# facebookresearch/PartDistillation

Measured on AMD Instinct MI355X. Metric: images/sec training step, R50 Mask2Former 1024² bs=2/GPU, 1/2/4/8 MI355X, higher is better.
Workload: dtype bf16

## Files before the change

### include/pd_fused.h

```cpp
#ifndef PD_FUSED_H
#define PD_FUSED_H

#include <stdint.h>

#ifdef __cplusplus
extern "C" {
#endif

int pd_maxpool3s2_fwd_bf16(const void *x, void *y, void *argmax, int B, int H, int W, int C, void *stream);
int pd_maxpool3s2_bwd_bf16(const void *dy, const void *argmax, void *dx, int B, int H, int W, int C, void *stream);

int pd_affine_act_fwd_bf16(const void *x, const void *residual, const float *scale, const float *bias, void *y,
                           int64_t n, int channels, int relu, void *stream);

int pd_affine_act_bwd_bf16(const void *gy, const void *y, const float *scale, void *gx, void *gres, int64_t n,
                           int channels, int relu, void *stream);
int pd_affine_act_bwd2_bf16(const void *gy, const void *gy2, const void *y, const float *scale, void *gx, void *gres, int64_t n,
                            int channels, int relu, void *stream);

int pd_multi_gather_sumsq(const int64_t *src_ptrs, const int32_t *src_is_bf16, const int32_t *blk_tensor,
                          const int64_t *blk_start, const int64_t *blk_dst, const int32_t *blk_len, float *dst,
                          double *sumsq, int block_begin, int block_end, void *stream);

int pd_nc_sums_f32(const float *x, const float *dy, const float *y, const float *a, const float *b, double *out, int N, int P,
                   int C, int mode, int relu, void *stream);
int pd_nc_affine_f32(const float *x, const float *a, const float *b, float *y, int N, int P, int C, int relu, void *stream);
int pd_nc_affine_amax_f32(const float *x, const float *a, const float *b, float *y, float *amax, int N, int P, int C, int relu, void *stream);
int pd_nc_affine2_amax_f32(const float *dy, const float *x, const float *y, const float *a, const float *p, const float *r, float *dx,
                           float *amax, int N, int P, int C, int relu, void *stream);
int pd_nc_affine2_f32(const float *dy, const float *x, const float *y, const float *a, const float *p, const float *r, float *dx,
                      int N, int P, int C, int relu, void *stream);

int pd_gn_coeffs_fwd(const double *sums, const float *weight, const float *bias, int N, int C, int G, int P, float eps, float *a,
                     float *b, float *mean_c, float *rstd_c, float *xb, void *stream);
int pd_gn_coeffs_bwd(const double *sums, const float *weight, const float *mean_c, const float *rstd_c, int N, int C, int G, int P,
                     float *a, float *pcoef, float *rcoef, float *gw, float *gb, void *stream);

#ifdef __cplusplus
}
#endif
#endif
```

### include/pd_gemm.h

```cpp
#ifndef PD_GEMM_H
#define PD_GEMM_H

#include <stdint.h>

#ifdef __cplusplus
extern "C" {
#endif

int pd_gemm_tn_f32(const float *A, const float *B, const float *bias, float *C, int M, int N, int K, int lda, int ldb,
                   int ldc, int relu, void *stream);

int pd_gemm_tn_f32x3(const float *A, const float *B, const float *bias, float *C, int M, int N, int K, int lda, int ldb,
                     int ldc, int relu, void *stream);

int pd_gemm_wgrad_f32(const float *dY, const float *X, float *dW, float *dB, int M, int N, int K, int ldy, int ldx,
                      int ldw, void *stream);

int pd_gemm_wgrad_acc_f32(const float *dY, const float *X, float *dW, float *dB, int M, int N, int K, int ldy, int ldx,
                          int ldw, void *stream);

int64_t pd_gemm_tn_f32x3_relu_bits_words(int M, int N);
int pd_split3_bf16(const float *W, int N, int K, int ldw, int transpose, void *planes, void *stream);
int pd_gemm_tn_f32x3_pre(const float *A, const void *Bplanes, const float *bias, float *C, uint32_t *bits, float *colsum, int M, int N, int K,
                         int lda, int ldc, int mode, void *stream);
int pd_gemm_tn_f32x3_relu_bits(const float *A, const float *B, const float *bias, float *C, uint32_t *bits, int M, int N, int K, int lda,
                               int ldb, int ldc, void *stream);
int pd_gemm_tn_f32x3_relumask(const float *A, const float *B, const uint32_t *bits, float *C, float *colsum, int M, int N, int K, int lda,
                              int ldb, int ldc, void *stream);

int pd_gemm_wgrad_acc_f32x3(const float *dY, const float *X, float *dW, float *dB, int M, int N, int K, int ldy, int ldx, int ldw,
                            void *stream);
int64_t pd_gemm_wgrad_f32x3_ws_floats(int N, int K);
int pd_gemm_wgrad_acc_f32x3_ws(const float *dY, const float *X, float *dW, float *dB, float *workspace, int64_t workspace_floats, int M, int N,
                               int K, int ldy, int ldx, int ldw, void *stream);

typedef struct PdGemmWgradDesc {
  const float *dY, *X;
  float *dW, *dB;
  int M, N, K, ldy, ldx, ldw;
  const float *y_amax, *x_amax;
} PdGemmWgradDesc;
int64_t pd_gemm_wgrad_f32x3_grouped_table_bytes(int max_count);
int64_t pd_gemm_wgrad_f32x3_grouped_ws_floats(const PdGemmWgradDesc *descs, int count);
int pd_gemm_wgrad_f32x3_grouped(const PdGemmWgradDesc *descs, int count, void *table_host_pinned, void *table_device, float *workspace,
                                int64_t workspace_floats, void *stream);

int pd_conv3x3_wgrad_nhwc_f32x3(const float *dY, const float *X, float *dWk, float *dB, float *workspace, int64_t workspace_floats, int B, int H,
                                int W, int Ci, int Co, void *stream);

int pd_conv3x3_nhwc_f32x3(const float *X, const float *Wk, const float *bias, float *Y, int B, int H, int W, int Ci, int Co,
                          void *stream);

int64_t pd_gemm_wgrad_f16x2_ws_floats(int N, int K);
int pd_gemm_wgrad_f16x2_takes_wide_tiles(int N, int K);
int64_t pd_gemm_wgrad_f16x2_grouped_ws_floats(const PdGemmWgradDesc *descs, int count);
int pd_gemm_wgrad_acc_f16x2_ws(const float *dY, const float *X, float *dW, float *dB, const float *y_amax, const float *x_amax,
                               float *workspace, int64_t workspace_floats, int M, int N, int K, int ldy, int ldx, int ldw, void *stream);
int pd_gemm_wgrad_f16x2_grouped(const PdGemmWgradDesc *descs, int count, void *table_host_pinned, void *table_device, float *workspace,
                                int64_t workspace_floats, void *stream);
int pd_conv3x3_wgrad_nhwc_f16x2(const float *dY, const float *X, float *dWk, float *dB, const float *y_amax, const float *x_amax,
                                float *workspace, int64_t workspace_floats, int B, int H, int W, int Ci, int Co, void *stream);
int pd_gemm_tn_f16x2_which(int M, int N, int K, int lda, int ldb, int mode, int has_bits, int has_a_amax, int has_b_amax, int has_c_amax,
                           int bf16_out);

int pd_conv3x3_nhwc_f16x2(const float *X, const float *Wk, const float *bias, float *Y, const float *x_amax, const float *w_amax, float *y_amax,
                          int B, int H, int W, int Ci, int Co, void *stream);
int64_t pd_gemm_tn_f16x2_bits_words(int M, int N);
int pd_gemm_tn_f16x2(const float *A, const float *B, const float *bias, float *C, uint32_t *bits, float *colsum, const float *a_amax,
                     const float *b_amax, float *c_amax, int M, int N, int K, int lda, int ldb, int ldc, int mode, void *stream);
int pd_row_amax_f32(const float *X, int rows, int cols, int ld, float *out, void *stream);
int pd_gemm_tn_f16x2_bf16out(const float *A, const float *B, const float *bias, void *C_bf16, const float *a_amax, const float *b_amax, int M, int N,
                             int K, int lda, int ldb, int ldc, void *stream);
int pd_cast_bf16_f32_amax(const void *X_bf16, int rows, int cols, float *Y, float *row_amax, void *stream);

#ifdef __cplusplus
}
#endif
#endif
```

### include/pd_rowwise.h

```cpp
#ifndef PD_ROWWISE_H
#define PD_ROWWISE_H

#include <stdint.h>

#ifdef __cplusplus
extern "C" {
#endif

int pd_add_layernorm_fwd(const void *x, int x_dtype, const float *res, const float *gamma, const float *beta, float eps,
                         float *z, float *y, void *y_c, const float *pos, int pos_div, void *ypos_c, int c_dtype,
                         float *mean, float *rstd, int rows, int C, void *stream);

int pd_add_layernorm_bwd(const float *dy, const float *dy2, const void *dy_c, const void *dypos_c, int c_dtype,
                         const float *z, const float *mean, const float *rstd, const float *gamma, float *dz, void *dz_c,
                         int dzc_dtype, float *dgamma, float *dbeta, float *dbias, float *dpos_acc, int pos_div,
                         int rows, int C, void *stream);

int pd_add_layernorm_fwd_amax(const void *x, int x_dtype, const float *res, const float *gamma, const float *beta, float eps,
                              float *z, float *y, void *y_c, const float *pos, int pos_div, void *ypos_c, int c_dtype,
                              float *mean, float *rstd, float *y_amax, float *ypos_amax, int rows, int C, void *stream);
int pd_add_layernorm_bwd_amax(const float *dy, const float *dy2, const void *dy_c, const void *dypos_c, int c_dtype,
                              const float *z, const float *mean, const float *rstd, const float *gamma, float *dz, void *dz_c,
                              int dzc_dtype, float *dgamma, float *dbeta, float *dbias, float *dpos_acc, int pos_div,
                              float *dz_amax, int rows, int C, void *stream);

int pd_colsum_acc(const void *x, int dtype, int rows, int N, float *acc, void *stream);

int pd_relu_bwd_colsum(void *dh, const void *h, int dtype, int rows, int N, float *acc, void *stream);

int pd_mem_prep_fwd(const float *tok, int64_t tok_batch_stride, const float *level_embed, const float *pos, void *mem_c,
                    void *mempos_c, int c_dtype, int B, int HW, int C, void *stream);

int pd_mem_prep_bwd(const void *dmem_c, const void *dmempos_c, int c_dtype, float *dtok, int64_t dtok_batch_stride, int B,
                    int HW, int C, void *stream);

int pd_attn_mask_u8(const void *logits, int dtype, int rows, int n, uint8_t *mask, void *stream);

int pd_matcher_point_terms(const void *x, int dtype, int rows, int n, float *x_f32, float *sigmoid_x, float *softplus_sum,
                           float *sigmoid_sum, void *stream);

int pd_msda_prep_fwd(const float *offs, const float *logits, const float *ref, const int64_t *spatial_shapes, float *loc,
                     float *attn, int64_t tokens, int M, int L, int P, int ld_offs, int ld_logits, void *stream);

int pd_msda_prep_bwd(const float *gloc, const float *gattn, const float *attn, const int64_t *spatial_shapes, float *d_offs,
                     float *d_logits, int64_t tokens, int M, int L, int P, int ld_offs, int ld_logits, void *stream);
int pd_msda_prep_bwd_amax(const float *gloc, const float *gattn, const float *attn, const int64_t *spatial_shapes, float *d_offs, float *d_logits,
                          float *row_amax, int64_t tokens, int M, int L, int P, int ld_offs, int ld_logits, void *stream);

int pd_point_sample_nhwc_f32(const float *in, const float *coords, float *out, int B, int H, int W, int C, int P, void *stream);
int pd_point_sample_nhwc_f32_bf16(const float *in, const float *coords, void *out, int B, int H, int W, int C, int P, void *stream);

int pd_point_sample_planar_f32(const float *in, const float *coords, float *out, int N, int C, int H, int W, int P, void *stream);
int pd_point_sample_planar_bwd_f32(const float *grad_out, const float *coords, float *grad_in, int N, int C, int H, int W, int P, void *stream);
int pd_point_sample_planar_bwd_needs_zero(int C, int H, int W);
int pd_point_sample_planar_bwd_needs_zero_n(int N, int C, int H, int W);

int pd_upsample_add_nhwc_f32(const float *lo, int64_t lo_batch_stride, const float *cur, float *y, int B, int h, int w, int H, int W, int C, void *stream);
int pd_upsample_add_amax_nhwc_f32(const float *lo, int64_t lo_batch_stride, const float *cur, float *y, float *amax, int B, int h, int w, int H, int W, int C,
                                  void *stream);
int pd_upsample2x_bwd_nhwc_f32(const float *dy, float *dlo, int B, int h, int w, int C, void *stream);

#define PD_RESIZE_MAX 4
int pd_resize_bilinear_nhwc_f32(const float *x, int B, int H, int W, int C, const int *heights, const int *widths, void *const *outs, int count,
                                int out_dtype, void *stream);


int pd_add_rows_amax_f32(const float *a, const float *b, float *q, float *a_copy, float *a_amax, float *q_amax, int rows, int cols, void *stream);

int pd_sum3_sum2_f32(const float *a, const float *b, const float *c, const float *d, float *out1, float *out2, int64_t n, void *stream);

int pd_skinny_linear_fwd(const void *x_bf16, const void *w, const void *b, int wb_dtype, float *y, int R, int C, int K, void *stream);
int64_t pd_skinny_linear_partial_floats(int R, int C, int K);
int pd_skinny_linear_bwd(const void *x_bf16, const void *w, int w_dtype, const float *dy, const void *dx_in_bf16, void *dx_out, int dx_dtype,
                         float *partial, void *dw, void *db, int b_dtype, int R, int C, int K, void *stream);

#define PD_TRANSPOSE_MAX 8
typedef struct {
  const void *src;
  void *dst;
  int64_t src_batch_stride, src_row_stride;
  int32_t batch, rows, cols, reserved;
} PdTransposeProblem;
int pd_transpose_batched_f32(const PdTransposeProblem *problems, int count, void *stream);

#define PD_COPY_MAX_SEGS 48
typedef struct PdCopySeg {
  const void *src;
  void *dst;
  int64_t bytes;
} PdCopySeg;
int pd_copy_segments(const PdCopySeg *segs, int count, void *stream);

#ifdef __cplusplus
}
#endif
#endif
```

### partdistillation_amd/csrc/cmdbuf.hip

```cpp
#include <hip/hip_runtime.h>
#include <stdint.h>
#include <string.h>

#include <type_traits>
#include <utility>

#include "pd_common.h"
#include "pd_cmdbuf.h"
#include "pd_attention.h"
#include "pd_conv.h"
#include "pd_declayer.h"
#include "pd_criterion.h"
#include "pd_fused.h"
#include "pd_gemm.h"
#include "pd_grouping.h"
#include "pd_igemm.h"
#include "pd_input.h"
#include "pd_kmeans.h"
#include "pd_msda.h"
#include "pd_mx8.h"
#include "pd_optim.h"
#include "pd_poly.h"
#include "pd_rowwise.h"
#include "pd_smallgemm.h"
// ... 11 lines not shown
  } else if constexpr (std::is_same_v<T, float>) {
    float f; uint32_t u = (uint32_t)w; memcpy(&f, &u, 4); return f;
  } else if constexpr (std::is_same_v<T, double>) {
    double d; memcpy(&d, &w, 8); return d;
  } else {
    return static_cast<T>(static_cast<int64_t>(w));
  }
}

template <auto F> struct Thunk;
template <class... A, int (*F)(A...)>
struct Thunk<F> {
  static constexpr int nargs = (int)sizeof...(A);
  template <size_t... I>
  static int invoke(const uint64_t *w, std::index_sequence<I...>) { return F(word_to<A>(w[I])...); }
  static int call(const uint64_t *w) { return invoke(w, std::index_sequence_for<A...>{}); }
};

struct Entry { const char *name; int (*call)(const uint64_t *); int nargs; };
#define PD_E(f) {#f, &Thunk<&f>::call, Thunk<&f>::nargs}
const Entry kTable[] = {
  PD_E(pd_adamw_clipped),
  PD_E(pd_adamw_clipped_shadow),
  PD_E(pd_add_layernorm_bwd),
  PD_E(pd_add_layernorm_bwd_amax),
  PD_E(pd_add_layernorm_fwd),
  PD_E(pd_add_layernorm_fwd_amax),
  PD_E(pd_add_rows_amax_f32),
  PD_E(pd_affine_act_bwd2_bf16),
  PD_E(pd_affine_act_bwd_bf16),
  PD_E(pd_affine_act_fwd_bf16),
  PD_E(pd_attn_bwd_d32),
  PD_E(pd_attn_fwd_d32),
  PD_E(pd_attn_mask_u8),
  PD_E(pd_cast_bf16_f32_amax),
  PD_E(pd_colsum_acc),
  PD_E(pd_conv3x3_nhwc_f16x2),
  PD_E(pd_conv3x3_nhwc_f32x3),
  PD_E(pd_conv3x3_wgrad_nhwc_f16x2),
  PD_E(pd_conv3x3_wgrad_nhwc_f32x3),
  PD_E(pd_conv_bf16_dgrad),
  PD_E(pd_conv_bf16_fwd),
  PD_E(pd_conv_bf16_wgrad),
  PD_E(pd_conv_bf16_wgrad_grouped),
  PD_E(pd_dec_bwd_a),
  PD_E(pd_dec_bwd_b),
  PD_E(pd_dec_fwd_a),
  PD_E(pd_dec_fwd_b),
  PD_E(pd_dec_pack_grouped),
  PD_E(pd_decoder_head_bf16),
  PD_E(pd_filter_transpose_grouped),
  PD_E(pd_gemm_tn_f16x2),
  PD_E(pd_gemm_tn_f16x2_bf16out),
  PD_E(pd_gemm_tn_f32),
  PD_E(pd_gemm_tn_f32x3),
  PD_E(pd_gemm_tn_f32x3_pre),
  PD_E(pd_gemm_tn_f32x3_relu_bits),
  PD_E(pd_gemm_tn_f32x3_relumask),
  PD_E(pd_gemm_wgrad_acc_f16x2_ws),
  PD_E(pd_gemm_wgrad_acc_f32),
  PD_E(pd_gemm_wgrad_acc_f32x3),
  PD_E(pd_gemm_wgrad_acc_f32x3_ws),
  PD_E(pd_gemm_wgrad_f16x2_grouped),
  PD_E(pd_gemm_wgrad_f32),
  PD_E(pd_gemm_wgrad_f32x3_grouped),
  PD_E(pd_gn_coeffs_bwd),
  PD_E(pd_gn_coeffs_fwd),
  PD_E(pd_igemm_bf16),
  PD_E(pd_igemm_bf16_seq),
  PD_E(pd_kmeans_assign),
  PD_E(pd_kmeans_assign_bounded),
  PD_E(pd_kmeans_assign_partial),
  PD_E(pd_kmeans_reduce),
  PD_E(pd_kmeans_reduce_update),
  PD_E(pd_kmeans_reduce_update_shift),
  PD_E(pd_kmeans_update),
  PD_E(pd_layernorm_rows_f32_bwd),
  PD_E(pd_layernorm_rows_f32_fwd),
  PD_E(pd_loss_vectors_bwd),
  PD_E(pd_loss_vectors_fwd),
  PD_E(pd_lsa_batched),
  PD_E(pd_mask_assign),
  PD_E(pd_mask_point_losses_bwd),
  PD_E(pd_mask_point_losses_fwd),
  PD_E(pd_matcher_costs),
  PD_E(pd_copy_segments),
  PD_E(pd_attn_fwd_d32_ld),
  PD_E(pd_attn_bwd_d32_ld),
  PD_E(pd_match_point_logits),
  PD_E(pd_swin_merge_ln_fwd),
  PD_E(pd_swin_tail_ln_fwd),
  PD_E(pd_swin_tail_ln_bwd),
  PD_E(pd_swin_merge_ln_bwd),
  PD_E(pd_matcher_point_terms),
  PD_E(pd_maxpool3s2_bwd_bf16),
  PD_E(pd_maxpool3s2_fwd_bf16),
  PD_E(pd_mem_prep_bwd),
  PD_E(pd_mem_prep_fwd),
  PD_E(pd_memcpy_d2d_async),
  PD_E(pd_memset_async),
  PD_E(pd_msda_backward),
  PD_E(pd_msda_forward),
  PD_E(pd_msda_forward_amax),
  PD_E(pd_msda_fused_backward),
  PD_E(pd_msda_fused_forward),
  PD_E(pd_msda_prep_bwd),
  PD_E(pd_msda_prep_bwd_amax),
  PD_E(pd_msda_prep_fwd),
  PD_E(pd_multi_gather_sumsq),
  PD_E(pd_mx8_gemm),
  PD_E(pd_mx8_quantize_bf16),
  PD_E(pd_mx8_quantize_grouped),
  PD_E(pd_nc_affine2_amax_f32),
  PD_E(pd_nc_affine2_f32),
  PD_E(pd_nc_affine_amax_f32),
  PD_E(pd_nc_affine_f32),
  PD_E(pd_nc_sums_f32),
  PD_E(pd_normalize_u8_nhwc),
  PD_E(pd_pair_logits_bwd_rows),
  PD_E(pd_pair_logits_bwd_tok),
  PD_E(pd_pair_logits_fwd),
  PD_E(pd_point_sample_nhwc_f32),
  PD_E(pd_point_sample_nhwc_f32_bf16),
  PD_E(pd_point_sample_planar_bwd_f32),
  PD_E(pd_point_sample_planar_f32),
  PD_E(pd_point_sample_u8),
  PD_E(pd_poly_crossings_i32),
  PD_E(pd_relu_bwd_colsum),
  PD_E(pd_resample_cols_canvas_u8),
  PD_E(pd_resample_cols_u8),
  PD_E(pd_resample_rows_u8),
  PD_E(pd_resize_bilinear_nhwc_f32),
  PD_E(pd_rle_sample_groups_canvas_u8),
  PD_E(pd_rle_sample_groups_u8),
  PD_E(pd_rle_sample_u8),
  PD_E(pd_row_amax_f32),
  PD_E(pd_scores_argmax_u8),
  PD_E(pd_sgemm_nn_bf16),
  PD_E(pd_sgemm_nn_splitn_bf16),
  PD_E(pd_sgemm_tn_batched_bf16),
  PD_E(pd_sgemm_tn_bf16),
  PD_E(pd_sgemm_tn_multi_bf16),
  PD_E(pd_sgemm_tn_splitk_bf16),
  PD_E(pd_sgemm_wgrad_bf16),
  PD_E(pd_sgemm_wgrad_grouped_bf16),
  PD_E(pd_sgemm_wgrad_split_bf16),
  PD_E(pd_skinny_linear_bwd),
  PD_E(pd_skinny_linear_fwd),
  PD_E(pd_split3_bf16),
  PD_E(pd_stem7x7_fwd),
  PD_E(pd_stem7x7_wgrad),
  PD_E(pd_sum3_sum2_f32),
  PD_E(pd_sumsq_accumulate),
  PD_E(pd_swin_ln_bwd),
  PD_E(pd_swin_ln_fwd),
  PD_E(pd_transpose_batched_f32),
  PD_E(pd_uncertain_points),
  PD_E(pd_upsample2x_bwd_nhwc_f32),
  PD_E(pd_upsample_add_amax_nhwc_f32),
  PD_E(pd_upsample_add_nhwc_f32),
  PD_E(pd_wgrad_bf16),
  PD_E(pd_wgrad_bf16_seq),
  PD_E(pd_window_attn_bwd_w12),
  PD_E(pd_window_attn_bwd_w7),
  PD_E(pd_window_attn_fwd_w12),
  PD_E(pd_window_attn_fwd_w7),
};
constexpr int kCount = (int)(sizeof(kTable) / sizeof(kTable[0]));
}

extern "C" int pd_memset_async(void *dst, int value, int64_t bytes, void *stream)
{
  if (bytes <= 0) return PD_OK;
  return hipMemsetAsync(dst, value, (size_t)bytes, (hipStream_t)stream) == hipSuccess ? PD_OK : pd_set_error(PD_ERR_LAUNCH, "pd_memset_async failed");
}

extern "C" int pd_memcpy_d2d_async(void *dst, const void *src, int64_t bytes, void *stream)
{
  if (bytes <= 0) return PD_OK;
  return hipMemcpyAsync(dst, src, (size_t)bytes, hipMemcpyDeviceToDevice, (hipStream_t)stream) == hipSuccess ? PD_OK
                                                                                                         : pd_set_error(PD_ERR_LAUNCH, "pd_memcpy_d2d_async failed");
}

extern "C" int pd_cmd_fn_index(const char *name)
{
  if (!name) return -1;
  for (int i = 0; i < kCount; ++i)
    if (!strcmp(kTable[i].name, name)) return i;
  return -1;
}

extern "C" int pd_cmd_fn_nargs(int fn) { return fn >= 0 && fn < kCount ? kTable[fn].nargs : -1; }

extern "C" int pd_cmd_replay(const PdCmd *cmds, int count, const uint64_t *slot_bases, int nslots, void *stream)
{
  uint64_t w[PD_CMD_MAX_ARGS];
  for (int c = 0; c < count; ++c) {
    const PdCmd &k = cmds[c];
    if (k.fn < 0 || k.fn >= kCount || k.nargs != kTable[k.fn].nargs || k.nargs > PD_CMD_MAX_ARGS)
      return pd_set_error(PD_ERR_INVALID_ARG, "pd_cmd_replay: command %d is malformed", c);
    for (int i = 0; i < k.nargs; ++i) {
      const int s = k.kind[i];
      if (s == PD_CMD_LITERAL) w[i] = k.a[i];
      else if (s == PD_CMD_STREAM) w[i] = (uint64_t)(uintptr_t)stream;
      else if (s >= 0 && s < nslots) w[i] = slot_bases[s] + k.a[i];
      else return pd_set_error(PD_ERR_INVALID_ARG, "pd_cmd_replay: command %d argument %d names slot %d of %d", c, i, s, nslots);
    }
    const int rc = kTable[k.fn].call(w);
    if (rc != PD_OK) return rc;
  }
  return PD_OK;
// ... 2 lines not shown
```

### partdistillation_amd/csrc/common.hip

```cpp
#include <hip/hip_runtime.h>
#include <stdarg.h>
#include <stdio.h>
#include <string.h>

#include "pd_common.h"
#include "pd_msda.h"

namespace {
thread_local char g_err[512] = {0};
}

int pd_set_error(int code, const char *fmt, ...)
{
  va_list ap;
  va_start(ap, fmt);
  vsnprintf(g_err, sizeof(g_err), fmt, ap);
  va_end(ap);
  return code;
}

int pd_check_launch(const char *what)
{
  hipError_t e = hipGetLastError();
  if (e == hipSuccess) return PD_OK;
  return pd_set_error(PD_ERR_LAUNCH, "%s: %s", what, hipGetErrorString(e));
}

extern "C" const char *pd_last_error(void) { return g_err; }
extern "C" int pd_abi_version(void) { return 49; }

extern int g_pd_dbg_atomic_scope;
extern int g_pd_dbg_force_generic;
extern int g_pd_dbg_ablate;
extern int g_pd_dbg_x3_narrow;
extern int g_pd_dbg_f16x2;
extern int g_pd_dbg_wgrad_wide;
extern "C" void pd_dbg_set_wgrad_xcd(int v);
extern "C" void pd_dbg_set_wgrad_fast(int v);
extern int g_pd_dbg_bwd_variant;
extern int g_pd_dbg_msda_gate_pct;
extern int g_pd_dbg_wgrad_wgs;
extern int g_pd_dbg_bwd_threads;
extern int g_pd_dbg_attn_scalar;
extern int g_pd_dbg_wattn;
extern int g_pd_dbg_wattn_chunk;
extern int g_pd_dbg_x3;
extern int g_pd_dbg_kmeans;
extern int g_pd_dbg_conv_group_rows;
extern int g_pd_dbg_conv_xcd_major;
extern int g_pd_dbg_sgemm_deep;
extern int g_ig_bn, g_ig_nst, g_ig_splits, g_ig_patch, g_ig_pcls;
extern int g_mx_bn, g_mx_nst;
extern int g_swin_ln_abl;
extern int g_ln_bwd_cap;
extern int g_crit_abl;
extern int g_attn_bwd_kc;
extern int g_wg_nst, g_wg_splits, g_wg_mode;
extern "C" int pd_debug_set(const char *key, int value)
{
  if (!key) return PD_ERR_INVALID_ARG;
  if (!strcmp(key, "msda_bwd_atomic_scope")) { g_pd_dbg_atomic_scope = value; return PD_OK; }
  if (!strcmp(key, "msda_ablate")) { g_pd_dbg_ablate = value; return PD_OK; }
  if (!strcmp(key, "msda_bwd_variant")) { g_pd_dbg_bwd_variant = value; return PD_OK; }
  if (!strcmp(key, "msda_gate_pct")) { g_pd_dbg_msda_gate_pct = value; return PD_OK; }
  if (!strcmp(key, "attn_scalar")) { g_pd_dbg_attn_scalar = value; return PD_OK; }
  if (!strcmp(key, "msda_bwd_threads")) { g_pd_dbg_bwd_threads = value; return PD_OK; }
  if (!strcmp(key, "wgrad_wgs")) { g_pd_dbg_wgrad_wgs = value; return PD_OK; }
  if (!strcmp(key, "kmeans_ablate")) { g_pd_dbg_kmeans = value; return PD_OK; }
  if (!strcmp(key, "wg_nst")) { g_wg_nst = value; return PD_OK; }
  if (!strcmp(key, "wg_splits")) { g_wg_splits = value; return PD_OK; }
  if (!strcmp(key, "wg_mode")) { g_wg_mode = value; return PD_OK; }
  if (!strcmp(key, "ig_bn")) { g_ig_bn = value; return PD_OK; }
  if (!strcmp(key, "ig_patch")) { g_ig_patch = value; return PD_OK; }
  if (!strcmp(key, "ig_pcls")) { g_ig_pcls = value; return PD_OK; }
  if (!strcmp(key, "ig_nst")) { g_ig_nst = value; return PD_OK; }
  if (!strcmp(key, "mx_bn")) { g_mx_bn = value; return PD_OK; }
  if (!strcmp(key, "attn_bwd_kc")) { g_attn_bwd_kc = value; return PD_OK; }
  if (!strcmp(key, "crit_abl")) { g_crit_abl = value; return PD_OK; }
  if (!strcmp(key, "ln_bwd_cap")) { g_ln_bwd_cap = value; return PD_OK; }
  if (!strcmp(key, "swin_ln_abl")) { g_swin_ln_abl = value; return PD_OK; }
  if (!strcmp(key, "mx_nst")) { g_mx_nst = value; return PD_OK; }
  if (!strcmp(key, "ig_splits")) { g_ig_splits = value; return PD_OK; }
  if (!strcmp(key, "sgemm_deep")) { g_pd_dbg_sgemm_deep = value; return PD_OK; }
  if (!strcmp(key, "conv_group_rows")) { g_pd_dbg_conv_group_rows = value; return PD_OK; }
  if (!strcmp(key, "conv_xcd_major")) { g_pd_dbg_conv_xcd_major = value; return PD_OK; }
  if (!strcmp(key, "x3_ablate")) { g_pd_dbg_x3 = value; return PD_OK; }
  if (!strcmp(key, "f16x2_tile")) { g_pd_dbg_f16x2 = value; return PD_OK; }
  if (!strcmp(key, "wgrad_wide")) { g_pd_dbg_wgrad_wide = value; return PD_OK; }
  if (!strcmp(key, "wgrad_xcd")) { pd_dbg_set_wgrad_xcd(value); return PD_OK; }
  if (!strcmp(key, "wgrad_fast")) { pd_dbg_set_wgrad_fast(value); return PD_OK; }
  if (!strcmp(key, "x3_narrow")) { g_pd_dbg_x3_narrow = value; return PD_OK; }
  if (!strcmp(key, "wattn_ablate")) { g_pd_dbg_wattn = value; return PD_OK; }
  if (!strcmp(key, "wattn_chunk")) {
    if (value < 0 || value > 8) return pd_set_error(PD_ERR_INVALID_ARG, "pd_debug_set: wattn_chunk is 0 (automatic) or 1..8, got %d", value);
    g_pd_dbg_wattn_chunk = value;
    return PD_OK;
  }
  if (!strcmp(key, "msda_force_generic")) { g_pd_dbg_force_generic = value; return PD_OK; }
  return pd_set_error(PD_ERR_INVALID_ARG, "pd_debug_set: unknown key %s", key);
}

extern "C" int pd_debug_get(const char *key, int *value)
{
  if (!key || !value) return PD_ERR_INVALID_ARG;
  if (!strcmp(key, "msda_bwd_variant")) { *value = g_pd_dbg_bwd_variant; return PD_OK; }
  if (!strcmp(key, "msda_gate_pct")) { *value = g_pd_dbg_msda_gate_pct; return PD_OK; }
  return pd_set_error(PD_ERR_INVALID_ARG, "pd_debug_get: unknown key %s", key);
}
```

### partdistillation_amd/csrc/fused.hip

```cpp
#include <hip/hip_runtime.h>
#include <stdlib.h>
#include <hip/hip_bf16.h>
#include <stdint.h>

#include "pd_common.h"
#include "pd_fused.h"
#include "pd_msda.h"

namespace {

typedef unsigned short u16x8 __attribute__((ext_vector_type(8)));

__device__ __forceinline__ float bf2f(unsigned short h) { return __uint_as_float((unsigned)h << 16); }
__device__ __forceinline__ unsigned short f2bf(float f)
{
  unsigned u = __float_as_uint(f);
  if ((u & 0x7fffffffu) > 0x7f800000u) return (unsigned short)((u >> 16) | 0x40);
  u += 0x7fffu + ((u >> 16) & 1u);
  return (unsigned short)(u >> 16);
}

__global__ __launch_bounds__(256) void maxpool3s2_fwd(const u16x8 *__restrict__ x, u16x8 *__restrict__ y, unsigned long long *__restrict__ arg,
                                                      int B, int H, int W, int OH, int OW, int c8)
{
// ... 134 lines not shown
  const int b = block_begin + blockIdx.x;
  const int t = blk_tensor[b];
  const int64_t start = blk_start[b];
  const int len = blk_len[b];
  float *d = dst + blk_dst[b];
  const int64_t base = src_ptrs[t];
  float acc = 0.f;
  if (base == 0) {
    for (int i = threadIdx.x; i < len; i += 256) d[i] = 0.f;
  } else if (is_bf16[t]) {
    const unsigned short *s = pd_as_global(reinterpret_cast<const unsigned short *>(base)) + start;
    if ((((uintptr_t)s | (uintptr_t)d) & 15) == 0) {
      const int l8 = len >> 3;
      for (int i = threadIdx.x; i < l8; i += 256) {
        const uint4 u = reinterpret_cast<const uint4 *>(s)[i];
        const float4 a = make_float4(__uint_as_float(u.x << 16), __uint_as_float(u.x & 0xffff0000u), __uint_as_float(u.y << 16), __uint_as_float(u.y & 0xffff0000u));
        const float4 c = make_float4(__uint_as_float(u.z << 16), __uint_as_float(u.z & 0xffff0000u), __uint_as_float(u.w << 16), __uint_as_float(u.w & 0xffff0000u));
        reinterpret_cast<float4 *>(d)[2 * i] = a;
        reinterpret_cast<float4 *>(d)[2 * i + 1] = c;
        acc += (a.x * a.x + a.y * a.y + a.z * a.z + a.w * a.w) + (c.x * c.x + c.y * c.y + c.z * c.z + c.w * c.w);
      }
      for (int i = (l8 << 3) + threadIdx.x; i < len; i += 256) { const float v = bf2f(s[i]); d[i] = v; acc += v * v; }
    } else {
      for (int i = threadIdx.x; i < len; i += 256) { const float v = bf2f(s[i]); d[i] = v; acc += v * v; }
    }
  } else {
    const float *s = pd_as_global(reinterpret_cast<const float *>(base)) + start;
    if ((((uintptr_t)s | (uintptr_t)d) & 15) == 0) {
      const int l4 = len >> 2;
      for (int i = threadIdx.x; i < l4; i += 256) {
        const float4 v = reinterpret_cast<const float4 *>(s)[i];
        reinterpret_cast<float4 *>(d)[i] = v;
        acc += v.x * v.x + v.y * v.y + v.z * v.z + v.w * v.w;
      }
      for (int i = (l4 << 2) + threadIdx.x; i < len; i += 256) { const float v = s[i]; d[i] = v; acc += v * v; }
    } else {
      for (int i = threadIdx.x; i < len; i += 256) { const float v = s[i]; d[i] = v; acc += v * v; }
    }
  }
  if (sumsq) {
    double a = (double)acc;
#pragma unroll
    for (int o = 32; o > 0; o >>= 1) a += __shfl_xor(a, o, 64);
    __shared__ double part[4];
    if ((threadIdx.x & 63) == 0) part[threadIdx.x >> 6] = a;
    __syncthreads();
    if (threadIdx.x == 0) unsafeAtomicAdd(sumsq, part[0] + part[1] + part[2] + part[3]);
  }
}

template <int MODE>
__global__ __launch_bounds__(256) void nc_sums(const float *__restrict__ x, const float *__restrict__ dy, const float *__restrict__ y,
                                                const float *__restrict__ a, const float *__restrict__ b, double *__restrict__ out,
                                                int P, int C, int pix_per_block, int relu)
{
  __shared__ float red[2][256][4];
  const int n = blockIdx.y, cq = C >> 2, q = threadIdx.x % cq, po = threadIdx.x / cq, pstride = 256 / cq;
  const int p0 = blockIdx.x * pix_per_block, p1 = min(P, p0 + pix_per_block);
  const int64_t base = (int64_t)n * P * C + q * 4;
  float4 s0 = make_float4(0, 0, 0, 0), s1 = s0, av = s0, bv = s0;
  if (MODE == 1) { av = *reinterpret_cast<const float4 *>(a + n * C + q * 4); bv = *reinterpret_cast<const float4 *>(b + n * C + q * 4); }
#pragma unroll 4
  for (int p = p0 + po; p < p1; p += pstride) {
    const float4 xv = *reinterpret_cast<const float4 *>(x + base + (int64_t)p * C);
    if (MODE == 0) {
      s0.x += xv.x; s0.y += xv.y; s0.z += xv.z; s0.w += xv.w;
      s1.x += xv.x * xv.x; s1.y += xv.y * xv.y; s1.z += xv.z * xv.z; s1.w += xv.w * xv.w;
    } else {
      float4 g = *reinterpret_cast<const float4 *>(dy + base + (int64_t)p * C);
      if (relu) {
        const float4 yv = *reinterpret_cast<const float4 *>(y + base + (int64_t)p * C);
        g.x = yv.x > 0 ? g.x : 0; g.y = yv.y > 0 ? g.y : 0; g.z = yv.z > 0 ? g.z : 0; g.w = yv.w > 0 ? g.w : 0;
      }
      s0.x += g.x * (xv.x * av.x + bv.x); s0.y += g.y * (xv.y * av.y + bv.y);
      s0.z += g.z * (xv.z * av.z + bv.z); s0.w += g.w * (xv.w * av.w + bv.w);
      s1.x += g.x; s1.y += g.y; s1.z += g.z; s1.w += g.w;
    }
  }
  red[0][threadIdx.x][0] = s0.x; red[0][threadIdx.x][1] = s0.y; red[0][threadIdx.x][2] = s0.z; red[0][threadIdx.x][3] = s0.w;
  red[1][threadIdx.x][0] = s1.x; red[1][threadIdx.x][1] = s1.y; red[1][threadIdx.x][2] = s1.z; red[1][threadIdx.x][3] = s1.w;
  __syncthreads();
  if (threadIdx.x < C) {
    const int c = threadIdx.x, qq = c >> 2, e = c & 3;
    double t0 = 0, t1 = 0;
    for (int k = 0; k < pstride; ++k) { t0 += red[0][k * cq + qq][e]; t1 += red[1][k * cq + qq][e]; }
    unsafeAtomicAdd(out + ((int64_t)n * C + c) * 2, t0);
    unsafeAtomicAdd(out + ((int64_t)n * C + c) * 2 + 1, t1);
  }
}

__device__ __forceinline__ void pixel_amax_store(float4 v, float *__restrict__ amax, int64_t i)
{
  float m = fmaxf(fmaxf(fabsf(v.x), fabsf(v.y)), fmaxf(fabsf(v.z), fabsf(v.w)));
#pragma unroll
  for (int o = 32; o; o >>= 1) m = fmaxf(m, __shfl_xor(m, o, 64));
  if ((threadIdx.x & 63) == 0) amax[i >> 6] = m;
}

template <bool RELU>
__global__ __launch_bounds__(256) void nc_affine(const float4 *__restrict__ x, const float *__restrict__ a, const float *__restrict__ b,
                                                  float4 *__restrict__ y, int64_t n4, int P, int C, float *__restrict__ amax)
{
  const int cq = C >> 2;
  const int64_t stride = (int64_t)gridDim.x * blockDim.x, per_img = (int64_t)P * cq;
  for (int64_t i = (int64_t)blockIdx.x * blockDim.x + threadIdx.x; i < n4; i += stride) {
    const int n = (int)(i / per_img), q = (int)(i % cq);
    const float4 av = *reinterpret_cast<const float4 *>(a + n * C + q * 4), bv = *reinterpret_cast<const float4 *>(b + n * C + q * 4);
    float4 v = x[i];
    v.x = v.x * av.x + bv.x; v.y = v.y * av.y + bv.y; v.z = v.z * av.z + bv.z; v.w = v.w * av.w + bv.w;
    if (RELU) { v.x = fmaxf(v.x, 0.f); v.y = fmaxf(v.y, 0.f); v.z = fmaxf(v.z, 0.f); v.w = fmaxf(v.w, 0.f); }
    y[i] = v;
    if (amax) pixel_amax_store(v, amax, i);
  }
}

template <bool RELU>
__global__ __launch_bounds__(256) void nc_affine2(const float4 *__restrict__ dy, const float4 *__restrict__ x, const float4 *__restrict__ y,
                                                   const float *__restrict__ a, const float *__restrict__ pc, const float *__restrict__ rc,
                                                   float4 *__restrict__ dx, int64_t n4, int P, int C, float *__restrict__ amax)
{
  const int cq = C >> 2;
  const int64_t stride = (int64_t)gridDim.x * blockDim.x, per_img = (int64_t)P * cq;
  for (int64_t i = (int64_t)blockIdx.x * blockDim.x + threadIdx.x; i < n4; i += stride) {
    const int n = (int)(i / per_img), q = (int)(i % cq);
    const float4 av = *reinterpret_cast<const float4 *>(a + n * C + q * 4), pv = *reinterpret_cast<const float4 *>(pc + n * C + q * 4),
                 rv = *reinterpret_cast<const float4 *>(rc + n * C + q * 4);
    float4 g = dy[i];
    const float4 xv = x[i];
    if (RELU) {
      const float4 yv = y[i];
      g.x = yv.x > 0 ? g.x : 0; g.y = yv.y > 0 ? g.y : 0; g.z = yv.z > 0 ? g.z : 0; g.w = yv.w > 0 ? g.w : 0;
    }
    const float4 o = make_float4(g.x * av.x + xv.x * pv.x + rv.x, g.y * av.y + xv.y * pv.y + rv.y, g.z * av.z + xv.z * pv.z + rv.z,
                                 g.w * av.w + xv.w * pv.w + rv.w);
    dx[i] = o;
    if (amax) pixel_amax_store(o, amax, i);
  }
}

inline int grid_for(int64_t n) { int64_t b = (n + 255) / 256; return (int)(b < 1 ? 1 : (b > 8192 ? 8192 : b)); }


__global__ __launch_bounds__(256) void gn_coeffs_fwd(const double *__restrict__ sums, const float *__restrict__ weight,
                                                     const float *__restrict__ bias, int N, int C, int G, double m, double eps,
                                                     float *__restrict__ a, float *__restrict__ b, float *__restrict__ mean_c,
                                                     float *__restrict__ rstd_c, float *__restrict__ xb)
{
  const int i = blockIdx.x * blockDim.x + threadIdx.x;
  if (i >= N * C) return;
  const int n = i / C, c = i - n * C, cpg = C / G, c0 = (c / cpg) * cpg;
  double s0 = 0.0, s1 = 0.0;
  for (int j = 0; j < cpg; ++j) {
    s0 += sums[((int64_t)n * C + c0 + j) * 2];
    s1 += sums[((int64_t)n * C + c0 + j) * 2 + 1];
  }
  const double mean = s0 / m;
  double var = s1 / m - mean * mean;
  var = var < 0.0 ? 0.0 : var;
  const float rstd = (float)(1.0 / sqrt(var + eps)), mu = (float)mean;
  const float av = rstd * weight[c];
  a[i] = av;
  b[i] = bias[c] - mu * av;
  mean_c[i] = mu;
  rstd_c[i] = rstd;
  xb[i] = -mu * rstd;
}

__global__ __launch_bounds__(256) void gn_coeffs_bwd(const double *__restrict__ sums, const float *__restrict__ weight,
                                                     const float *__restrict__ mean_c, const float *__restrict__ rstd_c, int N,
                                                     int C, int G, double m, float *__restrict__ a, float *__restrict__ pcoef,
                                                     float *__restrict__ rcoef, float *__restrict__ gw, float *__restrict__ gb)
{
  const int i = blockIdx.x * blockDim.x + threadIdx.x;
  if (i >= N * C) return;
  const int n = i / C, c = i - n * C, cpg = C / G, c0 = (c / cpg) * cpg;
  double S1 = 0.0, S2 = 0.0;
  for (int j = 0; j < cpg; ++j) {
    const double w = (double)weight[c0 + j];
    S1 += sums[((int64_t)n * C + c0 + j) * 2] * w;
    S2 += sums[((int64_t)n * C + c0 + j) * 2 + 1] * w;
  }
  S1 /= m; S2 /= m;
// ... 52 lines not shown
  dim3 g(grid_for(n8)), b(256);
#define LAUNCH(R, A) hipLaunchKernelGGL((affine_act_fwd<R, A>), g, b, 0, s, (const u16x8 *)x, (const u16x8 *)residual, scale, bias, (u16x8 *)y, n8, c8)
  if (residual) { if (relu) LAUNCH(true, true); else LAUNCH(true, false); }
  else { if (relu) LAUNCH(false, true); else LAUNCH(false, false); }
#undef LAUNCH
  return pd_check_launch("pd_affine_act_fwd_bf16");
}

extern "C" int pd_affine_act_bwd2_bf16(const void *gy, const void *gy2, const void *y, const float *scale, void *gx, void *gres, int64_t n,
                                       int channels, int relu, void *stream_)
{
  if (n < 0 || channels <= 0 || (channels & 7) || (n % channels)) return pd_set_error(PD_ERR_INVALID_ARG, "pd_affine_act_bwd_bf16: n=%lld channels=%d", (long long)n, channels);
  if (n == 0) return PD_OK;
  if (!gy || !scale || !gx || (relu && !y)) return pd_set_error(PD_ERR_INVALID_ARG, "pd_affine_act_bwd_bf16: null pointer");
  const int64_t n8 = n / 8;
  const int c8 = channels / 8;
  hipStream_t s = (hipStream_t)stream_;
  dim3 g(grid_for(n8)), b(256);
#define LAUNCH(R, A, T) hipLaunchKernelGGL((affine_act_bwd<R, A, T>), g, b, 0, s, (const u16x8 *)gy, (const u16x8 *)gy2, (const u16x8 *)y, scale, (u16x8 *)gx, (u16x8 *)gres, n8, c8)
#define LAUNCH2(R, A) do { if (gy2) LAUNCH(R, A, true); else LAUNCH(R, A, false); } while (0)
  if (gres) { if (relu) LAUNCH2(true, true); else LAUNCH2(true, false); }
  else { if (relu) LAUNCH2(false, true); else LAUNCH2(false, false); }
#undef LAUNCH2
#undef LAUNCH
  return pd_check_launch("pd_affine_act_bwd_bf16");
}

extern "C" int pd_affine_act_bwd_bf16(const void *gy, const void *y, const float *scale, void *gx, void *gres, int64_t n,
                                      int channels, int relu, void *stream_)
{
  return pd_affine_act_bwd2_bf16(gy, nullptr, y, scale, gx, gres, n, channels, relu, stream_);
}

extern "C" int pd_multi_gather_sumsq(const int64_t *src_ptrs, const int32_t *src_is_bf16, const int32_t *blk_tensor,
                                     const int64_t *blk_start, const int64_t *blk_dst, const int32_t *blk_len, float *dst,
                                     double *sumsq, int block_begin, int block_end, void *stream_)
{
  if (block_end < block_begin) return pd_set_error(PD_ERR_INVALID_ARG, "pd_multi_gather_sumsq: bad block range");
  if (block_end == block_begin) return PD_OK;
  if (!src_ptrs || !src_is_bf16 || !blk_tensor || !blk_start || !blk_dst || !blk_len || !dst)
    return pd_set_error(PD_ERR_INVALID_ARG, "pd_multi_gather_sumsq: null pointer");
  hipLaunchKernelGGL(multi_gather_sumsq, dim3(block_end - block_begin), dim3(256), 0, (hipStream_t)stream_, src_ptrs, src_is_bf16,
                     blk_tensor, blk_start, blk_dst, blk_len, dst, sumsq, block_begin);
  return pd_check_launch("pd_multi_gather_sumsq");
}

static int nc_check(int N, int P, int C, const char *who)
{
  if (N < 0 || P < 0 || C <= 0 || (C & 3) || (256 % (C >> 2)) != 0 || C > 256)
    return pd_set_error(PD_ERR_INVALID_ARG, "%s: N=%d P=%d C=%d (C must be 4*2^k <= 256)", who, N, P, C);
  return PD_OK;
}

extern "C" int pd_nc_sums_f32(const float *x, const float *dy, const float *y, const float *a, const float *b, double *out,
                              int N, int P, int C, int mode, int relu, void *stream_)
{
  int rc = nc_check(N, P, C, "pd_nc_sums_f32");
  if (rc) return rc;
  if (!out) return pd_set_error(PD_ERR_INVALID_ARG, "pd_nc_sums_f32: null output");
  hipStream_t s = (hipStream_t)stream_;
  (void)hipMemsetAsync(out, 0, (size_t)N * C * 2 * sizeof(double), s);
  if ((int64_t)N * P == 0) return pd_check_launch("pd_nc_sums_f32");
  if (!x || (mode == 1 && (!dy || !a || !b || (relu && !y)))) return pd_set_error(PD_ERR_INVALID_ARG, "pd_nc_sums_f32: null input");
  static const int ppb_env = []() { const char *e = getenv("PD_NC_PPB"); return e ? atoi(e) : 0; }();
  const int64_t np = (int64_t)N * P;
  int ppb = mode == 0 ? (np >= 131072 ? 512 : np >= 32768 ? 256 : np >= 8192 ? 128 : 64) : (np >= 131072 ? 256 : np >= 32768 ? 128 : 32);
  if (ppb_env > 0) ppb = ppb_env;
  dim3 grid((P + ppb - 1) / ppb, N);
  if (mode == 0) hipLaunchKernelGGL(nc_sums<0>, grid, dim3(256), 0, s, x, dy, y, a, b, out, P, C, ppb, relu);
  else hipLaunchKernelGGL(nc_sums<1>, grid, dim3(256), 0, s, x, dy, y, a, b, out, P, C, ppb, relu);
  return pd_check_launch("pd_nc_sums_f32");
}

static int nc_affine_launch(const float *x, const float *a, const float *b, float *y, int N, int P, int C, int relu, void *stream_, float *amax)
{
  int rc = nc_check(N, P, C, "pd_nc_affine_f32");
  if (amax && C != 256) return pd_set_error(PD_ERR_INVALID_ARG, "pd_nc_affine_amax_f32: pixel maxima need C == 256");
  if (rc) return rc;
  const int64_t n4 = (int64_t)N * P * C / 4;
  if (n4 == 0) return PD_OK;
  if (!x || !a || !b || !y) return pd_set_error(PD_ERR_INVALID_ARG, "pd_nc_affine_f32: null pointer");
  hipStream_t s = (hipStream_t)stream_;
  if (relu) hipLaunchKernelGGL(nc_affine<true>, dim3(grid_for(n4)), dim3(256), 0, s, (const float4 *)x, a, b, (float4 *)y, n4, P, C, amax);
  else hipLaunchKernelGGL(nc_affine<false>, dim3(grid_for(n4)), dim3(256), 0, s, (const float4 *)x, a, b, (float4 *)y, n4, P, C, amax);
  return pd_check_launch("pd_nc_affine_f32");
}

extern "C" int pd_nc_affine_f32(const float *x, const float *a, const float *b, float *y, int N, int P, int C, int relu, void *stream_)
{
  return nc_affine_launch(x, a, b, y, N, P, C, relu, stream_, nullptr);
}

extern "C" int pd_nc_affine_amax_f32(const float *x, const float *a, const float *b, float *y, float *amax, int N, int P, int C, int relu, void *stream_)
{
  return nc_affine_launch(x, a, b, y, N, P, C, relu, stream_, amax);
}

static int nc_affine2_launch(const float *dy, const float *x, const float *y, const float *a, const float *p, const float *r,
                             float *dx, int N, int P, int C, int relu, void *stream_, float *amax)
{
  int rc = nc_check(N, P, C, "pd_nc_affine2_f32");
  if (amax && C != 256) return pd_set_error(PD_ERR_INVALID_ARG, "pd_nc_affine2_amax_f32: pixel maxima need C == 256");
  if (rc) return rc;
  const int64_t n4 = (int64_t)N * P * C / 4;
  if (n4 == 0) return PD_OK;
  if (!dy || !x || !a || !p || !r || !dx || (relu && !y)) return pd_set_error(PD_ERR_INVALID_ARG, "pd_nc_affine2_f32: null pointer");
  hipStream_t s = (hipStream_t)stream_;
  if (relu) hipLaunchKernelGGL(nc_affine2<true>, dim3(grid_for(n4)), dim3(256), 0, s, (const float4 *)dy, (const float4 *)x, (const float4 *)y, a, p, r, (float4 *)dx, n4, P, C, amax);
  else hipLaunchKernelGGL(nc_affine2<false>, dim3(grid_for(n4)), dim3(256), 0, s, (const float4 *)dy, (const float4 *)x, (const float4 *)y, a, p, r, (float4 *)dx, n4, P, C, amax);
  return pd_check_launch("pd_nc_affine2_f32");
}

extern "C" int pd_nc_affine2_f32(const float *dy, const float *x, const float *y, const float *a, const float *p, const float *r,
                                 float *dx, int N, int P, int C, int relu, void *stream_)
{
  return nc_affine2_launch(dy, x, y, a, p, r, dx, N, P, C, relu, stream_, nullptr);
}

extern "C" int pd_nc_affine2_amax_f32(const float *dy, const float *x, const float *y, const float *a, const float *p, const float *r,
                                      float *dx, float *amax, int N, int P, int C, int relu, void *stream_)
{
  return nc_affine2_launch(dy, x, y, a, p, r, dx, N, P, C, relu, stream_, amax);
}

extern "C" int pd_gn_coeffs_fwd(const double *sums, const float *weight, const float *bias, int N, int C, int G, int P, float eps,
                                float *a, float *b, float *mean_c, float *rstd_c, float *xb, void *stream_)
{
  if (N < 0 || C <= 0 || G <= 0 || (C % G) || P <= 0) return pd_set_error(PD_ERR_INVALID_ARG, "pd_gn_coeffs_fwd: N=%d C=%d G=%d P=%d", N, C, G, P);
  if (N == 0) return PD_OK;
  if (!sums || !weight || !bias || !a || !b || !mean_c || !rstd_c || !xb) return pd_set_error(PD_ERR_INVALID_ARG, "pd_gn_coeffs_fwd: null pointer");
  hipLaunchKernelGGL(gn_coeffs_fwd, dim3((N * C + 255) / 256), dim3(256), 0, (hipStream_t)stream_, sums, weight, bias, N, C, G,
                     (double)P * (C / G), (double)eps, a, b, mean_c, rstd_c, xb);
  return pd_check_launch("pd_gn_coeffs_fwd");
}

extern "C" int pd_gn_coeffs_bwd(const double *sums, const float *weight, const float *mean_c, const float *rstd_c, int N, int C,
                                int G, int P, float *a, float *pcoef, float *rcoef, float *gw, float *gb, void *stream_)
{
  if (N < 0 || C <= 0 || G <= 0 || (C % G) || P <= 0) return pd_set_error(PD_ERR_INVALID_ARG, "pd_gn_coeffs_bwd: N=%d C=%d G=%d P=%d", N, C, G, P);
  if (N == 0) return PD_OK;
  if (!sums || !weight || !mean_c || !rstd_c || !a || !pcoef || !rcoef || !gw || !gb) return pd_set_error(PD_ERR_INVALID_ARG, "pd_gn_coeffs_bwd: null pointer");
  hipLaunchKernelGGL(gn_coeffs_bwd, dim3((N * C + 255) / 256), dim3(256), 0, (hipStream_t)stream_, sums, weight, mean_c, rstd_c, N, C,
                     G, (double)P * (C / G), a, pcoef, rcoef, gw, gb);
  return pd_check_launch("pd_gn_coeffs_bwd");
}
```

### partdistillation_amd/csrc/gemm_f16x2.hip

```cpp
#include <hip/hip_runtime.h>
#include <stdint.h>
#include <stdlib.h>
#include <utility>
#include <type_traits>

#include "f16x2.h"
#include "pd_common.h"
#include "xcd.h"
#include "pd_gemm.h"
#include "pd_msda.h"

#ifndef PD_ABL
#define PD_ABL 0
#endif

namespace {
using namespace pdh2;
__device__ __forceinline__ int xcd_chunk(int bid, int nb) { return pd_xcd_chunk(bid, nb); }
__device__ __forceinline__ unsigned short f2bf_rne(float f)
{
  unsigned u = __float_as_uint(f);
  if ((u & 0x7fffffffu) > 0x7f800000u) return (unsigned short)((u >> 16) | 0x40u);
  u += 0x7fffu + ((u >> 16) & 1u);
  return (unsigned short)(u >> 16);
}

template <int TM, int TN, int WN, int BKK, int MODE, bool CONV = false, int NRS = 1, int FAST = 0>
__global__ __launch_bounds__((TM / 64) * (TN / WN) * 64, (TM == 256 ? 1 : 2))
void gemm_tn_f16x2(const float *__restrict__ A, const float *__restrict__ B, const float *__restrict__ bias, float *__restrict__ C,
                   int M, int N, int K, int lda, int ldb, int ldc, int ntiles_n, uint32_t *__restrict__ bits,
                   float *__restrict__ colsum, const float *__restrict__ a_amax, const float *__restrict__ b_amax,
                   unsigned *__restrict__ c_amax, int H, int W, int tap_minor)
{
  constexpr int WVN = TN / WN, NW = (TM / 64) * WVN, NTH = NW * 64, NJ = WN / 32;
  constexpr int TPR = BKK / 4, RPP = NTH / TPR, APASS = TM / RPP, BPASS = TN / RPP, NPAN = BKK / 8;
  static_assert(TM % RPP == 0 && TN % RPP == 0, "staging passes");
  constexpr int ASZ = 2 * NPAN * TM * 8, BSZ = 2 * NPAN * TN * 8;
  extern __shared__ __attribute__((aligned(16))) float sc[];
  h16_t *smem = reinterpret_cast<h16_t *>(sc + 2 * (TM + TN));
  auto As = [&](int buf, int pl, int pan, int r) -> h16_t * { return smem + buf * (ASZ + BSZ) + (((pl * NPAN + pan) * TM + r) << 3); };
  auto Bs = [&](int buf, int pl, int pan, int r) -> h16_t * { return smem + buf * (ASZ + BSZ) + ASZ + (((pl * NPAN + pan) * TN + r) << 3); };
  const int lb = xcd_chunk(blockIdx.x, gridDim.x);
  const int m0 = (lb / ntiles_n) * TM, n0 = (lb % ntiles_n) * TN;
  const int t = threadIdx.x, lane = t & 63, wave = t >> 6;
  const int wm = (wave / WVN) * 64, wn = (wave % WVN) * WN;
  const int lr = t / TPR, lk = (t % TPR) * 4;
  for (int r = t; r < TM + TN; r += NTH) {
    const bool isa = r < TM;
    const int g = isa ? m0 + r : n0 + r - TM;
    const float *am = isa ? a_amax : b_amax;
    float s = 1.f, inv = 1.f;
    if (!(PD_ABL & 32) && am && g < (isa ? M : N)) {
      float mx = am[g];
      if (CONV && isa) {
        const int pix = g % (H * W), y = pix / W, x = pix - y * W;
#pragma unroll
        for (int dy = -1; dy <= 1; ++dy)
#pragma unroll
          for (int dx = -1; dx <= 1; ++dx)
            if (y + dy >= 0 && y + dy < H && x + dx >= 0 && x + dx < W) mx = fmaxf(mx, am[g + dy * W + dx]);
      }
      row_scale(mx, s, inv);
    }
    sc[r] = s; sc[TM + TN + r] = inv;
  }
  __syncthreads();
  float sa[APASS], sb[BPASS];
#pragma unroll
  for (int j = 0; j < APASS; ++j) sa[j] = sc[lr + RPP * j];
#pragma unroll
  for (int j = 0; j < BPASS; ++j) sb[j] = sc[TM + lr + RPP * j];
  float4 ra[NRS][APASS], rb[NRS][BPASS];
  int py[APASS], px[APASS];
  if (CONV) {
#pragma unroll
    for (int j = 0; j < APASS; ++j) {
      const int pix = (m0 + lr + RPP * j) % (H * W);
      py[j] = pix / W;
      px[j] = pix - py[j] * W;
    }
  }
  auto gload = [&](int rs, int k0) {
    if (PD_ABL & 8) {
#pragma unroll
      for (int j = 0; j < APASS; ++j) ra[rs][j] = make_float4(1.f, 0.5f, 0.25f, (float)k0);
#pragma unroll
      for (int j = 0; j < BPASS; ++j) rb[rs][j] = make_float4(1.f, 0.5f, 0.25f, (float)k0);
      return;
    }
    const int k = k0 + lk;
    int dy = 0, dx = 0, kc = k, kb = k;
    if (CONV) {
      int tap;
      if (tap_minor) { const int s = k0 / BKK; const int cb = s / 9; tap = s - cb * 9; kc = cb * BKK + lk; kb = tap * lda + kc; }
// ... 942 lines not shown
        }
        hipLaunchKernelGGL(split_planes_f16x2, dim3((unsigned)(((int64_t)N * (K / 4) + 255) / 256)), dim3(256), 0, st, B, ldb, b_amax, planes, N, K);
        const float *bpl = reinterpret_cast<const float *>(planes);
        if (p.abl == 16) KPC(true, 16, true, bpl);
        else if (a_amax) KPC(true, 0, true, bpl);
        else KPC(false, 0, true, bpl);
        return pd_check_launch("pd_gemm_tn_f16x2 (producer / consumer wavefronts, weight planes)");
      }
      if (p.abl) {
        with_constant(p.abl, KpcAbl{}, [&](auto abl) { KPC(true, decltype(abl)::value, false, B); });
        return pd_check_launch("pd_gemm_tn_f16x2 (producer / consumer wavefronts, ablation)");
      }
#endif
      if (a_amax) KPC(true, 0, false, B);
      else KPC(false, 0, false, B);
#undef KPC
      return pd_check_launch("pd_gemm_tn_f16x2 (producer / consumer wavefronts)");
    }
#define GO(TM, TN, WN, NRS, FAST) return launch_f16x2<TM, TN, WN, 16, false, NRS, FAST>(A, B, bias, C, M, N, K, lda, ldb, ldc, mode, bits, colsum, a_amax, b_amax, c_amax, st, flags)
    case F16X2_TILE256:
      if (p.refuse)
        return pd_set_error(PD_ERR_INVALID_ARG, bits ? "pd_gemm_tn_f16x2: sign bits need N %% 256 == 0 and M >= 1024" : "pd_gemm_tn_f16x2: 256 x 256 tiles need N %% 256 == 0 and M >= 1024");
      if (p.nrs == 1) GO(256, 256, 128, 1, 0);
      if (!p.fast) GO(256, 256, 128, 2, 0);
      GO(256, 256, 128, 2, 1);
    default:
      if (p.nrs == 1) GO(128, 128, 64, 1, 0);
      if (!p.fast) GO(128, 128, 64, 2, 0);
      GO(128, 128, 64, 2, 1);
#undef GO
  }
}

extern "C" int pd_gemm_tn_f16x2_which(int M, int N, int K, int lda, int ldb, int mode, int has_bits, int has_a_amax, int has_b_amax, int has_c_amax,
                                      int bf16_out)
{
  const F16x2Plan p = f16x2_plan(M, N, K, lda, ldb, mode, has_bits != 0, has_a_amax != 0, has_b_amax != 0, has_c_amax != 0, bf16_out != 0, g_pd_dbg_f16x2,
                                 cu_count());
  return p.refuse ? -1 : (int)p.family;
}

extern "C" int pd_gemm_tn_f16x2(const float *A, const float *B, const float *bias, float *C, uint32_t *bits, float *colsum, const float *a_amax,
                                const float *b_amax, float *c_amax, int M, int N, int K, int lda, int ldb, int ldc, int mode, void *stream_)
{
  return gemm_tn_f16x2_impl(A, B, bias, C, bits, colsum, a_amax, b_amax, c_amax, M, N, K, lda, ldb, ldc, mode, stream_, 0);
}

extern "C" int pd_gemm_tn_f16x2_bf16out(const float *A, const float *B, const float *bias, void *C_bf16, const float *a_amax, const float *b_amax,
                                        int M, int N, int K, int lda, int ldb, int ldc, void *stream_)
{
  return gemm_tn_f16x2_impl(A, B, bias, reinterpret_cast<float *>(C_bf16), nullptr, nullptr, a_amax, b_amax, nullptr, M, N, K, lda, ldb, ldc, 0, stream_, 1);
}

extern "C" int pd_cast_bf16_f32_amax(const void *X_bf16, int rows, int cols, float *Y, float *row_amax, void *stream_)
{
  if (rows < 0 || cols <= 0 || (cols & 7)) return pd_set_error(PD_ERR_INVALID_ARG, "pd_cast_bf16_f32_amax: rows=%d cols=%d (a multiple of 8)", rows, cols);
  if (rows == 0) return PD_OK;
  if (!X_bf16 || !Y || !row_amax || ((uintptr_t)X_bf16 & 15) || ((uintptr_t)Y & 15)) return pd_set_error(PD_ERR_INVALID_ARG, "pd_cast_bf16_f32_amax: null / misaligned pointer");
  hipLaunchKernelGGL(cast_bf16_f32_amax, dim3((unsigned)((rows + 3) / 4)), dim3(256), 0, (hipStream_t)stream_, (const unsigned short *)X_bf16, rows, cols, Y,
                     row_amax);
  return pd_check_launch("pd_cast_bf16_f32_amax");
}

extern "C" int pd_conv3x3_nhwc_f16x2(const float *X, const float *Wk, const float *bias, float *Y, const float *x_amax, const float *w_amax,
                                     float *y_amax, int B, int H, int W, int Ci, int Co, void *stream_)
{
  if (B < 0 || H <= 0 || W <= 0 || Ci <= 0 || Co <= 0 || (Ci & 15))
    return pd_set_error(PD_ERR_INVALID_ARG, "pd_conv3x3_nhwc_f16x2: B=%d H=%d W=%d Ci=%d (%% 16) Co=%d", B, H, W, Ci, Co);
  if (B == 0) return PD_OK;
  if (!X || !Wk || !Y || ((uintptr_t)X & 15) || ((uintptr_t)Wk & 15)) return pd_set_error(PD_ERR_INVALID_ARG, "pd_conv3x3_nhwc_f16x2: null / misaligned pointer");
  const int64_t M = (int64_t)B * H * W;
  if (M > 0x7fffffffLL - 4096) return pd_set_error(PD_ERR_INVALID_ARG, "pd_conv3x3_nhwc_f16x2: too many pixels");
  hipStream_t st = (hipStream_t)stream_;
  const int dbg = g_pd_dbg_f16x2;
#ifdef PD_PROBES
  if ((dbg == DBG_KPC_ANY || dbg == DBG_KPC_PLANES_STAMPS) && x_amax && w_amax && !y_amax && (Co % 256) == 0 && (Ci % KR_KC) == 0 && ((Ci / KR_KC) & (Ci / KR_KC - 1)) == 0 && M >= 8192 &&
      H < 65536 && W < 65536 && M * Ci * 4 < (1ll << 31) && (int64_t)Co * 9 * Ci * 4 < (1ll << 31)) {
    const int np = Co / 256, G = items_grid(cu_count(), M, np);
    if (dbg == DBG_KPC_PLANES_STAMPS) {
      launch_lds<gemm_kpc_f16x2<true, 16, false, true>>(G, 768, KP_LDS, st, X, Wk, bias, Y, (int)M, 9 * Ci, Ci, 9 * Ci, Co, np, x_amax, w_amax, H, W);
      return pd_check_launch("pd_conv3x3_nhwc_f16x2 (producer / consumer wavefronts, stamps)");
    }
    launch_lds<gemm_kpc_f16x2<true, 0, false, true>>(G, 768, KP_LDS, st, X, Wk, bias, Y, (int)M, 9 * Ci, Ci, 9 * Ci, Co, np, x_amax, w_amax, H, W);
    return pd_check_launch("pd_conv3x3_nhwc_f16x2 (producer / consumer wavefronts)");
  }
#endif
  const bool wide = dbg == DBG_WIDE_1 || (dbg != DBG_TILE_1 && (Co % 256) == 0 && M >= 65536);
  if (dbg == DBG_GUARDED || dbg == DBG_CONV_KORDER) {
    if (wide) return launch_f16x2<256, 256, 128, 16, true>(X, Wk, bias, Y, (int)M, Co, 9 * Ci, Ci, 9 * Ci, Co, 0, nullptr, nullptr, x_amax, w_amax, y_amax, st, H, W);
    return launch_f16x2<128, 128, 64, 16, true>(X, Wk, bias, Y, (int)M, Co, 9 * Ci, Ci, 9 * Ci, Co, 0, nullptr, nullptr, x_amax, w_amax, y_amax, st, H, W);
  }
  if (wide) return launch_f16x2<256, 256, 128, 16, true, 1, 1>(X, Wk, bias, Y, (int)M, Co, 9 * Ci, Ci, 9 * Ci, Co, 0, nullptr, nullptr, x_amax, w_amax, y_amax, st, H, W);
  return launch_f16x2<128, 128, 64, 16, true, 1, 1>(X, Wk, bias, Y, (int)M, Co, 9 * Ci, Ci, 9 * Ci, Co, 0, nullptr, nullptr, x_amax, w_amax, y_amax, st, H, W);
}

extern "C" int pd_row_amax_f32(const float *X, int rows, int cols, int ld, float *out, void *stream_)
{
  if (rows < 0 || cols < 0) return pd_set_error(PD_ERR_INVALID_ARG, "pd_row_amax_f32: negative size");
  if (rows == 0) return PD_OK;
  if (!X || !out) return pd_set_error(PD_ERR_INVALID_ARG, "pd_row_amax_f32: null pointer");
  hipLaunchKernelGGL(row_amax_f32, dim3((unsigned)((rows + 3) / 4)), dim3(256), 0, (hipStream_t)stream_, X, rows, cols, ld, out);
  return pd_check_launch("pd_row_amax_f32");
}

extern "C" int pd_debug_read_kpc_trace(unsigned long long *dst)
{
// ... 3 lines not shown
```

### partdistillation_amd/csrc/rowwise.hip

```cpp
#include <hip/hip_runtime.h>
#include <stdint.h>
#include <string.h>

#include "pd_common.h"
#include "pd_msda.h"
#include "pd_rowwise.h"

int g_ln_bwd_cap = 0;
namespace {

typedef unsigned short bf16_t;

__device__ __forceinline__ float bf2f(bf16_t h) { return __uint_as_float((unsigned)h << 16); }
__device__ __forceinline__ bf16_t f2bf(float f)
{
  unsigned u = __float_as_uint(f);
  if ((u & 0x7fffffffu) > 0x7f800000u) return (bf16_t)((u >> 16) | 0x40);
  u += 0x7fffu + ((u >> 16) & 1u);
  return (bf16_t)(u >> 16);
}

__device__ __forceinline__ float4 ld4(const float *p) { return *reinterpret_cast<const float4 *>(p); }
__device__ __forceinline__ float4 ld4(const bf16_t *p)
{
// ... 606 lines not shown
    const int lx = x0 - tx0, ly = y0 - ty0;
    float acc = 0.f;
    if (vy0 && vx0) acc += tile[ly * (PST + 1) + lx] * wnw;
    if (vy0 && vx1) acc += tile[ly * (PST + 1) + lx + 1] * wne;
    if (vy1 && vx0) acc += tile[(ly + 1) * (PST + 1) + lx] * wsw;
    if (vy1 && vx1) acc += tile[(ly + 1) * (PST + 1) + lx + 1] * wse;
    out[(int64_t)n * P + p] = acc;
  }
}

__global__ __launch_bounds__(256) void point_sample_tiled_bwd(const float *__restrict__ gout, const float *__restrict__ coords,
                                                              float *__restrict__ gin, int H, int W, int P, int tiles_x)
{
  extern __shared__ float tile[];
  const int n = blockIdx.y, ty0 = (blockIdx.x / tiles_x) * PST, tx0 = (blockIdx.x % tiles_x) * PST;
  for (int i = threadIdx.x; i < PST * PST; i += 256) tile[i] = 0.f;
  __syncthreads();
  const float *cn = coords + (int64_t)n * P * 2, *gn = gout + (int64_t)n * P;
  for (int p = threadIdx.x; p < P; p += 256) {
    const float2 c = *reinterpret_cast<const float2 *>(cn + 2 * p);
    const float gx = 2.0f * c.x - 1.0f, gy = 2.0f * c.y - 1.0f;
    const float ix = ((gx + 1.f) * W - 1.f) / 2.f, iy = ((gy + 1.f) * H - 1.f) / 2.f;
    const float fx = floorf(ix), fy = floorf(iy);
    if (fx < tx0 - 1.f || fx >= tx0 + PST || fy < ty0 - 1.f || fy >= ty0 + PST) continue;
    const int x0 = (int)fx, y0 = (int)fy, x1 = x0 + 1, y1 = y0 + 1;
    const float g = gn[p];
    const float wnw = (x1 - ix) * (y1 - iy), wne = (ix - x0) * (y1 - iy), wsw = (x1 - ix) * (iy - y0), wse = (ix - x0) * (iy - y0);
    const int lx0 = x0 - tx0, ly0 = y0 - ty0, lx1 = lx0 + 1, ly1 = ly0 + 1;
    const bool ax0 = lx0 >= 0 && lx0 < PST && x0 < W, ax1 = lx1 >= 0 && lx1 < PST && x1 < W;
    const bool ay0 = ly0 >= 0 && ly0 < PST && y0 < H, ay1 = ly1 >= 0 && ly1 < PST && y1 < H;
    if (ay0 && ax0) atomicAdd(&tile[ly0 * PST + lx0], g * wnw);
    if (ay0 && ax1) atomicAdd(&tile[ly0 * PST + lx1], g * wne);
    if (ay1 && ax0) atomicAdd(&tile[ly1 * PST + lx0], g * wsw);
    if (ay1 && ax1) atomicAdd(&tile[ly1 * PST + lx1], g * wse);
  }
  __syncthreads();
  float *m = gin + (int64_t)n * H * W;
  for (int i = threadIdx.x; i < PST * PST; i += 256) {
    const int y = ty0 + i / PST, x = tx0 + i % PST;
    if (y < H && x < W) m[(int64_t)y * W + x] = tile[i];
  }
}

__device__ __forceinline__ void up_src(int dst, float scale, int in_size, int &i0, int &ip, float &l0, float &l1)
{
  float src = scale * (dst + 0.5f) - 0.5f;
  src = src < 0.f ? 0.f : src;
  i0 = (int)src;
  ip = (i0 < in_size - 1) ? 1 : 0;
  l1 = src - i0;
  l0 = 1.f - l1;
}

__global__ __launch_bounds__(256) void upsample_add_nhwc(const float *__restrict__ lo, const float *__restrict__ cur,
                                                         float *__restrict__ y, int B, int h, int w, int H, int W, int C4,
                                                         float sh, float sw, float *__restrict__ amax, int64_t lo_bs4)
{
  const int64_t total = (int64_t)B * H * W * C4;
  for (int64_t i = (int64_t)blockIdx.x * blockDim.x + threadIdx.x; i < total; i += (int64_t)gridDim.x * blockDim.x) {
    const int c = (int)(i % C4);
    int64_t t = i / C4;
    const int ox = (int)(t % W); t /= W;
    const int oy = (int)(t % H);
    const int b = (int)(t / H);
    int y0, yp, x0, xp; float hy0, hy1, wx0, wx1;
    up_src(oy, sh, h, y0, yp, hy0, hy1);
    up_src(ox, sw, w, x0, xp, wx0, wx1);
    const float4 *L = reinterpret_cast<const float4 *>(lo) + (int64_t)b * lo_bs4;
    const float4 a = L[((int64_t)y0 * w + x0) * C4 + c], bq = L[((int64_t)y0 * w + x0 + xp) * C4 + c];
    const float4 cq = L[((int64_t)(y0 + yp) * w + x0) * C4 + c], d = L[((int64_t)(y0 + yp) * w + x0 + xp) * C4 + c];
    const float4 u = reinterpret_cast<const float4 *>(cur)[i];
    float4 o;
    o.x = u.x + (hy0 * (wx0 * a.x + wx1 * bq.x) + hy1 * (wx0 * cq.x + wx1 * d.x));
    o.y = u.y + (hy0 * (wx0 * a.y + wx1 * bq.y) + hy1 * (wx0 * cq.y + wx1 * d.y));
    o.z = u.z + (hy0 * (wx0 * a.z + wx1 * bq.z) + hy1 * (wx0 * cq.z + wx1 * d.z));
    o.w = u.w + (hy0 * (wx0 * a.w + wx1 * bq.w) + hy1 * (wx0 * cq.w + wx1 * d.w));
    reinterpret_cast<float4 *>(y)[i] = o;
    if (amax) {
      float m = amax4(o);
#pragma unroll
      for (int of = 32; of; of >>= 1) m = fmaxf(m, __shfl_xor(m, of, 64));
      if ((threadIdx.x & 63) == 0) amax[i >> 6] = m;
    }
  }
}

struct ResizeLevels { void *out[PD_RESIZE_MAX]; int h[PD_RESIZE_MAX], w[PD_RESIZE_MAX]; int64_t first[PD_RESIZE_MAX + 1]; int count; };

template <bool BF16>
__global__ __launch_bounds__(256) void resize_bilinear_nhwc_multi(const float *__restrict__ x, int B, int H, int W, int C4, ResizeLevels lv)
{
  for (int64_t i = (int64_t)blockIdx.x * 256 + threadIdx.x; i < lv.first[lv.count]; i += (int64_t)gridDim.x * 256) {
    int l = 0;
#pragma unroll
    for (int k = 1; k < PD_RESIZE_MAX; ++k) l += (k < lv.count && i >= lv.first[k]) ? 1 : 0;
    const int h = lv.h[l], w = lv.w[l];
    int64_t t = i - lv.first[l];
    const int c = (int)(t % C4); t /= C4;
    const int ox = (int)(t % w); t /= w;
    const int oy = (int)(t % h);
    const int b = (int)(t / h);
    int y0, yp, x0, xp; float hy0, hy1, wx0, wx1;
    up_src(oy, (float)H / (float)h, H, y0, yp, hy0, hy1);
    up_src(ox, (float)W / (float)w, W, x0, xp, wx0, wx1);
    const float4 *L = reinterpret_cast<const float4 *>(x) + (int64_t)b * H * W * C4;
    const float4 a = L[((int64_t)y0 * W + x0) * C4 + c], bq = L[((int64_t)y0 * W + x0 + xp) * C4 + c];
    const float4 cq = L[((int64_t)(y0 + yp) * W + x0) * C4 + c], d = L[((int64_t)(y0 + yp) * W + x0 + xp) * C4 + c];
    float4 o;
    o.x = hy0 * (wx0 * a.x + wx1 * bq.x) + hy1 * (wx0 * cq.x + wx1 * d.x);
    o.y = hy0 * (wx0 * a.y + wx1 * bq.y) + hy1 * (wx0 * cq.y + wx1 * d.y);
    o.z = hy0 * (wx0 * a.z + wx1 * bq.z) + hy1 * (wx0 * cq.z + wx1 * d.z);
    o.w = hy0 * (wx0 * a.w + wx1 * bq.w) + hy1 * (wx0 * cq.w + wx1 * d.w);
    const int64_t oi = (((int64_t)b * h + oy) * w + ox) * C4 + c;
    if (BF16) st4(reinterpret_cast<bf16_t *>(lv.out[l]) + oi * 4, o);
    else st4(reinterpret_cast<float *>(lv.out[l]) + oi * 4, o);
  }
}

__global__ __launch_bounds__(256) void upsample2x_bwd_nhwc(const float *__restrict__ dy, float *__restrict__ dlo, int B, int h,
                                                           int w, int C4)
{
  const int H = 2 * h, W = 2 * w;
  const int64_t total = (int64_t)B * h * w * C4;
  for (int64_t i = (int64_t)blockIdx.x * blockDim.x + threadIdx.x; i < total; i += (int64_t)gridDim.x * blockDim.x) {
// ... 351 lines not shown
    return pd_set_error(PD_ERR_INVALID_ARG, "pd_msda_prep_bwd: row strides %d / %d (>= row length, multiples of 4)", ld_offs, ld_logits);
  if (tokens < 0 || M <= 0 || L <= 0 || P <= 0) return pd_set_error(PD_ERR_INVALID_ARG, "pd_msda_prep_bwd: tokens=%lld M=%d L=%d P=%d", (long long)tokens, M, L, P);
  if (tokens == 0) return PD_OK;
  if (!gloc || !gattn || !attn || !spatial_shapes || !d_offs || !d_logits) return pd_set_error(PD_ERR_INVALID_ARG, "pd_msda_prep_bwd: null pointer");
  const int64_t total = tokens * M;
  const dim3 g((unsigned)((total + 255) / 256)), b(256);
  hipStream_t s = (hipStream_t)stream_;
  const int LP = L * P;
#define LAUNCH(KER) hipLaunchKernelGGL(KER, g, b, 0, s, gloc, gattn, attn, spatial_shapes, d_offs, d_logits, total, M, L, P, ld_offs, ld_logits, row_amax)
  if ((P & 1) == 0 && LP == 12) LAUNCH(msda_prep_bwd_v<3>);
  else if ((P & 1) == 0 && LP == 16) LAUNCH(msda_prep_bwd_v<4>);
  else if ((P & 1) == 0 && LP == 8) LAUNCH(msda_prep_bwd_v<2>);
  else hipLaunchKernelGGL(msda_prep_bwd, g, b, 0, s, gloc, gattn, attn, spatial_shapes, d_offs, d_logits, total, M, L, P, ld_offs, ld_logits);
#undef LAUNCH
  return pd_check_launch("pd_msda_prep_bwd");
}

extern "C" int pd_msda_prep_bwd(const float *gloc, const float *gattn, const float *attn, const int64_t *spatial_shapes, float *d_offs,
                                float *d_logits, int64_t tokens, int M, int L, int P, int ld_offs, int ld_logits, void *stream_)
{
  return msda_prep_bwd_launch(gloc, gattn, attn, spatial_shapes, d_offs, d_logits, tokens, M, L, P, ld_offs, ld_logits, stream_, nullptr);
}

extern "C" int pd_msda_prep_bwd_amax(const float *gloc, const float *gattn, const float *attn, const int64_t *spatial_shapes, float *d_offs,
                                     float *d_logits, float *row_amax, int64_t tokens, int M, int L, int P, int ld_offs, int ld_logits, void *stream_)
{
  return msda_prep_bwd_launch(gloc, gattn, attn, spatial_shapes, d_offs, d_logits, tokens, M, L, P, ld_offs, ld_logits, stream_, row_amax);
}

extern "C" int pd_point_sample_nhwc_f32(const float *in, const float *coords, float *out, int B, int H, int W, int C, int P,
                                        void *stream_)
{
  if (B < 0 || H <= 0 || W <= 0 || C <= 0 || (C & 3) || P < 0) return pd_set_error(PD_ERR_INVALID_ARG, "pd_point_sample_nhwc_f32: B=%d H=%d W=%d C=%d P=%d", B, H, W, C, P);
  if (B == 0 || P == 0) return PD_OK;
  if (!in || !coords || !out) return pd_set_error(PD_ERR_INVALID_ARG, "pd_point_sample_nhwc_f32: null pointer");
  const int64_t total = (int64_t)B * P;
  const unsigned grid = (unsigned)((total + 3) / 4 < 16384 ? (total + 3) / 4 : 16384);
  hipLaunchKernelGGL(point_sample_nhwc<float>, dim3(grid), dim3(256), 0, (hipStream_t)stream_, in, coords, out, B, H, W, C, P);
  return pd_check_launch("pd_point_sample_nhwc_f32");
}

extern "C" int pd_point_sample_nhwc_f32_bf16(const float *in, const float *coords, void *out, int B, int H, int W, int C, int P,
                                             void *stream_)
{
  if (B < 0 || H <= 0 || W <= 0 || C <= 0 || (C & 3) || P < 0) return pd_set_error(PD_ERR_INVALID_ARG, "pd_point_sample_nhwc_f32_bf16: B=%d H=%d W=%d C=%d P=%d", B, H, W, C, P);
  if (B == 0 || P == 0) return PD_OK;
  if (!in || !coords || !out) return pd_set_error(PD_ERR_INVALID_ARG, "pd_point_sample_nhwc_f32_bf16: null pointer");
  const int64_t total = (int64_t)B * P;
  const unsigned grid = (unsigned)((total + 3) / 4 < 16384 ? (total + 3) / 4 : 16384);
  hipLaunchKernelGGL(point_sample_nhwc<bf16_t>, dim3(grid), dim3(256), 0, (hipStream_t)stream_, in, coords, (bf16_t *)out, B, H, W, C, P);
  return pd_check_launch("pd_point_sample_nhwc_f32_bf16");
}

static int upsample_add_launch(const float *lo, int64_t lo_bs, const float *cur, float *y, int B, int h, int w, int H, int W, int C, void *stream_, float *amax)
{
  if (lo_bs == 0) lo_bs = (int64_t)h * w * C;
  if (lo_bs < (int64_t)h * w * C || (lo_bs & 3)) return pd_set_error(PD_ERR_INVALID_ARG, "pd_upsample_add_nhwc_f32: lo_batch_stride %lld (>= h w C, a multiple of 4)", (long long)lo_bs);
  if (amax && C != 256) return pd_set_error(PD_ERR_INVALID_ARG, "pd_upsample_add_amax_nhwc_f32: pixel maxima need C == 256");
  if (B < 0 || h <= 0 || w <= 0 || H <= 0 || W <= 0 || C <= 0 || (C & 3)) return pd_set_error(PD_ERR_INVALID_ARG, "pd_upsample_add_nhwc_f32: bad sizes");
  if (B == 0) return PD_OK;
  if (!lo || !cur || !y) return pd_set_error(PD_ERR_INVALID_ARG, "pd_upsample_add_nhwc_f32: null pointer");
  const int64_t total = (int64_t)B * H * W * (C / 4);
  const unsigned grid = (unsigned)((total + 255) / 256 < 32768 ? (total + 255) / 256 : 32768);
  hipLaunchKernelGGL(upsample_add_nhwc, dim3(grid), dim3(256), 0, (hipStream_t)stream_, lo, cur, y, B, h, w, H, W, C / 4,
                     (float)h / (float)H, (float)w / (float)W, amax, lo_bs / 4);
  return pd_check_launch("pd_upsample_add_nhwc_f32");
}

extern "C" int pd_upsample_add_nhwc_f32(const float *lo, int64_t lo_batch_stride, const float *cur, float *y, int B, int h, int w, int H, int W, int C,
                                        void *stream_)
{
  return upsample_add_launch(lo, lo_batch_stride, cur, y, B, h, w, H, W, C, stream_, nullptr);
}

extern "C" int pd_upsample_add_amax_nhwc_f32(const float *lo, int64_t lo_batch_stride, const float *cur, float *y, float *amax, int B, int h, int w, int H,
                                             int W, int C, void *stream_)
{
  return upsample_add_launch(lo, lo_batch_stride, cur, y, B, h, w, H, W, C, stream_, amax);
}

extern "C" int pd_upsample2x_bwd_nhwc_f32(const float *dy, float *dlo, int B, int h, int w, int C, void *stream_)
{
  if (B < 0 || h <= 0 || w <= 0 || C <= 0 || (C & 3)) return pd_set_error(PD_ERR_INVALID_ARG, "pd_upsample2x_bwd_nhwc_f32: bad sizes");
  if (B == 0) return PD_OK;
  if (!dy || !dlo) return pd_set_error(PD_ERR_INVALID_ARG, "pd_upsample2x_bwd_nhwc_f32: null pointer");
  const int64_t total = (int64_t)B * h * w * (C / 4);
  const unsigned grid = (unsigned)((total + 255) / 256 < 32768 ? (total + 255) / 256 : 32768);
  hipLaunchKernelGGL(upsample2x_bwd_nhwc, dim3(grid), dim3(256), 0, (hipStream_t)stream_, dy, dlo, B, h, w, C / 4);
  return pd_check_launch("pd_upsample2x_bwd_nhwc_f32");
}

extern "C" int pd_point_sample_planar_f32(const float *in, const float *coords, float *out, int N, int C, int H, int W, int P, void *stream_)
{
  if (N < 0 || C <= 0 || H <= 0 || W <= 0 || P < 0) return pd_set_error(PD_ERR_INVALID_ARG, "pd_point_sample_planar_f32: N=%d C=%d H=%d W=%d P=%d", N, C, H, W, P);
  if ((int64_t)N * P == 0) return PD_OK;
  if (!in || !coords || !out) return pd_set_error(PD_ERR_INVALID_ARG, "pd_point_sample_planar_f32: null pointer");
  const int tx = (W + PST - 1) / PST, ty = (H + PST - 1) / PST;
  if (C == 1 && tx * ty <= 1 && N <= 65535) {
    hipLaunchKernelGGL(point_sample_tiled_fwd, dim3(tx * ty, N), dim3(256), (PST + 1) * (PST + 1) * sizeof(float), (hipStream_t)stream_, in,
                       coords, out, H, W, P, tx);
    return pd_check_launch("pd_point_sample_planar_f32");
  }
  const int64_t blocks = ((int64_t)N * P + 255) / 256;
  hipLaunchKernelGGL(point_sample_planar_fwd, dim3((unsigned)(blocks > 65536 ? 65536 : blocks)), dim3(256), 0, (hipStream_t)stream_, in, coords, out,
                     N, C, H, W, P);
  return pd_check_launch("pd_point_sample_planar_f32");
}

extern "C" int pd_point_sample_planar_bwd_f32(const float *grad_out, const float *coords, float *grad_in, int N, int C, int H, int W, int P,
                                              void *stream_)
{
  if (N < 0 || C <= 0 || H <= 0 || W <= 0 || P < 0) return pd_set_error(PD_ERR_INVALID_ARG, "pd_point_sample_planar_bwd_f32: N=%d C=%d H=%d W=%d P=%d", N, C, H, W, P);
  if ((int64_t)N * P == 0) return PD_OK;
  if (!grad_out || !coords || !grad_in) return pd_set_error(PD_ERR_INVALID_ARG, "pd_point_sample_planar_bwd_f32: null pointer");
  const int tx = (W + PST - 1) / PST, ty = (H + PST - 1) / PST;
  if (C == 1 && tx * ty <= 16 && N <= 65535) {
    hipLaunchKernelGGL(point_sample_tiled_bwd, dim3(tx * ty, N), dim3(256), PST * PST * sizeof(float), (hipStream_t)stream_, grad_out, coords,
                       grad_in, H, W, P, tx);
    return pd_check_launch("pd_point_sample_planar_bwd_f32");
// ... 210 lines not shown
```

### partdistillation_amd/functions/conv_x3.py

```python
import torch
from torch.autograd import Function

from .. import lib as _lib


H2 = __import__("os").environ.get("PD_H2_CONV", "1") != "0"
H2_1X1 = __import__("os").environ.get("PD_H2_1X1", "1") != "0"
WGRAD_X3 = True


def supported(x, conv):
    return (x.is_cuda and x.dtype == torch.float32 and x.dim() == 4 and conv.weight.dtype == torch.float32
            and tuple(conv.kernel_size) == (3, 3) and tuple(conv.stride) == (1, 1) and tuple(conv.padding) == (1, 1)
            and tuple(conv.dilation) == (1, 1) and conv.groups == 1 and x.shape[1] % 16 == 0 and conv.weight.shape[0] % 16 == 0
            and x.is_contiguous(memory_format=torch.channels_last))


def _pixel_amax(x):
    from . import amax_cache
    from .gemm import row_amax
    am = amax_cache.get(x)
    return am if am is not None else row_amax(x.permute(0, 2, 3, 1).reshape(-1, x.shape[1]))


# ... 16 lines not shown
class Conv3x3X3(Function):
    @staticmethod
    def forward(ctx, x, weight, bias):
        if not x.is_cuda:
            raise RuntimeError("pd_conv3x3_nhwc_f32x3 runs on the GPU only (no CPU fallback in partdistillation_amd)")
        x = x.contiguous(memory_format=torch.channels_last)
        wk = weight.permute(0, 2, 3, 1).contiguous()
        x_am = _pixel_amax(x) if H2 else None
        ctx.save_for_backward(x, weight, x_am)
        ctx.has_bias = bias is not None
        return _raw(x, wk, bias, weight.shape[0], x_am)

    @staticmethod
    def backward(ctx, dy):
        x, weight, x_am = ctx.saved_tensors
        dy = dy.contiguous(memory_format=torch.channels_last)
        co, ci = weight.shape[0], weight.shape[1]
        dx = dw = db = None
        dy_am = _pixel_amax(dy) if x_am is not None else None
        if ctx.needs_input_grad[0]:
            wt = weight.permute(0, 2, 3, 1).reshape(co, 9, ci).flip(1).permute(2, 1, 0).contiguous()
            dx = _raw(dy, wt, None, ci, dy_am)
        want_w, want_b = ctx.needs_input_grad[1], ctx.has_bias and ctx.needs_input_grad[2]
        if (want_w or want_b) and WGRAD_X3 and ci % 128 == 0 and co % 4 == 0:
            from .gemm import _wgrad_workspace
            L = _lib.load()
            B, _, H, W = x.shape
            buf = torch.zeros(co * 9 * ci + co, dtype=torch.float32, device=x.device)
            dwk, dbv = buf[:co * 9 * ci].view(co, 3, 3, ci), buf[co * 9 * ci:]
            ws = _wgrad_workspace(x.device, int((L.pd_gemm_wgrad_f16x2_ws_floats if x_am is not None else L.pd_gemm_wgrad_f32x3_ws_floats)(co, 9 * ci)))
            if x_am is not None:
                _lib.check(L.pd_conv3x3_wgrad_nhwc_f16x2(dy.data_ptr(), x.data_ptr(), dwk.data_ptr(), dbv.data_ptr() if want_b else None,
                                                         dy_am.data_ptr(), x_am.data_ptr(), ws.data_ptr() if ws is not None else None,
                                                         ws.numel() if ws is not None else 0, B, H, W, ci, co, _lib.current_stream()))
            else:
                _lib.check(L.pd_conv3x3_wgrad_nhwc_f32x3(dy.data_ptr(), x.data_ptr(), dwk.data_ptr(), dbv.data_ptr() if want_b else None,
                                                         ws.data_ptr() if ws is not None else None, ws.numel() if ws is not None else 0,
                                                         B, H, W, ci, co, _lib.current_stream()))
            dw = dwk.permute(0, 3, 1, 2) if want_w else None
            db = dbv if want_b else None
        elif want_w or want_b:
            _, dw, db = torch.ops.aten.convolution_backward(dy, x, weight, [co] if ctx.has_bias else None, [1, 1], [1, 1], [1, 1], False,
                                                            [0, 0], 1, [False, True, ctx.has_bias])
        return dx, dw, db


def conv3x3(x, weight, bias=None):
    return Conv3x3X3.apply(x, weight, bias)


class Conv1x1OwnWgrad(Function):

    @staticmethod
    def forward(ctx, x, weight, bias):
        ctx.has_bias = bias is not None
        ctx.x_bf16 = x.dtype == torch.bfloat16
        if H2 and H2_1X1 and x.is_contiguous(memory_format=torch.channels_last):
            from .gemm import cast_rows_amax, gemm_tn_h2, row_amax
            B, ci, Hh, Ww = x.shape
            co = weight.shape[0]
            if ctx.x_bf16:
                x2, x_am = cast_rows_amax(x.permute(0, 2, 3, 1).reshape(-1, ci))
                x = x2.view(B, Hh, Ww, ci).permute(0, 3, 1, 2)
            else:
                x_am = _pixel_amax(x)
            w2 = weight.reshape(co, ci)
            y = gemm_tn_h2(x.permute(0, 2, 3, 1).reshape(-1, ci), w2, bias, a_amax=x_am, b_amax=row_amax(w2))
            ctx.save_for_backward(x, weight, x_am)
            return y.view(B, Hh, Ww, co).permute(0, 3, 1, 2)
        if ctx.x_bf16:
            x = x.float()
        ctx.save_for_backward(x, weight, None)
        return torch.ops.aten.convolution(x, weight, bias, [1, 1], [0, 0], [1, 1], False, [0, 0], 1)

    @staticmethod
    def backward(ctx, dy):
        from .gemm import gemm_tn_h2, gemm_tn_h2_bf16out, gemm_wgrad_acc, row_amax
        x, weight, x_am = ctx.saved_tensors
        dy = dy.contiguous(memory_format=torch.channels_last)
        co, ci = weight.shape[0], weight.shape[1]
        dx = dw = db = None
        rows = lambda t: t.permute(0, 2, 3, 1).reshape(-1, t.shape[1])
        h2 = x_am is not None
        dy_am = _pixel_amax(dy) if h2 else None
        if ctx.needs_input_grad[0]:
            if h2:
                wt = weight.reshape(co, ci).t().contiguous()
                B, _, Hh, Ww = x.shape
                mm = gemm_tn_h2_bf16out if ctx.x_bf16 else gemm_tn_h2
                dx = mm(rows(dy), wt, None, a_amax=dy_am, b_amax=row_amax(wt)).view(B, Hh, Ww, ci).permute(0, 3, 1, 2)
            else:
                dx = torch.ops.aten.convolution_backward(dy, x, weight, None, [1, 1], [0, 0], [1, 1], False, [0, 0], 1, [True, False, False])[0]
                dx = dx.to(torch.bfloat16) if ctx.x_bf16 else dx
        want_w, want_b = ctx.needs_input_grad[1], ctx.has_bias and ctx.needs_input_grad[2]
        if want_w or want_b:
            buf = torch.zeros(co * ci + co, dtype=torch.float32, device=x.device)
            dw2, dbv = buf[:co * ci].view(co, ci), buf[co * ci:]
            if h2:
                gemm_wgrad_acc(rows(dy), rows(x), dw2, dbv if want_b else None, h2=True, y_amax=dy_am, x_amax=x_am)
            else:
                gemm_wgrad_acc(rows(dy), rows(x), dw2, dbv if want_b else None, x3=True)
            dw = dw2.view(co, ci, 1, 1).as_strided(weight.shape, weight.stride()) if want_w else None
            db = dbv if want_b else None
        return dx, dw, db


def conv1x1_supported(x, conv):
    return (WGRAD_X3 and x.is_cuda and (x.dtype == torch.float32 or (x.dtype == torch.bfloat16 and H2 and H2_1X1 and x.shape[1] % 8 == 0))
            and x.dim() == 4 and conv.weight.dtype == torch.float32
            and tuple(conv.kernel_size) == (1, 1) and tuple(conv.stride) == (1, 1) and tuple(conv.padding) == (0, 0)
            and tuple(conv.dilation) == (1, 1) and conv.groups == 1 and x.shape[1] % 4 == 0 and conv.weight.shape[0] % 4 == 0
            and x.is_contiguous(memory_format=torch.channels_last) and torch.is_grad_enabled())


def conv1x1(x, weight, bias=None):
    return Conv1x1OwnWgrad.apply(x, weight, bias)
```

### partdistillation_amd/functions/fused.py

```python
import numpy as np
import torch
from torch.autograd import Function

from . import amax_cache

from .. import lib as _lib


def _stream():
    return _lib.current_stream()


def _nhwc(t):
    return t if t.is_contiguous(memory_format=torch.channels_last) else t.contiguous(memory_format=torch.channels_last)


class MaxPool3x3S2(Function):

    @staticmethod
    def forward(ctx, x):
        x = _nhwc(x)
        B, C, H, W = x.shape
        OH, OW = (H - 1) // 2 + 1, (W - 1) // 2 + 1
        y = torch.empty((B, C, OH, OW), dtype=x.dtype, device=x.device, memory_format=torch.channels_last)
        arg = torch.empty(B * OH * OW * C, dtype=torch.uint8, device=x.device)
        _lib.check(_lib.load().pd_maxpool3s2_fwd_bf16(x.data_ptr(), y.data_ptr(), arg.data_ptr(), B, H, W, C, _stream()))
        ctx.save_for_backward(arg)
        ctx.dims = (B, C, H, W)
        return y

    @staticmethod
    def backward(ctx, gy):
        (arg,) = ctx.saved_tensors
        B, C, H, W = ctx.dims
        gy = _nhwc(gy)
        gx = torch.empty((B, C, H, W), dtype=gy.dtype, device=gy.device, memory_format=torch.channels_last)
        _lib.check(_lib.load().pd_maxpool3s2_bwd_bf16(gy.data_ptr(), arg.data_ptr(), gx.data_ptr(), B, H, W, C, _stream()))
        return gx


def max_pool3x3s2_supported(x):
    return x.is_cuda and x.dtype == torch.bfloat16 and x.dim() == 4 and x.shape[1] % 8 == 0 and x.is_contiguous(memory_format=torch.channels_last)


def max_pool3x3s2(x):
    return MaxPool3x3S2.apply(x)


class AffineAct(Function):

    @staticmethod
    def forward(ctx, x, scale, bias, residual, relu):
# ... 184 lines not shown
        bt, bs, bd, bl, first = [], [], [], [], []
        for t, (n, off) in enumerate(zip(numels, dst_offsets)):
            first.append(len(bt))
            for s in range(0, max(n, 1), self.CHUNK):
                bt.append(t), bs.append(s), bd.append(off + s), bl.append(min(self.CHUNK, n - s))
        first.append(len(bt))
        self.first_block = first
        self.nblocks, self.ntensors = len(bt), len(numels)
        self.blk_tensor = torch.tensor(bt, dtype=torch.int32, device=device)
        self.blk_start = torch.tensor(bs, dtype=torch.int64, device=device)
        self.blk_dst = torch.tensor(bd, dtype=torch.int64, device=device)
        self.blk_len = torch.tensor(bl, dtype=torch.int32, device=device)
        pin = device.type == "cuda"
        self._host_ptrs = PinnedRing(self.ntensors, torch.int64, pin)
        self._host_bf16 = PinnedRing(self.ntensors, torch.int32, pin)
        self.src_ptrs = torch.zeros(self.ntensors, dtype=torch.int64, device=device)
        self.src_bf16 = torch.zeros(self.ntensors, dtype=torch.int32, device=device)
        self._last = None

    def upload(self, grads, t_begin=0):
        tp, tb = self._host_ptrs.acquire(), self._host_bf16.acquire()
        hp, hb = tp.numpy(), tb.numpy()
        for i, g in enumerate(grads, start=t_begin):
            if g is None:
                hp[i], hb[i] = 0, 0
            else:
                hp[i], hb[i] = g.data_ptr(), 1 if g.dtype == torch.bfloat16 else 0
        t_end = t_begin + len(grads)
        last = self._last
        capturing = self.src_ptrs.is_cuda and torch.cuda.is_current_stream_capturing()
        if last is not None and not capturing and (last[0][t_begin:t_end] == hp[t_begin:t_end]).all() and (last[1][t_begin:t_end] == hb[t_begin:t_end]).all():
            self._host_ptrs.release(), self._host_bf16.release()
            return
        if last is None:
            last = self._last = (hp.copy(), hb.copy())
            last[0][:] = -1
        last[0][t_begin:t_end] = hp[t_begin:t_end]
        last[1][t_begin:t_end] = hb[t_begin:t_end]
        self.src_ptrs[t_begin:t_end].copy_(tp[t_begin:t_end], non_blocking=True)
        self.src_bf16[t_begin:t_end].copy_(tb[t_begin:t_end], non_blocking=True)
        self._host_ptrs.release(), self._host_bf16.release()

    def gather(self, dst, sumsq=None, t_begin=0, t_end=None):
        t_end = self.ntensors if t_end is None else t_end
        b0, b1 = self.first_block[t_begin], self.first_block[t_end]
        with torch.cuda.device(dst.device):
            rc = _lib.load().pd_multi_gather_sumsq(self.src_ptrs.data_ptr(), self.src_bf16.data_ptr(), self.blk_tensor.data_ptr(),
                                                   self.blk_start.data_ptr(), self.blk_dst.data_ptr(), self.blk_len.data_ptr(),
                                                   dst.data_ptr(), sumsq.data_ptr() if sumsq is not None else None, b0, b1,
                                                   _stream())
        _lib.check(rc)


class GroupNormNHWC(Function):

    @staticmethod
    def forward(ctx, x, weight, bias, groups, eps, relu):
        N, C, H, W = x.shape
        P = H * W
        lib = _lib.load()
        st = _stream()
        sums = torch.empty((N, C, 2), dtype=torch.float64, device=x.device)
        coef = torch.empty((5, N, C), dtype=torch.float32, device=x.device)
        _lib.check(lib.pd_nc_sums_f32(x.data_ptr(), None, None, None, None, sums.data_ptr(), N, P, C, 0, 0, st))
        _lib.check(lib.pd_gn_coeffs_fwd(sums.data_ptr(), weight.data_ptr(), bias.data_ptr(), N, C, groups, P, float(eps),
                                        coef[0].data_ptr(), coef[1].data_ptr(), coef[2].data_ptr(), coef[3].data_ptr(),
                                        coef[4].data_ptr(), st))
        y = torch.empty_like(x, memory_format=torch.channels_last)
        if C == 256:
            am = torch.empty(N * P, dtype=torch.float32, device=x.device)
            _lib.check(lib.pd_nc_affine_amax_f32(x.data_ptr(), coef[0].data_ptr(), coef[1].data_ptr(), y.data_ptr(), am.data_ptr(), N, P, C, int(relu), st))
            ctx.y_am = am
        else:
            _lib.check(lib.pd_nc_affine_f32(x.data_ptr(), coef[0].data_ptr(), coef[1].data_ptr(), y.data_ptr(), N, P, C, int(relu), st))
            ctx.y_am = None
        ctx.save_for_backward(x, y if relu else None, weight, coef)
        ctx.groups, ctx.relu = groups, relu
        return y

    @staticmethod
    def backward(ctx, gy):
        x, y, weight, coef = ctx.saved_tensors
        N, C, H, W = x.shape
        P, G = H * W, ctx.groups
        gy = _nhwc(gy)
        lib = _lib.load()
        st = _stream()
        mean_c, rstd_c, xb = coef[2], coef[3], coef[4]
        sums = torch.empty((N, C, 2), dtype=torch.float64, device=x.device)
        _lib.check(lib.pd_nc_sums_f32(x.data_ptr(), gy.data_ptr(), y.data_ptr() if y is not None else None, rstd_c.data_ptr(),
                                      xb.data_ptr(), sums.data_ptr(), N, P, C, 1, int(ctx.relu), st))
        out = torch.empty((3 * N * C + 2 * C,), dtype=torch.float32, device=x.device)
        a, pc, rc = out[:N * C], out[N * C:2 * N * C], out[2 * N * C:3 * N * C]
        gw, gb = out[3 * N * C:3 * N * C + C], out[3 * N * C + C:]
        _lib.check(lib.pd_gn_coeffs_bwd(sums.data_ptr(), weight.data_ptr(), mean_c.data_ptr(), rstd_c.data_ptr(), N, C, G, P,
                                        a.data_ptr(), pc.data_ptr(), rc.data_ptr(), gw.data_ptr(), gb.data_ptr(), st))
        dx = torch.empty_like(x, memory_format=torch.channels_last)
        if C == 256:
            am = torch.empty(N * P, dtype=torch.float32, device=x.device)
            _lib.check(lib.pd_nc_affine2_amax_f32(gy.data_ptr(), x.data_ptr(), y.data_ptr() if y is not None else None, a.data_ptr(),
                                                  pc.data_ptr(), rc.data_ptr(), dx.data_ptr(), am.data_ptr(), N, P, C, int(ctx.relu), st))
            amax_cache.put(dx, am)
        else:
            _lib.check(lib.pd_nc_affine2_f32(gy.data_ptr(), x.data_ptr(), y.data_ptr() if y is not None else None, a.data_ptr(),
                                             pc.data_ptr(), rc.data_ptr(), dx.data_ptr(), N, P, C, int(ctx.relu), st))
        return dx, gw, gb, None, None, None


def group_norm_nhwc_supported(x, groups):
    C = x.shape[1] if x.dim() == 4 else 0
    return (x.is_cuda and x.dtype == torch.float32 and x.dim() == 4 and C % 4 == 0 and C <= 256 and 256 % (C // 4) == 0
            and C % groups == 0 and not torch.is_autocast_enabled())


def group_norm_nhwc(x, weight, bias, groups=32, eps=1e-5, relu=False):
    if not group_norm_nhwc_supported(x, groups):
        raise RuntimeError("pd group norm: fp32 CUDA NCHW-shaped tensor with C = 4*2^k <= 256 required (no fallback here)")
    y = GroupNormNHWC.apply(_nhwc(x), weight, bias, groups, eps, relu)
    am = getattr(y.grad_fn, "y_am", None) if y.grad_fn is not None else None
    if am is not None:
        amax_cache.put(y, am)
    return y
```

### partdistillation_amd/functions/gemm.py

```python
import ctypes

import torch
from torch.autograd import Function

from .. import lib as _lib


def _stream():
    return _lib.current_stream()


def gemm_tn(a, b, bias=None, relu=False):
    if not a.is_cuda:
        raise RuntimeError("pd_gemm_tn_f32 runs on the GPU only (no CPU fallback in partdistillation_amd)")
    assert a.dtype == torch.float32 and b.dtype == torch.float32 and a.stride(1) == 1 and b.stride(1) == 1
    M, K = a.shape
    N = b.shape[0]
    c = torch.empty((M, N), dtype=torch.float32, device=a.device)
    with torch.cuda.device(a.device):
        rc = _lib.load().pd_gemm_tn_f32(a.data_ptr(), b.data_ptr(), bias.data_ptr() if bias is not None else None,
                                        c.data_ptr(), M, N, K, a.stride(0), b.stride(0), N, int(relu), _stream())
    _lib.check(rc)
    return c

# ... 39 lines not shown

def cast_rows_amax(x):
    assert x.is_cuda and x.dtype == torch.bfloat16 and x.dim() == 2 and x.is_contiguous() and x.shape[1] % 8 == 0
    y = torch.empty(x.shape, dtype=torch.float32, device=x.device)
    am = torch.empty(x.shape[0], dtype=torch.float32, device=x.device)
    _lib.check(_lib.load().pd_cast_bf16_f32_amax(x.data_ptr(), x.shape[0], x.shape[1], y.data_ptr(), am.data_ptr(), _stream()))
    return y, am


def gemm_tn_h2_bf16out(a, b, bias=None, a_amax=None, b_amax=None):
    if not a.is_cuda:
        raise RuntimeError("pd_gemm_tn_f16x2_bf16out runs on the GPU only (no CPU fallback in partdistillation_amd)")
    assert a.dtype == torch.float32 and b.dtype == torch.float32 and a.stride(1) == 1 and b.stride(1) == 1 and b.shape[1] == a.shape[1]
    M, K = a.shape
    N = b.shape[0]
    c = torch.empty((M, N), dtype=torch.bfloat16, device=a.device)
    p = lambda t: t.data_ptr() if t is not None else None
    _lib.check(_lib.load().pd_gemm_tn_f16x2_bf16out(a.data_ptr(), b.data_ptr(), p(bias), c.data_ptr(), p(a_amax), p(b_amax), M, N, K, a.stride(0),
                                                    b.stride(0), N, _stream()))
    return c


def h2_bits_supported(M, N):
    return N % 256 == 0 and M >= 1024


def gemm_tn_h2(a, b, bias=None, mode=0, bits=None, colsum=None, a_amax=None, b_amax=None, c_amax=None, want_bits=False):
    if not a.is_cuda:
        raise RuntimeError("pd_gemm_tn_f16x2 runs on the GPU only (no CPU fallback in partdistillation_amd)")
    assert a.dtype == torch.float32 and b.dtype == torch.float32 and a.stride(1) == 1 and b.stride(1) == 1
    M, K = a.shape
    N = b.shape[0]
    assert b.shape[1] == K
    for v, n in ((a_amax, M), (b_amax, N), (c_amax, M)):
        assert v is None or (v.dtype == torch.float32 and v.is_contiguous() and v.numel() == n)
    L = _lib.load()
    c = torch.empty((M, N), dtype=torch.float32, device=a.device)
    if mode == 1 and want_bits:
        bits = torch.empty(int(L.pd_gemm_tn_f16x2_bits_words(M, N)), dtype=torch.int32, device=a.device)
    p = lambda t: t.data_ptr() if t is not None else None
    args = (a.data_ptr(), b.data_ptr(), p(bias), c.data_ptr(), p(bits), p(colsum), p(a_amax), p(b_amax), p(c_amax), M, N, K, a.stride(0), b.stride(0), N, mode,
            _stream())
    if not _TIMING["on"]:
        _lib.check(L.pd_gemm_tn_f16x2(*args))
        return (c, bits) if (mode == 1 and want_bits) else c
    which = int(L.pd_gemm_tn_f16x2_which(M, N, K, a.stride(0), b.stride(0), mode, int(bits is not None), int(a_amax is not None),
                                         int(b_amax is not None), int(c_amax is not None), 0))
    label = (f"gemm_rows_f16x2_k256<true, {mode}>" if which == 2 else f"gemm_ra_f16x2_k256<{mode}>" if which == 3
             else "gemm_kres_f16x2<true, 0>" if which == 4 else "gemm_kpc_f16x2<true, 0, false, false>" if which == 5
             else f"gemm_tn_f16x2<{'256, 256, 128, 16' if which == 1 else '128, 128, 64, 16'}, {mode}>")
    with _timed_fwd(2.0 * M * N * K, label, 4.0 * (M * K + N * K + M * N)):
        _lib.check(L.pd_gemm_tn_f16x2(*args))
    return (c, bits) if (mode == 1 and want_bits) else c


def split3(w, transpose=False):
    assert w.is_cuda and w.dtype == torch.float32 and w.dim() == 2 and w.stride(1) == 1
    N, K = w.shape
    out = torch.empty((3, K, N) if transpose else (3, N, K), dtype=torch.bfloat16, device=w.device)
    _lib.check(_lib.load().pd_split3_bf16(w.data_ptr(), N, K, w.stride(0), int(transpose), out.data_ptr(), _stream()))
    return out


def pre_supported(M, N, K):
    return N % 256 == 0 and K % 16 == 0 and M >= 1024 and (-(-M // 256)) * (N // 256) >= 128


def gemm_tn_x3_pre(a, planes, bias=None, mode=0, bits=None, colsum=None, want_bits=False):
    assert a.is_cuda and a.dtype == torch.float32 and a.stride(1) == 1 and planes.dtype == torch.bfloat16 and planes.is_contiguous()
    M, K = a.shape
    N = planes.shape[1]
    assert planes.shape[2] == K
    L = _lib.load()
    c = torch.empty((M, N), dtype=torch.float32, device=a.device)
    if mode == 1 and want_bits:
        bits = torch.empty(int(L.pd_gemm_tn_f32x3_relu_bits_words(M, N)), dtype=torch.int32, device=a.device)
    _lib.check(L.pd_gemm_tn_f32x3_pre(a.data_ptr(), planes.data_ptr(), bias.data_ptr() if bias is not None else None, c.data_ptr(),
                                      bits.data_ptr() if bits is not None else None, colsum.data_ptr() if colsum is not None else None,
                                      M, N, K, a.stride(0), N, mode, _stream()))
    return (c, bits) if (mode == 1 and want_bits) else c


def relu_bits_supported(M, N):
    return N % 256 == 0 and M >= 1024


def gemm_tn_x3_relu_bits(a, b, bias):
    assert a.is_cuda and a.dtype == torch.float32 and b.dtype == torch.float32 and a.stride(1) == 1 and b.stride(1) == 1
    M, K = a.shape
    N = b.shape[0]
    L = _lib.load()
    c = torch.empty((M, N), dtype=torch.float32, device=a.device)
    bits = torch.empty(int(L.pd_gemm_tn_f32x3_relu_bits_words(M, N)), dtype=torch.int32, device=a.device)
    with _timed_fwd(2.0 * M * N * K, "gemm_tn_f32x3_wide<relu + sign bits>"):
        _lib.check(L.pd_gemm_tn_f32x3_relu_bits(a.data_ptr(), b.data_ptr(), bias.data_ptr() if bias is not None else None, c.data_ptr(),
                                                bits.data_ptr(), M, N, K, a.stride(0), b.stride(0), N, _stream()))
    return c, bits


def gemm_tn_x3_relumask(a, b, bits, colsum):
    assert a.is_cuda and a.dtype == torch.float32 and b.dtype == torch.float32 and a.stride(1) == 1 and b.stride(1) == 1
    M, K = a.shape
    N = b.shape[0]
    assert bits.dtype == torch.int32 and colsum.dtype == torch.float32 and colsum.numel() == N
    c = torch.empty((M, N), dtype=torch.float32, device=a.device)
    with _timed_fwd(2.0 * M * N * K, "gemm_tn_f32x3_wide<relu mask + column sums>"):
# ... 207 lines not shown
```

### partdistillation_amd/lib.py

```python
import ctypes
import os
import subprocess

_HERE = os.path.dirname(os.path.abspath(__file__))
LIB_PATH = os.environ.get("PD_LIB_PATH") or os.path.join(_HERE, "libpd_hip.so")
CSRC = os.path.join(_HERE, "csrc")

PD_F32, PD_F64, PD_BF16 = 0, 1, 2
ABI_VERSION = 49

_c_int, _c_vp = ctypes.c_int, ctypes.c_void_p

SIGNATURES = {
    "pd_msda_forward": (_c_int, [_c_vp] * 6 + [_c_int] * 9 + [_c_vp]),
    "pd_msda_backward": (_c_int, [_c_vp] * 9 + [_c_int] * 9 + [_c_vp]),
    "pd_msda_backward_last_gate": (_c_int, [_c_vp]),
    "pd_stem7x7_fwd": (_c_int, [_c_vp, _c_int] + [_c_vp] * 4 + [_c_int] * 4 + [_c_vp]),
    "pd_stem_wgrad_workspace_floats": (ctypes.c_int64, []),
    "pd_stem7x7_wgrad": (_c_int, [_c_vp, _c_int] + [_c_vp] * 4 + [_c_int, _c_vp] + [_c_int] * 4 + [_c_vp]),
    "pd_msda_fused_supported": (_c_int, [_c_int] * 7),
    "pd_msda_fused_forward": (_c_int, [_c_vp] * 4 + [_c_int] + [_c_vp] * 4 + [_c_int] * 7 + [_c_vp]),
    "pd_msda_fused_backward": (_c_int, [_c_vp] * 4 + [_c_int] + [_c_vp] * 6 + [_c_int, _c_vp, _c_vp] + [_c_int] * 7 + [_c_vp]),
    "pd_lsa_batched": (_c_int, [_c_vp] * 4 + [_c_int] * 3 + [_c_vp]),
    "pd_sumsq_accumulate": (_c_int, [_c_vp, ctypes.c_int64, _c_int, _c_vp, _c_vp]),
    "pd_adamw_clipped": (_c_int, [_c_vp] * 4 + [ctypes.c_int64, _c_int] + [ctypes.c_double] * 5 + [_c_int, _c_vp, ctypes.c_double, _c_vp, _c_vp]),
    "pd_gemm_tn_f32": (_c_int, [_c_vp] * 4 + [_c_int] * 7 + [_c_vp]),
    "pd_gemm_tn_f32x3": (_c_int, [_c_vp] * 4 + [_c_int] * 7 + [_c_vp]),
    "pd_gemm_wgrad_f16x2_takes_wide_tiles": (_c_int, [_c_int] * 2),
    "pd_gemm_wgrad_f16x2_ws_floats": (ctypes.c_int64, [_c_int] * 2),
    "pd_gemm_wgrad_f16x2_grouped_ws_floats": (ctypes.c_int64, [_c_vp, _c_int]),
    "pd_gemm_wgrad_acc_f16x2_ws": (_c_int, [_c_vp] * 7 + [ctypes.c_int64] + [_c_int] * 6 + [_c_vp]),
    "pd_gemm_wgrad_f16x2_grouped": (_c_int, [_c_vp, _c_int, _c_vp, _c_vp, _c_vp, ctypes.c_int64, _c_vp]),
    "pd_conv3x3_wgrad_nhwc_f16x2": (_c_int, [_c_vp] * 7 + [ctypes.c_int64] + [_c_int] * 5 + [_c_vp]),
    "pd_conv3x3_nhwc_f16x2": (_c_int, [_c_vp] * 7 + [_c_int] * 5 + [_c_vp]),
    "pd_gemm_tn_f16x2_which": (_c_int, [_c_int] * 11),
    "pd_gemm_tn_f16x2_bits_words": (ctypes.c_int64, [_c_int] * 2),
    "pd_gemm_tn_f16x2": (_c_int, [_c_vp] * 9 + [_c_int] * 7 + [_c_vp]),
    "pd_gemm_tn_f16x2_bf16out": (_c_int, [_c_vp] * 6 + [_c_int] * 6 + [_c_vp]),
    "pd_cast_bf16_f32_amax": (_c_int, [_c_vp, _c_int, _c_int, _c_vp, _c_vp, _c_vp]),
    "pd_row_amax_f32": (_c_int, [_c_vp, _c_int, _c_int, _c_int, _c_vp, _c_vp]),
    "pd_gemm_tn_f32x3_relumask": (_c_int, [_c_vp] * 5 + [_c_int] * 6 + [_c_vp]),
    "pd_gemm_tn_f32x3_relu_bits": (_c_int, [_c_vp] * 5 + [_c_int] * 6 + [_c_vp]),
    "pd_gemm_tn_f32x3_relu_bits_words": (ctypes.c_int64, [_c_int] * 2),
    "pd_split3_bf16": (_c_int, [_c_vp, _c_int, _c_int, _c_int, _c_int, _c_vp, _c_vp]),
    "pd_gemm_tn_f32x3_pre": (_c_int, [_c_vp] * 6 + [_c_int] * 6 + [_c_vp]),
    "pd_gemm_wgrad_f32": (_c_int, [_c_vp] * 4 + [_c_int] * 6 + [_c_vp]),
    "pd_gemm_wgrad_acc_f32": (_c_int, [_c_vp] * 4 + [_c_int] * 6 + [_c_vp]),
    "pd_conv3x3_nhwc_f32x3": (_c_int, [_c_vp] * 4 + [_c_int] * 5 + [_c_vp]),
    "pd_gemm_wgrad_acc_f32x3": (_c_int, [_c_vp] * 4 + [_c_int] * 6 + [_c_vp]),
    "pd_conv3x3_wgrad_nhwc_f32x3": (_c_int, [_c_vp] * 5 + [ctypes.c_int64] + [_c_int] * 5 + [_c_vp]),
    "pd_gemm_wgrad_f32x3_ws_floats": (ctypes.c_int64, [_c_int] * 2),
    "pd_gemm_wgrad_f32x3_grouped_table_bytes": (ctypes.c_int64, [_c_int]),
    "pd_gemm_wgrad_f32x3_grouped_ws_floats": (ctypes.c_int64, [_c_vp, _c_int]),
    "pd_gemm_wgrad_f32x3_grouped": (_c_int, [_c_vp, _c_int, _c_vp, _c_vp, _c_vp, ctypes.c_int64, _c_vp]),
    "pd_gemm_wgrad_acc_f32x3_ws": (_c_int, [_c_vp] * 5 + [ctypes.c_int64] + [_c_int] * 6 + [_c_vp]),
    "pd_adamw_clipped_shadow": (_c_int, [_c_vp] * 5 + [ctypes.c_int64] + [ctypes.c_double] * 5 + [_c_int, _c_vp, ctypes.c_double, _c_vp, _c_vp]),
    "pd_conv_bf16_supported": (_c_int, [_c_int] * 5),
    "pd_conv_bf16_fwd": (_c_int, [_c_vp] * 6 + [_c_int] * 11 + [_c_vp]),
    "pd_conv_bf16_wgrad_workspace_floats": (ctypes.c_int64, [_c_int] * 6),
    "pd_conv_bf16_wgrad": (_c_int, [_c_vp] * 4 + [ctypes.c_int64] + [_c_int] * 10 + [_c_vp]),
    "pd_conv_bf16_wgrad_grouped_table_bytes": (ctypes.c_int64, [_c_int]),
    "pd_conv_bf16_wgrad_grouped_workspace_floats": (ctypes.c_int64, [_c_vp, _c_int]),
    "pd_conv_bf16_wgrad_grouped": (_c_int, [_c_vp, _c_int, _c_vp, _c_vp, _c_vp, ctypes.c_int64, _c_vp]),
    "pd_conv_bf16_dgrad": (_c_int, [_c_vp] * 4 + [_c_int] * 10 + [_c_vp]),
    "pd_maxpool3s2_fwd_bf16": (_c_int, [_c_vp] * 3 + [_c_int] * 4 + [_c_vp]),
    "pd_maxpool3s2_bwd_bf16": (_c_int, [_c_vp] * 3 + [_c_int] * 4 + [_c_vp]),
    "pd_affine_act_fwd_bf16": (_c_int, [_c_vp] * 5 + [ctypes.c_int64, _c_int, _c_int, _c_vp]),
    "pd_affine_act_bwd_bf16": (_c_int, [_c_vp] * 5 + [ctypes.c_int64, _c_int, _c_int, _c_vp]),
    "pd_affine_act_bwd2_bf16": (_c_int, [_c_vp] * 6 + [ctypes.c_int64, _c_int, _c_int, _c_vp]),
    "pd_multi_gather_sumsq": (_c_int, [_c_vp] * 8 + [_c_int, _c_int, _c_vp]),
    "pd_attn_workspace_floats": (ctypes.c_int64, [_c_int] * 4),
    "pd_attn_fwd_d32": (_c_int, [_c_vp] * 7 + [_c_int] * 4 + [ctypes.c_float, _c_int, _c_vp]),
    "pd_attn_bwd_d32": (_c_int, [_c_vp] * 11 + [_c_int] * 4 + [ctypes.c_float, _c_int, _c_vp]),
    "pd_attn_fwd_d32_ld": (_c_int, [_c_vp] * 7 + [_c_int] * 4 + [ctypes.c_float, _c_int, _c_int, _c_vp]),
    "pd_attn_bwd_d32_ld": (_c_int, [_c_vp] * 11 + [_c_int] * 4 + [ctypes.c_float, _c_int, _c_int, _c_vp]),
    "pd_nc_sums_f32": (_c_int, [_c_vp] * 6 + [_c_int] * 5 + [_c_vp]),
    "pd_nc_affine_f32": (_c_int, [_c_vp] * 4 + [_c_int] * 4 + [_c_vp]),
    "pd_nc_affine_amax_f32": (_c_int, [_c_vp] * 5 + [_c_int] * 4 + [_c_vp]),
    "pd_nc_affine2_amax_f32": (_c_int, [_c_vp] * 8 + [_c_int] * 4 + [_c_vp]),
    "pd_upsample_add_amax_nhwc_f32": (_c_int, [_c_vp, ctypes.c_int64] + [_c_vp] * 3 + [_c_int] * 6 + [_c_vp]),
    "pd_nc_affine2_f32": (_c_int, [_c_vp] * 7 + [_c_int] * 4 + [_c_vp]),
    "pd_add_layernorm_fwd": (_c_int, [_c_vp, _c_int, _c_vp, _c_vp, _c_vp, ctypes.c_float, _c_vp, _c_vp, _c_vp, _c_vp, _c_int, _c_vp,
                                      _c_int, _c_vp, _c_vp, _c_int, _c_int, _c_vp]),
    "pd_add_layernorm_bwd": (_c_int, [_c_vp] * 4 + [_c_int] + [_c_vp] * 6 + [_c_int] + [_c_vp] * 4 + [_c_int] * 3 + [_c_vp]),
    "pd_add_layernorm_fwd_amax": (_c_int, [_c_vp, _c_int, _c_vp, _c_vp, _c_vp, ctypes.c_float, _c_vp, _c_vp, _c_vp, _c_vp, _c_int, _c_vp,
                                           _c_int, _c_vp, _c_vp, _c_vp, _c_vp, _c_int, _c_int, _c_vp]),
    "pd_add_layernorm_bwd_amax": (_c_int, [_c_vp] * 4 + [_c_int] + [_c_vp] * 6 + [_c_int] + [_c_vp] * 4 + [_c_int] + [_c_vp] + [_c_int] * 2 + [_c_vp]),
    "pd_colsum_acc": (_c_int, [_c_vp, _c_int, _c_int, _c_int, _c_vp, _c_vp]),
    "pd_relu_bwd_colsum": (_c_int, [_c_vp, _c_vp, _c_int, _c_int, _c_int, _c_vp, _c_vp]),
    "pd_mem_prep_fwd": (_c_int, [_c_vp, ctypes.c_int64, _c_vp, _c_vp, _c_vp, _c_vp, _c_int, _c_int, _c_int, _c_int, _c_vp]),
    "pd_mem_prep_bwd": (_c_int, [_c_vp, _c_vp, _c_int, _c_vp, ctypes.c_int64, _c_int, _c_int, _c_int, _c_vp]),
    "pd_attn_mask_u8": (_c_int, [_c_vp, _c_int, _c_int, _c_int, _c_vp, _c_vp]),
    "pd_add_rows_amax_f32": (_c_int, [_c_vp] * 6 + [_c_int, _c_int, _c_vp]),
    "pd_sum3_sum2_f32": (_c_int, [_c_vp] * 6 + [ctypes.c_int64, _c_vp]),
    "pd_transpose_batched_f32": (_c_int, [_c_vp, _c_int, _c_vp]),
    "pd_normalize_u8_nhwc": (_c_int, [_c_vp, _c_int, _c_int, _c_int, _c_vp, _c_vp, _c_vp, _c_vp]),
    "pd_resize_bilinear_nhwc_f32": (_c_int, [_c_vp] + [_c_int] * 4 + [_c_vp] * 3 + [_c_int, _c_int, _c_vp]),
    "pd_matcher_point_terms": (_c_int, [_c_vp, _c_int, _c_int, _c_int, _c_vp, _c_vp, _c_vp, _c_vp, _c_vp]),
    "pd_match_point_logits": (_c_int, [_c_vp] * 4 + [_c_int] * 7 + [_c_vp]),
    "pd_matcher_costs": (_c_int, [_c_vp, _c_int, _c_vp] + [ctypes.c_int64] * 3 + [_c_vp] * 3 + [_c_int] * 6 + [ctypes.c_float] * 3 + [_c_vp]),
    "pd_mask_point_losses_fwd": (_c_int, [_c_vp] * 5 + [_c_int, _c_int, _c_vp]),
    "pd_mask_point_losses_bwd": (_c_int, [_c_vp] * 6 + [_c_int, _c_int, _c_vp]),
    "pd_uncertain_points": (_c_int, [_c_vp] * 4 + [_c_int] * 4 + [_c_vp]),
    "pd_point_sample_u8": (_c_int, [_c_vp] * 4 + [_c_int] * 5 + [_c_vp]),
    "pd_skinny_linear_fwd": (_c_int, [_c_vp] * 3 + [_c_int, _c_vp] + [_c_int] * 3 + [_c_vp]),
    "pd_skinny_linear_partial_floats": (ctypes.c_int64, [_c_int] * 3),
    "pd_skinny_linear_bwd": (_c_int, [_c_vp, _c_vp, _c_int, _c_vp, _c_vp, _c_vp, _c_int, _c_vp, _c_vp, _c_vp] + [_c_int] * 4 + [_c_vp]),
    "pd_loss_vectors_fwd": (_c_int, [_c_vp, ctypes.c_int64, ctypes.c_int64] + [_c_vp] * 9 + [_c_int] * 5 + [_c_vp]),
    "pd_loss_vectors_bwd": (_c_int, [_c_vp, ctypes.c_int64, ctypes.c_int64] + [_c_vp] * 10 + [_c_int] * 5 + [_c_vp]),
    "pd_pair_logits_fwd": (_c_int, [_c_vp] * 5 + [_c_int] * 4 + [_c_vp]),
    "pd_pair_logits_bwd_tok": (_c_int, [_c_vp] * 5 + [_c_int] * 4 + [_c_vp]),
    "pd_pair_logits_workspace_floats": (ctypes.c_int64, [_c_int] * 3),
    "pd_pair_logits_bwd_rows": (_c_int, [_c_vp] * 6 + [_c_int] * 4 + [_c_vp]),
    "pd_msda_prep_fwd": (_c_int, [_c_vp] * 6 + [ctypes.c_int64] + [_c_int] * 5 + [_c_vp]),
    "pd_msda_prep_bwd_amax": (_c_int, [_c_vp] * 7 + [ctypes.c_int64] + [_c_int] * 5 + [_c_vp]),
    "pd_msda_forward_amax": (_c_int, [_c_vp] * 7 + [_c_int] * 9 + [_c_vp]),
    "pd_msda_prep_bwd": (_c_int, [_c_vp] * 6 + [ctypes.c_int64] + [_c_int] * 5 + [_c_vp]),
    "pd_sgemm_tn_batched_bf16": (_c_int, [_c_vp] * 3 + [_c_int] * 7 + [ctypes.c_int64] * 3 + [_c_vp]),
    "pd_sgemm_tn_multi_bf16": (_c_int, [_c_vp, _c_int, _c_int, _c_vp]),
    "pd_decoder_head_bf16": (_c_int, [_c_vp] * 3 + [ctypes.c_float] + [_c_vp] * 10 + [_c_int] * 4 + [_c_vp]),
    "pd_dec_fwd_a": (_c_int, [_c_vp] * 3 + [_c_int] + [_c_vp] * 4 + [ctypes.c_float] + [_c_vp] * 10 + [_c_int] + [_c_vp]),
    "pd_dec_fwd_b": (_c_int, [_c_vp] * 3 + [_c_int] + [_c_vp] * 20 + [ctypes.c_float] + [_c_vp] * 13 + [_c_int] * 2 + [_c_vp]),
    "pd_dec_bwd_b": (_c_int, [_c_vp] * 14 + [_c_int] + [_c_vp] * 15 + [_c_int] + [_c_vp]),
    "pd_dec_split": (_c_int, []),
    "pd_dec_workspace_bytes": (ctypes.c_int64, [_c_int]),
    "pd_dec_pack_table_bytes": (ctypes.c_int64, [_c_int]),
    "pd_dec_pack_grouped": (_c_int, [_c_vp, _c_int, _c_vp, _c_vp, _c_vp]),
    "pd_dec_bwd_a": (_c_int, [_c_vp] * 11 + [_c_int] + [_c_vp] * 4 + [_c_int] + [_c_vp]),
    "pd_sgemm_split_workspace_floats": (ctypes.c_int64, [_c_int] * 3),
# ... 160 lines not shown
```

### partdistillation_amd/modeling/pixel_decoder/msdeformattn.py

```python
from typing import Callable, Dict, List, Optional, Union

import numpy as np
import torch
import torch.nn.functional as F
from torch import nn
from torch.nn.init import normal_

from ...compat import SEM_SEG_HEADS_REGISTRY, ShapeSpec, configurable
from ...compat.layers import Conv2d, c2_xavier_fill, get_norm
from ..transformer_decoder.position_encoding import PositionEmbeddingSine
from ...functions import conv_x3
from ...functions.fused import group_norm_nhwc, group_norm_nhwc_supported
from ...functions.gemm import linear_f32
from .ops.modules import MSDeformAttn
from ...functions.encoder_core import EncoderCore, EncoderSpec
from ...functions.rowwise import supports_width, upsample_add, upsample_add_supported


class MSDeformAttnTransformerEncoderLayer(nn.Module):
    def __init__(self, d_model=256, d_ffn=1024, dropout=0.1, activation="relu", n_levels=4, n_heads=8, n_points=4):
        super().__init__()
        assert activation == "relu"
        self.self_attn = MSDeformAttn(d_model, n_levels, n_heads, n_points)
        self.dropout1 = nn.Dropout(dropout)
        self.norm1 = nn.LayerNorm(d_model)
        self.linear1 = nn.Linear(d_model, d_ffn)
        self.dropout2 = nn.Dropout(dropout)
        self.linear2 = nn.Linear(d_ffn, d_model)
        self.dropout3 = nn.Dropout(dropout)
        self.norm2 = nn.LayerNorm(d_model)

    def forward(self, src, pos, reference_points, spatial_shapes, level_start_index, padding_mask=None):
        q = src if pos is None else src + pos
        attn = self.self_attn(q, reference_points, src, spatial_shapes, level_start_index, padding_mask)
        src = self.norm1(src + self.dropout1(attn))
        lin = MSDeformAttn._linear
        if self.dropout2.p == 0.0 and src.dtype == torch.float32 and src.is_cuda and not torch.is_autocast_enabled():
            hidden = linear_f32(src, self.linear1.weight, self.linear1.bias, True)
        else:
            hidden = self.dropout2(F.relu(self.linear1(src)))
        ffn = lin(self.linear2, hidden)
        return self.norm2(src + self.dropout3(ffn))


class MSDeformAttnTransformerEncoder(nn.Module):
    def __init__(self, encoder_layer_factory, num_layers):
        super().__init__()
        self.layers = nn.ModuleList([encoder_layer_factory() for _ in range(num_layers)])
        self.num_layers = num_layers
        self._ref_cache = {}

    @staticmethod
    def get_reference_points(spatial_shapes, valid_ratios, device):
        refs = []
        for lvl, (H_, W_) in enumerate(spatial_shapes):
            H_, W_ = int(H_), int(W_)
            ry, rx = torch.meshgrid(torch.linspace(0.5, H_ - 0.5, H_, dtype=torch.float32, device=device),
                                    torch.linspace(0.5, W_ - 0.5, W_, dtype=torch.float32, device=device), indexing="ij")
            ry = ry.reshape(-1)[None] / (valid_ratios[:, None, lvl, 1] * H_)
            rx = rx.reshape(-1)[None] / (valid_ratios[:, None, lvl, 0] * W_)
            refs.append(torch.stack((rx, ry), -1))
        ref = torch.cat(refs, 1)
        return ref[:, :, None] * valid_ratios[:, None]

    def forward(self, src, spatial_shapes, level_start_index, valid_ratios, pos=None, padding_mask=None,
# ... 100 lines not shown


class MSDeformAttnTransformerEncoderOnly(nn.Module):
    def __init__(self, d_model=256, nhead=8, num_encoder_layers=6, dim_feedforward=1024, dropout=0.1,
                 activation="relu", num_feature_levels=4, enc_n_points=4):
        super().__init__()
        self.d_model, self.nhead = d_model, nhead
        self.encoder = MSDeformAttnTransformerEncoder(
            lambda: MSDeformAttnTransformerEncoderLayer(d_model, dim_feedforward, dropout, activation,
                                                        num_feature_levels, nhead, enc_n_points), num_encoder_layers)
        self.level_embed = nn.Parameter(torch.Tensor(num_feature_levels, d_model))
        self._shape_cache = {}
        self._reset_parameters()

    def _reset_parameters(self):
        for p in self.parameters():
            if p.dim() > 1:
                nn.init.xavier_uniform_(p)
        for m in self.modules():
            if isinstance(m, MSDeformAttn):
                m._reset_parameters()
        normal_(self.level_embed)

    def forward(self, srcs, pos_embeds):
        shapes_host = [(int(s.shape[2]), int(s.shape[3])) for s in srcs]
        key = (tuple(shapes_host), str(srcs[0].device))
        if key not in self._shape_cache:
            sh = torch.as_tensor(shapes_host, dtype=torch.long, device=srcs[0].device)
            self._shape_cache[key] = (sh, torch.cat((sh.new_zeros((1,)), sh.prod(1).cumsum(0)[:-1])))
        spatial_shapes, level_start_index = self._shape_cache[key]
        if srcs[0].is_cuda:
            src = CatLevels.apply(*srcs)
        else:
            src = torch.cat([s.flatten(2).transpose(1, 2) for s in srcs], 1)
        if src.is_cuda and src.dtype == torch.float32 and self.level_embed.dtype == torch.float32 and self.d_model % 128 == 0:
            pos = LevelPos.apply(self.level_embed, *pos_embeds)
        else:
            pos = torch.cat([p.flatten(2).transpose(1, 2) + self.level_embed[i].view(1, 1, -1)
                             for i, p in enumerate(pos_embeds)], 1)
        valid_ratios = src.new_ones((src.shape[0], len(srcs), 2))
        memory = self.encoder(src, spatial_shapes, level_start_index, valid_ratios, pos, None, shapes_host=shapes_host)
        return memory, spatial_shapes, level_start_index, shapes_host


CONV_X3 = bool(int(__import__("os").environ.get("PD_CONV_X3", "1")))


def _as_fp32_input(x, conv):
    if x.dtype == torch.bfloat16 and CONV_X3 and conv_x3.conv1x1_supported(x, conv) and x.requires_grad:
        return x
    return x.float()


def _conv_gn(conv, gn, x, relu=False):
    if CONV_X3 and conv_x3.supported(x, conv):
        y = conv_x3.conv3x3(x, conv.weight, conv.bias)
    elif CONV_X3 and conv_x3.conv1x1_supported(x, conv):
        y = conv_x3.conv1x1(x, conv.weight, conv.bias)
    else:
        y = F.conv2d(x, conv.weight, conv.bias, conv.stride, conv.padding, conv.dilation, conv.groups)
    if isinstance(gn, nn.GroupNorm) and group_norm_nhwc_supported(y, gn.num_groups):
        return group_norm_nhwc(y, gn.weight, gn.bias, gn.num_groups, gn.eps, relu)
    if gn is not None:
        y = gn(y)
    return F.relu(y) if relu else y


@SEM_SEG_HEADS_REGISTRY.register()
class MSDeformAttnPixelDecoder(nn.Module):
    @configurable
    def __init__(self, input_shape: Dict[str, ShapeSpec], *, transformer_dropout: float, transformer_nheads: int,
                 transformer_dim_feedforward: int, transformer_enc_layers: int, conv_dim: int, mask_dim: int,
                 norm: Optional[Union[str, Callable]] = None, transformer_in_features: List[str], common_stride: int):
        super().__init__()
        tf_shape = {k: v for k, v in input_shape.items() if k in transformer_in_features}
        by_stride = sorted(input_shape.items(), key=lambda kv: kv[1].stride)
        self.in_features = [k for k, _ in by_stride]
        self.feature_strides = [v.stride for _, v in by_stride]
        self.feature_channels = [v.channels for _, v in by_stride]
        tf_by_stride = sorted(tf_shape.items(), key=lambda kv: kv[1].stride)
        self.transformer_in_features = [k for k, _ in tf_by_stride]
        tf_channels = [v.channels for _, v in tf_by_stride]
        self.transformer_feature_strides = [v.stride for _, v in tf_by_stride]
        self.transformer_num_feature_levels = len(self.transformer_in_features)
        chans = tf_channels[::-1] if self.transformer_num_feature_levels > 1 else [tf_channels[-1]]
        self.input_proj = nn.ModuleList(
            [nn.Sequential(nn.Conv2d(c, conv_dim, kernel_size=1), nn.GroupNorm(32, conv_dim)) for c in chans])
        for proj in self.input_proj:
            nn.init.xavier_uniform_(proj[0].weight, gain=1)
            nn.init.constant_(proj[0].bias, 0)
        self.transformer = MSDeformAttnTransformerEncoderOnly(
            d_model=conv_dim, dropout=transformer_dropout, nhead=transformer_nheads,
            dim_feedforward=transformer_dim_feedforward, num_encoder_layers=transformer_enc_layers,
            num_feature_levels=self.transformer_num_feature_levels)
        self.pe_layer = PositionEmbeddingSine(conv_dim // 2, normalize=True)
        self.mask_dim = mask_dim
        self.mask_features = Conv2d(conv_dim, mask_dim, kernel_size=1, stride=1, padding=0)
        c2_xavier_fill(self.mask_features)
        self.maskformer_num_feature_levels = 3
        self.common_stride = common_stride
        self.num_fpn_levels = int(np.log2(min(self.transformer_feature_strides)) - np.log2(self.common_stride))
        lateral_convs, output_convs = [], []
        use_bias = norm == ""
        for idx, in_channels in enumerate(self.feature_channels[: self.num_fpn_levels]):
            lateral = Conv2d(in_channels, conv_dim, kernel_size=1, bias=use_bias, norm=get_norm(norm, conv_dim))
            output = Conv2d(conv_dim, conv_dim, kernel_size=3, stride=1, padding=1, bias=use_bias,
                            norm=get_norm(norm, conv_dim), activation=F.relu)
            c2_xavier_fill(lateral)
            c2_xavier_fill(output)
            self.add_module(f"adapter_{idx + 1}", lateral)
            self.add_module(f"layer_{idx + 1}", output)
            lateral_convs.append(lateral)
            output_convs.append(output)
        self.lateral_convs = lateral_convs[::-1]
        self.output_convs = output_convs[::-1]

    @classmethod
    def from_config(cls, cfg, input_shape: Dict[str, ShapeSpec]):
        head = cfg.MODEL.SEM_SEG_HEAD
        return dict(
            input_shape={k: v for k, v in input_shape.items() if k in head.IN_FEATURES},
            conv_dim=head.CONVS_DIM, mask_dim=head.MASK_DIM, norm=head.NORM,
            transformer_dropout=cfg.MODEL.MASK_FORMER.DROPOUT, transformer_nheads=cfg.MODEL.MASK_FORMER.NHEADS,
            transformer_dim_feedforward=1024,
            transformer_enc_layers=head.TRANSFORMER_ENC_LAYERS,
            transformer_in_features=head.DEFORMABLE_TRANSFORMER_ENCODER_IN_FEATURES,
            common_stride=head.COMMON_STRIDE)

    def forward_features(self, features):
        with torch.autocast(device_type=next(iter(features.values())).device.type, enabled=False):
            srcs, pos = [], []
            for idx, f in enumerate(self.transformer_in_features[::-1]):
                x = _as_fp32_input(features[f], self.input_proj[idx][0])
                srcs.append(_conv_gn(self.input_proj[idx][0], self.input_proj[idx][1], x))
                pos.append(self.pe_layer(x))
            y, spatial_shapes, level_start_index, shapes_host = self.transformer(srcs, pos)
            bs = y.shape[0]
            sizes = [h * w for h, w in shapes_host]
            out = [z.transpose(1, 2).reshape(bs, -1, h, w) for z, (h, w) in zip(torch.split(y, sizes, dim=1), shapes_host)]
            for idx, f in enumerate(self.in_features[: self.num_fpn_levels][::-1]):
                x = _as_fp32_input(features[f], self.lateral_convs[idx])
                lat, outc = self.lateral_convs[idx], self.output_convs[idx]
                cur = _conv_gn(lat, lat.norm, x, relu=lat.activation is not None)
                if upsample_add_supported(out[-1], cur):
                    y = upsample_add(out[-1], cur)
                else:
                    y = cur + F.interpolate(out[-1], size=cur.shape[-2:], mode="bilinear", align_corners=False)
                out.append(_conv_gn(outc, outc.norm, y, relu=outc.activation is not None))
            multi_scale = out[: self.maskformer_num_feature_levels]
            mf = self.mask_features
            if CONV_X3 and mf.norm is None and mf.activation is None and conv_x3.conv1x1_supported(out[-1], mf):
                return conv_x3.conv1x1(out[-1], mf.weight, mf.bias), out[0], multi_scale
            return mf(out[-1]), out[0], multi_scale
```

Measured before the change: 108.6.

## Fuse GroupNorm stats into split-K conv1x1 and GN into upsample-add in pixel decoder

Adds a split-K f16x2 GEMM for small-tile conv1x1 projections whose reduce step also accumulates per-channel GroupNorm sums, so GN can skip a separate statistics pass. It fuses the lateral GroupNorm affine into the upsample-add kernel and recomputes ReLU masks from x and the forward coefficients in backward instead of reading y. A pooled buffer for GN sums avoids per-call allocation and memset. This reduces memory passes and raises occupancy on low-tile GEMMs, at the cost of split-K workspace traffic and more code paths.

```diff
diff --git a/include/pd_fused.h b/include/pd_fused.h
--- a/include/pd_fused.h
+++ b/include/pd_fused.h
@@ -30,6 +30,10 @@
                            float *amax, int N, int P, int C, int relu, void *stream);
 int pd_nc_affine2_f32(const float *dy, const float *x, const float *y, const float *a, const float *p, const float *r, float *dx,
                       int N, int P, int C, int relu, void *stream);
+int pd_nc_sums_acc_f32(const float *x, const float *dy, const float *y, const float *a, const float *b, const float *fa, const float *fb,
+                       double *out, int N, int P, int C, int mode, int relu, void *stream);
+int pd_nc_affine2_xmask_f32(const float *dy, const float *x, const float *fa, const float *fb, const float *a, const float *p, const float *r,
+                            float *dx, float *amax, int N, int P, int C, void *stream);
 
 int pd_gn_coeffs_fwd(const double *sums, const float *weight, const float *bias, int N, int C, int G, int P, float eps, float *a,
                      float *b, float *mean_c, float *rstd_c, float *xb, void *stream);
diff --git a/include/pd_gemm.h b/include/pd_gemm.h
--- a/include/pd_gemm.h
+++ b/include/pd_gemm.h
@@ -69,6 +69,11 @@
 int pd_gemm_tn_f16x2(const float *A, const float *B, const float *bias, float *C, uint32_t *bits, float *colsum, const float *a_amax,
                      const float *b_amax, float *c_amax, int M, int N, int K, int lda, int ldb, int ldc, int mode, void *stream);
 int pd_row_amax_f32(const float *X, int rows, int cols, int ld, float *out, void *stream);
+int pd_gemm_tn_f16x2_splitk_slices(int M, int N, int K);
+int pd_gemm_tn_f16x2_splitk_slices_cu(int M, int N, int K, int cu);
+int pd_gemm_tn_f16x2_splitk(const float *A, const float *B, const float *bias, float *C, const float *a_amax, const float *b_amax, float *workspace,
+                            int64_t workspace_floats, double *sums, int rows_per_image, int M, int N, int K, int lda, int ldb, int ldc, int S,
+                            void *stream);
 int pd_gemm_tn_f16x2_bf16out(const float *A, const float *B, const float *bias, void *C_bf16, const float *a_amax, const float *b_amax, int M, int N,
                              int K, int lda, int ldb, int ldc, void *stream);
 int pd_cast_bf16_f32_amax(const void *X_bf16, int rows, int cols, float *Y, float *row_amax, void *stream);
diff --git a/include/pd_rowwise.h b/include/pd_rowwise.h
--- a/include/pd_rowwise.h
+++ b/include/pd_rowwise.h
@@ -58,6 +58,8 @@
 int pd_upsample_add_nhwc_f32(const float *lo, int64_t lo_batch_stride, const float *cur, float *y, int B, int h, int w, int H, int W, int C, void *stream);
 int pd_upsample_add_amax_nhwc_f32(const float *lo, int64_t lo_batch_stride, const float *cur, float *y, float *amax, int B, int h, int w, int H, int W, int C,
                                   void *stream);
+int pd_upsample_add_affine_nhwc_f32(const float *lo, int64_t lo_batch_stride, const float *x, const float *a, const float *b, float *y, float *amax, int B,
+                                    int h, int w, int H, int W, int C, void *stream);
 int pd_upsample2x_bwd_nhwc_f32(const float *dy, float *dlo, int B, int h, int w, int C, void *stream);
 
 #define PD_RESIZE_MAX 4
diff --git a/partdistillation_amd/csrc/cmdbuf.hip b/partdistillation_amd/csrc/cmdbuf.hip
--- a/partdistillation_amd/csrc/cmdbuf.hip
+++ b/partdistillation_amd/csrc/cmdbuf.hip
@@ -87,6 +87,7 @@
   PD_E(pd_filter_transpose_grouped),
   PD_E(pd_gemm_tn_f16x2),
   PD_E(pd_gemm_tn_f16x2_bf16out),
+  PD_E(pd_gemm_tn_f16x2_splitk),
   PD_E(pd_gemm_tn_f32),
   PD_E(pd_gemm_tn_f32x3),
   PD_E(pd_gemm_tn_f32x3_pre),
@@ -148,8 +149,10 @@
   PD_E(pd_mx8_quantize_grouped),
   PD_E(pd_nc_affine2_amax_f32),
   PD_E(pd_nc_affine2_f32),
+  PD_E(pd_nc_affine2_xmask_f32),
   PD_E(pd_nc_affine_amax_f32),
   PD_E(pd_nc_affine_f32),
+  PD_E(pd_nc_sums_acc_f32),
   PD_E(pd_nc_sums_f32),
   PD_E(pd_normalize_u8_nhwc),
   PD_E(pd_pair_logits_bwd_rows),
@@ -192,6 +195,7 @@
   PD_E(pd_transpose_batched_f32),
   PD_E(pd_uncertain_points),
   PD_E(pd_upsample2x_bwd_nhwc_f32),
+  PD_E(pd_upsample_add_affine_nhwc_f32),
   PD_E(pd_upsample_add_amax_nhwc_f32),
   PD_E(pd_upsample_add_nhwc_f32),
   PD_E(pd_wgrad_bf16),
diff --git a/partdistillation_amd/csrc/common.hip b/partdistillation_amd/csrc/common.hip
--- a/partdistillation_amd/csrc/common.hip
+++ b/partdistillation_amd/csrc/common.hip
@@ -27,7 +27,7 @@
 }
 
 extern "C" const char *pd_last_error(void) { return g_err; }
-extern "C" int pd_abi_version(void) { return 49; }
+extern "C" int pd_abi_version(void) { return 50; }
 
 extern int g_pd_dbg_atomic_scope;
 extern int g_pd_dbg_force_generic;
@@ -35,6 +35,7 @@
 extern int g_pd_dbg_x3_narrow;
 extern int g_pd_dbg_f16x2;
 extern int g_pd_dbg_wgrad_wide;
+extern int g_pd_dbg_splitk_tiles;
 extern "C" void pd_dbg_set_wgrad_xcd(int v);
 extern "C" void pd_dbg_set_wgrad_fast(int v);
 extern int g_pd_dbg_bwd_variant;
@@ -86,6 +87,7 @@
   if (!strcmp(key, "conv_xcd_major")) { g_pd_dbg_conv_xcd_major = value; return PD_OK; }
   if (!strcmp(key, "x3_ablate")) { g_pd_dbg_x3 = value; return PD_OK; }
   if (!strcmp(key, "f16x2_tile")) { g_pd_dbg_f16x2 = value; return PD_OK; }
+  if (!strcmp(key, "f16x2_splitk_tiles")) { g_pd_dbg_splitk_tiles = value; return PD_OK; }
   if (!strcmp(key, "wgrad_wide")) { g_pd_dbg_wgrad_wide = value; return PD_OK; }
   if (!strcmp(key, "wgrad_xcd")) { pd_dbg_set_wgrad_xcd(value); return PD_OK; }
   if (!strcmp(key, "wgrad_fast")) { pd_dbg_set_wgrad_fast(value); return PD_OK; }
diff --git a/partdistillation_amd/csrc/fused.hip b/partdistillation_amd/csrc/fused.hip
--- a/partdistillation_amd/csrc/fused.hip
+++ b/partdistillation_amd/csrc/fused.hip
@@ -210,14 +210,16 @@
 template <int MODE>
 __global__ __launch_bounds__(256) void nc_sums(const float *__restrict__ x, const float *__restrict__ dy, const float *__restrict__ y,
                                                 const float *__restrict__ a, const float *__restrict__ b, double *__restrict__ out,
-                                                int P, int C, int pix_per_block, int relu)
+                                                int P, int C, int pix_per_block, int relu, const float *__restrict__ fa,
+                                                const float *__restrict__ fb)
 {
   __shared__ float red[2][256][4];
   const int n = blockIdx.y, cq = C >> 2, q = threadIdx.x % cq, po = threadIdx.x / cq, pstride = 256 / cq;
   const int p0 = blockIdx.x * pix_per_block, p1 = min(P, p0 + pix_per_block);
   const int64_t base = (int64_t)n * P * C + q * 4;
-  float4 s0 = make_float4(0, 0, 0, 0), s1 = s0, av = s0, bv = s0;
-  if (MODE == 1) { av = *reinterpret_cast<const float4 *>(a + n * C + q * 4); bv = *reinterpret_cast<const float4 *>(b + n * C + q * 4); }
+  float4 s0 = make_float4(0, 0, 0, 0), s1 = s0, av = s0, bv = s0, fav = s0, fbv = s0;
+  if (MODE != 0) { av = *reinterpret_cast<const float4 *>(a + n * C + q * 4); bv = *reinterpret_cast<const float4 *>(b + n * C + q * 4); }
+  if (MODE == 2) { fav = *reinterpret_cast<const float4 *>(fa + n * C + q * 4); fbv = *reinterpret_cast<const float4 *>(fb + n * C + q * 4); }
 #pragma unroll 4
   for (int p = p0 + po; p < p1; p += pstride) {
     const float4 xv = *reinterpret_cast<const float4 *>(x + base + (int64_t)p * C);
@@ -226,7 +228,10 @@
       s1.x += xv.x * xv.x; s1.y += xv.y * xv.y; s1.z += xv.z * xv.z; s1.w += xv.w * xv.w;
     } else {
       float4 g = *reinterpret_cast<const float4 *>(dy + base + (int64_t)p * C);
-      if (relu) {
+      if (MODE == 2) {
+        const float4 yv = make_float4(xv.x * fav.x + fbv.x, xv.y * fav.y + fbv.y, xv.z * fav.z + fbv.z, xv.w * fav.w + fbv.w);
+        g.x = yv.x > 0 ? g.x : 0; g.y = yv.y > 0 ? g.y : 0; g.z = yv.z > 0 ? g.z : 0; g.w = yv.w > 0 ? g.w : 0;
+      } else if (relu) {
         const float4 yv = *reinterpret_cast<const float4 *>(y + base + (int64_t)p * C);
         g.x = yv.x > 0 ? g.x : 0; g.y = yv.y > 0 ? g.y : 0; g.z = yv.z > 0 ? g.z : 0; g.w = yv.w > 0 ? g.w : 0;
       }
@@ -272,10 +277,11 @@
   }
 }
 
-template <bool RELU>
+template <int RELU>
 __global__ __launch_bounds__(256) void nc_affine2(const float4 *__restrict__ dy, const float4 *__restrict__ x, const float4 *__restrict__ y,
                                                    const float *__restrict__ a, const float *__restrict__ pc, const float *__restrict__ rc,
-                                                   float4 *__restrict__ dx, int64_t n4, int P, int C, float *__restrict__ amax)
+                                                   float4 *__restrict__ dx, int64_t n4, int P, int C, float *__restrict__ amax,
+                                                   const float *__restrict__ fa, const float *__restrict__ fb)
 {
   const int cq = C >> 2;
   const int64_t stride = (int64_t)gridDim.x * blockDim.x, per_img = (int64_t)P * cq;
@@ -285,7 +291,11 @@
                  rv = *reinterpret_cast<const float4 *>(rc + n * C + q * 4);
     float4 g = dy[i];
     const float4 xv = x[i];
-    if (RELU) {
+    if (RELU == 2) {
+      const float4 fav = *reinterpret_cast<const float4 *>(fa + n * C + q * 4), fbv = *reinterpret_cast<const float4 *>(fb + n * C + q * 4);
+      const float4 yv = make_float4(xv.x * fav.x + fbv.x, xv.y * fav.y + fbv.y, xv.z * fav.z + fbv.z, xv.w * fav.w + fbv.w);
+      g.x = yv.x > 0 ? g.x : 0; g.y = yv.y > 0 ? g.y : 0; g.z = yv.z > 0 ? g.z : 0; g.w = yv.w > 0 ? g.w : 0;
+    } else if (RELU == 1) {
       const float4 yv = y[i];
       g.x = yv.x > 0 ? g.x : 0; g.y = yv.y > 0 ? g.y : 0; g.z = yv.z > 0 ? g.z : 0; g.w = yv.w > 0 ? g.w : 0;
     }
@@ -444,24 +454,39 @@
   return PD_OK;
 }
 
-extern "C" int pd_nc_sums_f32(const float *x, const float *dy, const float *y, const float *a, const float *b, double *out,
-                              int N, int P, int C, int mode, int relu, void *stream_)
+static int nc_sums_launch(const float *x, const float *dy, const float *y, const float *a, const float *b, const float *fa, const float *fb,
+                          double *out, int N, int P, int C, int mode, int relu, bool zero, void *stream_)
 {
   int rc = nc_check(N, P, C, "pd_nc_sums_f32");
   if (rc) return rc;
   if (!out) return pd_set_error(PD_ERR_INVALID_ARG, "pd_nc_sums_f32: null output");
   hipStream_t s = (hipStream_t)stream_;
-  (void)hipMemsetAsync(out, 0, (size_t)N * C * 2 * sizeof(double), s);
+  if (zero) (void)hipMemsetAsync(out, 0, (size_t)N * C * 2 * sizeof(double), s);
   if ((int64_t)N * P == 0) return pd_check_launch("pd_nc_sums_f32");
-  if (!x || (mode == 1 && (!dy || !a || !b || (relu && !y)))) return pd_set_error(PD_ERR_INVALID_ARG, "pd_nc_sums_f32: null input");
+  const bool xmask = mode == 1 && relu && fa && fb;
+  if (!x || (mode == 1 && (!dy || !a || !b || (relu && !y && !xmask)))) return pd_set_error(PD_ERR_INVALID_ARG, "pd_nc_sums_f32: null input");
   static const int ppb_env = []() { const char *e = getenv("PD_NC_PPB"); return e ? atoi(e) : 0; }();
   const int64_t np = (int64_t)N * P;
   int ppb = mode == 0 ? (np >= 131072 ? 512 : np >= 32768 ? 256 : np >= 8192 ? 128 : 64) : (np >= 131072 ? 256 : np >= 32768 ? 128 : 32);
   if (ppb_env > 0) ppb = ppb_env;
   dim3 grid((P + ppb - 1) / ppb, N);
-  if (mode == 0) hipLaunchKernelGGL(nc_sums<0>, grid, dim3(256), 0, s, x, dy, y, a, b, out, P, C, ppb, relu);
-  else hipLaunchKernelGGL(nc_sums<1>, grid, dim3(256), 0, s, x, dy, y, a, b, out, P, C, ppb, relu);
+  if (mode == 0) hipLaunchKernelGGL(nc_sums<0>, grid, dim3(256), 0, s, x, dy, y, a, b, out, P, C, ppb, relu, fa, fb);
+  else if (xmask) hipLaunchKernelGGL(nc_sums<2>, grid, dim3(256), 0, s, x, dy, y, a, b, out, P, C, ppb, relu, fa, fb);
+  else hipLaunchKernelGGL(nc_sums<1>, grid, dim3(256), 0, s, x, dy, y, a, b, out, P, C, ppb, relu, fa, fb);
   return pd_check_launch("pd_nc_sums_f32");
+}
+
+extern "C" int pd_nc_sums_f32(const float *x, const float *dy, const float *y, const float *a, const float *b, double *out,
+                              int N, int P, int C, int mode, int relu, void *stream_)
+{
+  return nc_sums_launch(x, dy, y, a, b, nullptr, nullptr, out, N, P, C, mode, relu, true, stream_);
+}
+
+extern "C" int pd_nc_sums_acc_f32(const float *x, const float *dy, const float *y, const float *a, const float *b, const float *fa,
+                                  const float *fb, double *out, int N, int P, int C, int mode, int relu, void *stream_)
+{
+  if ((fa == nullptr) != (fb == nullptr)) return pd_set_error(PD_ERR_INVALID_ARG, "pd_nc_sums_acc_f32: fa and fb come together");
+  return nc_sums_launch(x, dy, y, a, b, fa, fb, out, N, P, C, mode, relu, false, stream_);
 }
 
 static int nc_affine_launch(const float *x, const float *a, const float *b, float *y, int N, int P, int C, int relu, void *stream_, float *amax)
@@ -489,18 +514,28 @@
 }
 
 static int nc_affine2_launch(const float *dy, const float *x, const float *y, const float *a, const float *p, const float *r,
-                             float *dx, int N, int P, int C, int relu, void *stream_, float *amax)
+                             float *dx, int N, int P, int C, int relu, void *stream_, float *amax, const float *fa = nullptr,
+                             const float *fb = nullptr)
 {
   int rc = nc_check(N, P, C, "pd_nc_affine2_f32");
   if (amax && C != 256) return pd_set_error(PD_ERR_INVALID_ARG, "pd_nc_affine2_amax_f32: pixel maxima need C == 256");
   if (rc) return rc;
   const int64_t n4 = (int64_t)N * P * C / 4;
   if (n4 == 0) return PD_OK;
-  if (!dy || !x || !a || !p || !r || !dx || (relu && !y)) return pd_set_error(PD_ERR_INVALID_ARG, "pd_nc_affine2_f32: null pointer");
+  const bool xmask = relu && fa && fb;
+  if (!dy || !x || !a || !p || !r || !dx || (relu && !y && !xmask)) return pd_set_error(PD_ERR_INVALID_ARG, "pd_nc_affine2_f32: null pointer");
   hipStream_t s = (hipStream_t)stream_;
-  if (relu) hipLaunchKernelGGL(nc_affine2<true>, dim3(grid_for(n4)), dim3(256), 0, s, (const float4 *)dy, (const float4 *)x, (const float4 *)y, a, p, r, (float4 *)dx, n4, P, C, amax);
-  else hipLaunchKernelGGL(nc_affine2<false>, dim3(grid_for(n4)), dim3(256), 0, s, (const float4 *)dy, (const float4 *)x, (const float4 *)y, a, p, r, (float4 *)dx, n4, P, C, amax);
+  if (xmask) hipLaunchKernelGGL(nc_affine2<2>, dim3(grid_for(n4)), dim3(256), 0, s, (const float4 *)dy, (const float4 *)x, (const float4 *)y, a, p, r, (float4 *)dx, n4, P, C, amax, fa, fb);
+  else if (relu) hipLaunchKernelGGL(nc_affine2<1>, dim3(grid_for(n4)), dim3(256), 0, s, (const float4 *)dy, (const float4 *)x, (const float4 *)y, a, p, r, (float4 *)dx, n4, P, C, amax, fa, fb);
+  else hipLaunchKernelGGL(nc_affine2<0>, dim3(grid_for(n4)), dim3(256), 0, s, (const float4 *)dy, (const float4 *)x, (const float4 *)y, a, p, r, (float4 *)dx, n4, P, C, amax, fa, fb);
   return pd_check_launch("pd_nc_affine2_f32");
+}
+
+extern "C" int pd_nc_affine2_xmask_f32(const float *dy, const float *x, const float *fa, const float *fb, const float *a, const float *p,
+                                       const float *r, float *dx, float *amax, int N, int P, int C, void *stream_)
+{
+  if (!fa || !fb) return pd_set_error(PD_ERR_INVALID_ARG, "pd_nc_affine2_xmask_f32: null forward coefficients");
+  return nc_affine2_launch(dy, x, nullptr, a, p, r, dx, N, P, C, 1, stream_, amax, fa, fb);
 }
 
 extern "C" int pd_nc_affine2_f32(const float *dy, const float *x, const float *y, const float *a, const float *p, const float *r,
diff --git a/partdistillation_amd/csrc/gemm_f16x2.hip b/partdistillation_amd/csrc/gemm_f16x2.hip
--- a/partdistillation_amd/csrc/gemm_f16x2.hip
+++ b/partdistillation_amd/csrc/gemm_f16x2.hip
@@ -40,6 +40,9 @@
   h16_t *smem = reinterpret_cast<h16_t *>(sc + 2 * (TM + TN));
   auto As = [&](int buf, int pl, int pan, int r) -> h16_t * { return smem + buf * (ASZ + BSZ) + (((pl * NPAN + pan) * TM + r) << 3); };
   auto Bs = [&](int buf, int pl, int pan, int r) -> h16_t * { return smem + buf * (ASZ + BSZ) + ASZ + (((pl * NPAN + pan) * TN + r) << 3); };
+  if (gridDim.y > 1) {
+    A += (int64_t)blockIdx.y * K; B += (int64_t)blockIdx.y * K; C += (int64_t)blockIdx.y * M * ldc;
+  }
   const int lb = xcd_chunk(blockIdx.x, gridDim.x);
   const int m0 = (lb / ntiles_n) * TM, n0 = (lb % ntiles_n) * TN;
   const int t = threadIdx.x, lane = t & 63, wave = t >> 6;
@@ -1088,6 +1091,104 @@
   return gemm_tn_f16x2_impl(A, B, bias, reinterpret_cast<float *>(C_bf16), nullptr, nullptr, a_amax, b_amax, nullptr, M, N, K, lda, ldb, ldc, 0, stream_, 1);
 }
 
+int g_pd_dbg_splitk_tiles = 0;
+
+static int f16x2_splitk_slices(int M, int N, int K, int ncu, int dbg_tiles)
+{
+  if (M <= 0 || N <= 0 || K < 1024 || (N & 3) || N > 1024 || (256 % (N >> 2)) != 0) return 1;
+  const int64_t tiles = (int64_t)((M + 127) / 128) * ((N + 127) / 128);
+  if (dbg_tiles < 0 || tiles > (dbg_tiles > 0 ? dbg_tiles : ncu / 2)) return 1;
+  int S = 1;
+  while (S < 8 && tiles * (2 * S) <= ncu && (K % (2 * S)) == 0 && ((K / (2 * S)) % 32) == 0 && K / (2 * S) >= 256) S *= 2;
+  return S;
+}
+
+namespace {
+template <int S>
+__global__ __launch_bounds__(256) void gemm_tn_f16x2_splitk_reduce(const float *__restrict__ ws, const float *__restrict__ bias, float *__restrict__ C,
+                                                                   double *__restrict__ sums, int M, int N, int ldc, int P, int rpb)
+{
+  __shared__ float red[2][256][4];
+  const int img = blockIdx.y, cq = N >> 2, q = threadIdx.x % cq, po = threadIdx.x / cq, pstride = 256 / cq;
+  const int p0 = blockIdx.x * rpb, p1 = min(P, p0 + rpb);
+  const int64_t slab = (int64_t)M * N;
+  const float4 bv = bias ? *reinterpret_cast<const float4 *>(bias + q * 4) : make_float4(0.f, 0.f, 0.f, 0.f);
+  float4 s0 = make_float4(0.f, 0.f, 0.f, 0.f), s1 = s0;
+  for (int p = p0 + po; p < p1; p += pstride) {
+    const int64_t row = (int64_t)img * P + p;
+    const float *src = ws + row * N + q * 4;
+    float4 u[S];
+#pragma unroll
+    for (int s = 0; s < S; ++s) u[s] = *reinterpret_cast<const float4 *>(src + s * slab);
+    float4 v = u[0];
+#pragma unroll
+    for (int s = 1; s < S; ++s) { v.x += u[s].x; v.y += u[s].y; v.z += u[s].z; v.w += u[s].w; }
+    v.x += bv.x; v.y += bv.y; v.z += bv.z; v.w += bv.w;
+    *reinterpret_cast<float4 *>(C + row * ldc + q * 4) = v;
+    s0.x += v.x; s0.y += v.y; s0.z += v.z; s0.w += v.w;
+    s1.x += v.x * v.x; s1.y += v.y * v.y; s1.z += v.z * v.z; s1.w += v.w * v.w;
+  }
+  if (!sums) return;
+  red[0][threadIdx.x][0] = s0.x; red[0][threadIdx.x][1] = s0.y; red[0][threadIdx.x][2] = s0.z; red[0][threadIdx.x][3] = s0.w;
+  red[1][threadIdx.x][0] = s1.x; red[1][threadIdx.x][1] = s1.y; red[1][threadIdx.x][2] = s1.z; red[1][threadIdx.x][3] = s1.w;
+  __syncthreads();
+  if (threadIdx.x < N) {
+    const int c = threadIdx.x, qq = c >> 2, e = c & 3;
+    double t0 = 0, t1 = 0;
+    for (int k = 0; k < pstride; ++k) { t0 += red[0][k * cq + qq][e]; t1 += red[1][k * cq + qq][e]; }
+    unsafeAtomicAdd(sums + ((int64_t)img * N + c) * 2, t0);
+    unsafeAtomicAdd(sums + ((int64_t)img * N + c) * 2 + 1, t1);
+  }
+}
+}
+
+extern "C" int pd_gemm_tn_f16x2_splitk_slices(int M, int N, int K)
+{
+  return f16x2_splitk_slices(M, N, K, cu_count(), g_pd_dbg_splitk_tiles);
+}
+
+extern "C" int pd_gemm_tn_f16x2_splitk_slices_cu(int M, int N, int K, int cu)
+{
+  return f16x2_splitk_slices(M, N, K, cu, 0);
+}
+
+extern "C" int pd_gemm_tn_f16x2_splitk(const float *A, const float *B, const float *bias, float *C, const float *a_amax, const float *b_amax,
+                                       float *workspace, int64_t workspace_floats, double *sums, int rows_per_image, int M, int N, int K, int lda,
+                                       int ldb, int ldc, int S, void *stream_)
+{
+  if (M < 0 || N <= 0 || K <= 0) return pd_set_error(PD_ERR_INVALID_ARG, "pd_gemm_tn_f16x2_splitk: M=%d N=%d K=%d", M, N, K);
+  if (S != 2 && S != 4 && S != 8) return pd_set_error(PD_ERR_INVALID_ARG, "pd_gemm_tn_f16x2_splitk: %d slices (2, 4 or 8; one slice is pd_gemm_tn_f16x2)", S);
+  if ((K % S) != 0 || ((K / S) % 16) != 0)
+    return pd_set_error(PD_ERR_INVALID_ARG, "pd_gemm_tn_f16x2_splitk: K = %d in %d slices: a slice must be a multiple of the 16-deep step", K, S);
+  if ((N & 3) || N > 1024 || (256 % (N >> 2)) != 0 || (ldc & 3) || ldc < N)
+    return pd_set_error(PD_ERR_INVALID_ARG, "pd_gemm_tn_f16x2_splitk: N=%d (4 * 2^k <= 1024), ldc=%d (>= N, a multiple of 4)", N, ldc);
+  if (M == 0) return PD_OK;
+  if (!A || !B || !C || !workspace) return pd_set_error(PD_ERR_INVALID_ARG, "pd_gemm_tn_f16x2_splitk: null pointer");
+  if ((lda & 3) || (ldb & 3) || lda < K || ldb < K || ((uintptr_t)A & 15) || ((uintptr_t)B & 15) || ((uintptr_t)C & 15) || ((uintptr_t)workspace & 15) ||
+      (bias && ((uintptr_t)bias & 15)))
+    return pd_set_error(PD_ERR_INVALID_ARG, "pd_gemm_tn_f16x2_splitk: lda, ldb multiples of 4 and >= K; A, B, C, bias, workspace 16-byte aligned");
+  if (workspace_floats < (int64_t)S * M * N) return pd_set_error(PD_ERR_INVALID_ARG, "pd_gemm_tn_f16x2_splitk: workspace of %lld floats, %lld needed", (long long)workspace_floats, (long long)S * M * N);
+  if (sums && (N > 256 || rows_per_image <= 0 || (M % rows_per_image) != 0))
+    return pd_set_error(PD_ERR_INVALID_ARG, "pd_gemm_tn_f16x2_splitk: statistics need N <= 256 and M = images x rows_per_image (M=%d, %d rows)", M, rows_per_image);
+  hipStream_t st = (hipStream_t)stream_;
+  constexpr int TM = 128, TN = 128, NTH = 256;
+  constexpr size_t stage = (size_t)2 * 2 * (TM + TN) * 16 * sizeof(h16_t), red = (size_t)(NTH / 64) * 64 * 33 * sizeof(float);
+  constexpr size_t lds = (stage > red ? stage : red) + (size_t)2 * (TM + TN) * sizeof(float);
+  const int tn = (N + TN - 1) / TN, tm = (M + TM - 1) / TM;
+  hipLaunchKernelGGL((gemm_tn_f16x2<128, 128, 64, 16, 0, false, 2, 1>), dim3((unsigned)((int64_t)tm * tn), (unsigned)S), dim3(NTH), lds, st, A, B,
+                     (const float *)nullptr, workspace, M, N, K / S, lda, ldb, N, tn, (uint32_t *)nullptr, (float *)nullptr, a_amax, b_amax,
+                     (unsigned *)nullptr, 0, 0, 1);
+  int rc = pd_check_launch("pd_gemm_tn_f16x2_splitk");
+  if (rc) return rc;
+  const int P = sums ? rows_per_image : M, images = sums ? M / rows_per_image : 1;
+  const int rpb = M >= 8192 ? 32 : 16;
+  const dim3 grid((unsigned)((P + rpb - 1) / rpb), (unsigned)images);
+#define REDUCE(NS) hipLaunchKernelGGL(gemm_tn_f16x2_splitk_reduce<NS>, grid, dim3(256), 0, st, workspace, bias, C, sums, M, N, ldc, P, rpb)
+  if (S == 2) REDUCE(2); else if (S == 4) REDUCE(4); else REDUCE(8);
+#undef REDUCE
+  return pd_check_launch("pd_gemm_tn_f16x2_splitk (reduce)");
+}
+
 extern "C" int pd_cast_bf16_f32_amax(const void *X_bf16, int rows, int cols, float *Y, float *row_amax, void *stream_)
 {
   if (rows < 0 || cols <= 0 || (cols & 7)) return pd_set_error(PD_ERR_INVALID_ARG, "pd_cast_bf16_f32_amax: rows=%d cols=%d (a multiple of 8)", rows, cols);
diff --git a/partdistillation_amd/csrc/rowwise.hip b/partdistillation_amd/csrc/rowwise.hip
--- a/partdistillation_amd/csrc/rowwise.hip
+++ b/partdistillation_amd/csrc/rowwise.hip
@@ -682,9 +682,11 @@
   l0 = 1.f - l1;
 }
 
+template <bool AFFINE>
 __global__ __launch_bounds__(256) void upsample_add_nhwc(const float *__restrict__ lo, const float *__restrict__ cur,
                                                          float *__restrict__ y, int B, int h, int w, int H, int W, int C4,
-                                                         float sh, float sw, float *__restrict__ amax, int64_t lo_bs4)
+                                                         float sh, float sw, float *__restrict__ amax, int64_t lo_bs4,
+                                                         const float *__restrict__ ga, const float *__restrict__ gb)
 {
   const int64_t total = (int64_t)B * H * W * C4;
   for (int64_t i = (int64_t)blockIdx.x * blockDim.x + threadIdx.x; i < total; i += (int64_t)gridDim.x * blockDim.x) {
@@ -699,7 +701,11 @@
     const float4 *L = reinterpret_cast<const float4 *>(lo) + (int64_t)b * lo_bs4;
     const float4 a = L[((int64_t)y0 * w + x0) * C4 + c], bq = L[((int64_t)y0 * w + x0 + xp) * C4 + c];
     const float4 cq = L[((int64_t)(y0 + yp) * w + x0) * C4 + c], d = L[((int64_t)(y0 + yp) * w + x0 + xp) * C4 + c];
-    const float4 u = reinterpret_cast<const float4 *>(cur)[i];
+    float4 u = reinterpret_cast<const float4 *>(cur)[i];
+    if (AFFINE) {
+      const float4 av = reinterpret_cast<const float4 *>(ga)[b * C4 + c], bv = reinterpret_cast<const float4 *>(gb)[b * C4 + c];
+      u.x = u.x * av.x + bv.x; u.y = u.y * av.y + bv.y; u.z = u.z * av.z + bv.z; u.w = u.w * av.w + bv.w;
+    }
     float4 o;
     o.x = u.x + (hy0 * (wx0 * a.x + wx1 * bq.x) + hy1 * (wx0 * cq.x + wx1 * d.x));
     o.y = u.y + (hy0 * (wx0 * a.y + wx1 * bq.y) + hy1 * (wx0 * cq.y + wx1 * d.y));
@@ -1157,7 +1163,8 @@
   return pd_check_launch("pd_point_sample_nhwc_f32_bf16");
 }
 
-static int upsample_add_launch(const float *lo, int64_t lo_bs, const float *cur, float *y, int B, int h, int w, int H, int W, int C, void *stream_, float *amax)
+static int upsample_add_launch(const float *lo, int64_t lo_bs, const float *cur, float *y, int B, int h, int w, int H, int W, int C, void *stream_, float *amax,
+                               const float *ga = nullptr, const float *gb = nullptr)
 {
   if (lo_bs == 0) lo_bs = (int64_t)h * w * C;
   if (lo_bs < (int64_t)h * w * C || (lo_bs & 3)) return pd_set_error(PD_ERR_INVALID_ARG, "pd_upsample_add_nhwc_f32: lo_batch_stride %lld (>= h w C, a multiple of 4)", (long long)lo_bs);
@@ -1167,9 +1174,18 @@
   if (!lo || !cur || !y) return pd_set_error(PD_ERR_INVALID_ARG, "pd_upsample_add_nhwc_f32: null pointer");
   const int64_t total = (int64_t)B * H * W * (C / 4);
   const unsigned grid = (unsigned)((total + 255) / 256 < 32768 ? (total + 255) / 256 : 32768);
-  hipLaunchKernelGGL(upsample_add_nhwc, dim3(grid), dim3(256), 0, (hipStream_t)stream_, lo, cur, y, B, h, w, H, W, C / 4,
-                     (float)h / (float)H, (float)w / (float)W, amax, lo_bs / 4);
+  if (ga) hipLaunchKernelGGL(upsample_add_nhwc<true>, dim3(grid), dim3(256), 0, (hipStream_t)stream_, lo, cur, y, B, h, w, H, W, C / 4,
+                             (float)h / (float)H, (float)w / (float)W, amax, lo_bs / 4, ga, gb);
+  else hipLaunchKernelGGL(upsample_add_nhwc<false>, dim3(grid), dim3(256), 0, (hipStream_t)stream_, lo, cur, y, B, h, w, H, W, C / 4,
+                          (float)h / (float)H, (float)w / (float)W, amax, lo_bs / 4, ga, gb);
   return pd_check_launch("pd_upsample_add_nhwc_f32");
+}
+
+extern "C" int pd_upsample_add_affine_nhwc_f32(const float *lo, int64_t lo_batch_stride, const float *x, const float *a, const float *b, float *y, float *amax,
+                                               int B, int h, int w, int H, int W, int C, void *stream_)
+{
+  if (!a || !b) return pd_set_error(PD_ERR_INVALID_ARG, "pd_upsample_add_affine_nhwc_f32: null coefficients");
+  return upsample_add_launch(lo, lo_batch_stride, x, y, B, h, w, H, W, C, stream_, amax, a, b);
 }
 
 extern "C" int pd_upsample_add_nhwc_f32(const float *lo, int64_t lo_batch_stride, const float *cur, float *y, int B, int h, int w, int H, int W, int C,
diff --git a/partdistillation_amd/functions/conv_x3.py b/partdistillation_amd/functions/conv_x3.py
--- a/partdistillation_amd/functions/conv_x3.py
+++ b/partdistillation_amd/functions/conv_x3.py
@@ -92,11 +92,11 @@
 class Conv1x1OwnWgrad(Function):
 
     @staticmethod
-    def forward(ctx, x, weight, bias):
+    def forward(ctx, x, weight, bias, split=None):
         ctx.has_bias = bias is not None
         ctx.x_bf16 = x.dtype == torch.bfloat16
         if H2 and H2_1X1 and x.is_contiguous(memory_format=torch.channels_last):
-            from .gemm import cast_rows_amax, gemm_tn_h2, row_amax
+            from .gemm import cast_rows_amax, gemm_tn_h2, gemm_tn_h2_splitk, row_amax
             B, ci, Hh, Ww = x.shape
             co = weight.shape[0]
             if ctx.x_bf16:
@@ -105,9 +105,13 @@
             else:
                 x_am = _pixel_amax(x)
             w2 = weight.reshape(co, ci)
-            y = gemm_tn_h2(x.permute(0, 2, 3, 1).reshape(-1, ci), w2, bias, a_amax=x_am, b_amax=row_amax(w2))
+            if split is not None:
+                y = gemm_tn_h2_splitk(x.permute(0, 2, 3, 1).reshape(-1, ci), w2, bias, x_am, row_amax(w2), split[0], split[1], Hh * Ww)
+            else:
+                y = gemm_tn_h2(x.permute(0, 2, 3, 1).reshape(-1, ci), w2, bias, a_amax=x_am, b_amax=row_amax(w2))
             ctx.save_for_backward(x, weight, x_am)
             return y.view(B, Hh, Ww, co).permute(0, 3, 1, 2)
+        assert split is None
         if ctx.x_bf16:
             x = x.float()
         ctx.save_for_backward(x, weight, None)
@@ -142,7 +146,7 @@
                 gemm_wgrad_acc(rows(dy), rows(x), dw2, dbv if want_b else None, x3=True)
             dw = dw2.view(co, ci, 1, 1).as_strided(weight.shape, weight.stride()) if want_w else None
             db = dbv if want_b else None
-        return dx, dw, db
+        return dx, dw, db, None
 
 
 def conv1x1_supported(x, conv):
@@ -153,5 +157,13 @@
             and x.is_contiguous(memory_format=torch.channels_last) and torch.is_grad_enabled())
 
 
-def conv1x1(x, weight, bias=None):
-    return Conv1x1OwnWgrad.apply(x, weight, bias)
+def conv1x1_slices(x, conv):
+    if not (H2 and H2_1X1 and x.is_contiguous(memory_format=torch.channels_last)):
+        return 1
+    from .gemm import h2_splitk_slices
+    B, ci, Hh, Ww = x.shape
+    return h2_splitk_slices(B * Hh * Ww, conv.weight.shape[0], ci)
+
+
+def conv1x1(x, weight, bias=None, split=None):
+    return Conv1x1OwnWgrad.apply(x, weight, bias, split)
diff --git a/partdistillation_amd/functions/fused.py b/partdistillation_amd/functions/fused.py
--- a/partdistillation_amd/functions/fused.py
+++ b/partdistillation_amd/functions/fused.py
@@ -1,3 +1,5 @@
+import os
+
 import numpy as np
 import torch
 from torch.autograd import Function
@@ -288,20 +290,95 @@
         _lib.check(rc)
 
 
+PDSHELL_FUSED = bool(int(os.environ.get("PD_PDSHELL_FUSED", "1")))
+
+
+class GNSumsPool:
+
+    def __init__(self, slots):
+        self.slots, self.buf, self.n, self.i = slots, None, 0, 0
+
+    def take(self, N, C, device):
+        n = N * C * 2
+        if self.buf is None:
+            self.buf, self.n = torch.zeros(self.slots * n, dtype=torch.float64, device=device), n
+        if n != self.n or self.i >= self.slots or self.buf.device != device:
+            return torch.zeros((N, C, 2), dtype=torch.float64, device=device)
+        self.i += 1
+        return self.buf[(self.i - 1) * n:self.i * n].view(N, C, 2)
+
+
+def _gn_coef_fwd(ctx, x, weight, bias, groups, eps, pool, sums=None):
+    N, C, H, W = x.shape
+    P = H * W
+    lib = _lib.load()
+    st = _stream()
+    coef = torch.empty((5, N, C), dtype=torch.float32, device=x.device)
+    if sums is not None:
+        assert pool is not None and sums.shape == (N, C, 2) and sums.dtype == torch.float64
+    elif pool is None:
+        sums = torch.empty((N, C, 2), dtype=torch.float64, device=x.device)
+        _lib.check(lib.pd_nc_sums_f32(x.data_ptr(), None, None, None, None, sums.data_ptr(), N, P, C, 0, 0, st))
+    else:
+        sums = pool.take(N, C, x.device)
+        _lib.check(lib.pd_nc_sums_acc_f32(x.data_ptr(), None, None, None, None, None, None, sums.data_ptr(), N, P, C, 0, 0, st))
+    ctx.bsums = pool.take(N, C, x.device) if pool is not None and any(ctx.needs_input_grad[:3]) else None
+    ctx.pooled = pool is not None
+    _lib.check(lib.pd_gn_coeffs_fwd(sums.data_ptr(), weight.data_ptr(), bias.data_ptr(), N, C, groups, P, float(eps),
+                                    coef[0].data_ptr(), coef[1].data_ptr(), coef[2].data_ptr(), coef[3].data_ptr(),
+                                    coef[4].data_ptr(), st))
+    return coef
+
+
+def _gn_backward(ctx, gy, x, y, weight, coef, relu):
+    N, C, H, W = x.shape
+    P, G = H * W, ctx.groups
+    gy = _nhwc(gy)
+    lib = _lib.load()
+    st = _stream()
+    mean_c, rstd_c, xb = coef[2], coef[3], coef[4]
+    xmask = relu and ctx.pooled
+    if ctx.pooled:
+        sums, ctx.bsums = ctx.bsums, None
+        if sums is None:
+            sums = torch.zeros((N, C, 2), dtype=torch.float64, device=x.device)
+        _lib.check(lib.pd_nc_sums_acc_f32(x.data_ptr(), gy.data_ptr(), None, rstd_c.data_ptr(), xb.data_ptr(),
+                                          coef[0].data_ptr() if xmask else None, coef[1].data_ptr() if xmask else None,
+                                          sums.data_ptr(), N, P, C, 1, int(relu), st))
+    else:
+        sums = torch.empty((N, C, 2), dtype=torch.float64, device=x.device)
+        _lib.check(lib.pd_nc_sums_f32(x.data_ptr(), gy.data_ptr(), y.data_ptr() if y is not None else None, rstd_c.data_ptr(),
+                                      xb.data_ptr(), sums.data_ptr(), N, P, C, 1, int(relu), st))
+    out = torch.empty((3 * N * C + 2 * C,), dtype=torch.float32, device=x.device)
+    a, pc, rc = out[:N * C], out[N * C:2 * N * C], out[2 * N * C:3 * N * C]
+    gw, gb = out[3 * N * C:3 * N * C + C], out[3 * N * C + C:]
+    _lib.check(lib.pd_gn_coeffs_bwd(sums.data_ptr(), weight.data_ptr(), mean_c.data_ptr(), rstd_c.data_ptr(), N, C, G, P,
+                                    a.data_ptr(), pc.data_ptr(), rc.data_ptr(), gw.data_ptr(), gb.data_ptr(), st))
+    dx = torch.empty_like(x, memory_format=torch.channels_last)
+    am = torch.empty(N * P, dtype=torch.float32, device=x.device) if C == 256 else None
+    if xmask:
+        _lib.check(lib.pd_nc_affine2_xmask_f32(gy.data_ptr(), x.data_ptr(), coef[0].data_ptr(), coef[1].data_ptr(), a.data_ptr(), pc.data_ptr(),
+                                               rc.data_ptr(), dx.data_ptr(), am.data_ptr() if am is not None else None, N, P, C, st))
+    elif C == 256:
+        _lib.check(lib.pd_nc_affine2_amax_f32(gy.data_ptr(), x.data_ptr(), y.data_ptr() if y is not None else None, a.data_ptr(),
+                                              pc.data_ptr(), rc.data_ptr(), dx.data_ptr(), am.data_ptr(), N, P, C, int(relu), st))
+    else:
+        _lib.check(lib.pd_nc_affine2_f32(gy.data_ptr(), x.data_ptr(), y.data_ptr() if y is not None else None, a.data_ptr(),
+                                         pc.data_ptr(), rc.data_ptr(), dx.data_ptr(), N, P, C, int(relu), st))
+    if am is not None:
+        amax_cache.put(dx, am)
+    return dx, gw, gb
+
+
 class GroupNormNHWC(Function):
 
     @staticmethod
-    def forward(ctx, x, weight, bias, groups, eps, relu):
+    def forward(ctx, x, weight, bias, groups, eps, relu, pool=None, sums=None):
         N, C, H, W = x.shape
         P = H * W
         lib = _lib.load()
         st = _stream()
-        sums = torch.empty((N, C, 2), dtype=torch.float64, device=x.device)
-        coef = torch.empty((5, N, C), dtype=torch.float32, device=x.device)
-        _lib.check(lib.pd_nc_sums_f32(x.data_ptr(), None, None, None, None, sums.data_ptr(), N, P, C, 0, 0, st))
-        _lib.check(lib.pd_gn_coeffs_fwd(sums.data_ptr(), weight.data_ptr(), bias.data_ptr(), N, C, groups, P, float(eps),
-                                        coef[0].data_ptr(), coef[1].data_ptr(), coef[2].data_ptr(), coef[3].data_ptr(),
-                                        coef[4].data_ptr(), st))
+        coef = _gn_coef_fwd(ctx, x, weight, bias, groups, eps, pool, sums)
         y = torch.empty_like(x, memory_format=torch.channels_last)
         if C == 256:
             am = torch.empty(N * P, dtype=torch.float32, device=x.device)
@@ -310,37 +387,48 @@
         else:
             _lib.check(lib.pd_nc_affine_f32(x.data_ptr(), coef[0].data_ptr(), coef[1].data_ptr(), y.data_ptr(), N, P, C, int(relu), st))
             ctx.y_am = None
-        ctx.save_for_backward(x, y if relu else None, weight, coef)
+        ctx.save_for_backward(x, y if relu and pool is None else None, weight, coef)
         ctx.groups, ctx.relu = groups, relu
         return y
 
     @staticmethod
     def backward(ctx, gy):
         x, y, weight, coef = ctx.saved_tensors
+        dx, gw, gb = _gn_backward(ctx, gy, x, y, weight, coef, ctx.relu)
+        return dx, gw, gb, None, None, None, None, None
+
+
+class GroupNormUpsampleAdd(Function):
+
+    @staticmethod
+    def forward(ctx, x, weight, bias, groups, eps, lo, pool):
         N, C, H, W = x.shape
-        P, G = H * W, ctx.groups
-        gy = _nhwc(gy)
-        lib = _lib.load()
-        st = _stream()
-        mean_c, rstd_c, xb = coef[2], coef[3], coef[4]
-        sums = torch.empty((N, C, 2), dtype=torch.float64, device=x.device)
-        _lib.check(lib.pd_nc_sums_f32(x.data_ptr(), gy.data_ptr(), y.data_ptr() if y is not None else None, rstd_c.data_ptr(),
-                                      xb.data_ptr(), sums.data_ptr(), N, P, C, 1, int(ctx.relu), st))
-        out = torch.empty((3 * N * C + 2 * C,), dtype=torch.float32, device=x.device)
-        a, pc, rc = out[:N * C], out[N * C:2 * N * C], out[2 * N * C:3 * N * C]
-        gw, gb = out[3 * N * C:3 * N * C + C], out[3 * N * C + C:]
-        _lib.check(lib.pd_gn_coeffs_bwd(sums.data_ptr(), weight.data_ptr(), mean_c.data_ptr(), rstd_c.data_ptr(), N, C, G, P,
-                                        a.data_ptr(), pc.data_ptr(), rc.data_ptr(), gw.data_ptr(), gb.data_ptr(), st))
-        dx = torch.empty_like(x, memory_format=torch.channels_last)
-        if C == 256:
-            am = torch.empty(N * P, dtype=torch.float32, device=x.device)
-            _lib.check(lib.pd_nc_affine2_amax_f32(gy.data_ptr(), x.data_ptr(), y.data_ptr() if y is not None else None, a.data_ptr(),
-                                                  pc.data_ptr(), rc.data_ptr(), dx.data_ptr(), am.data_ptr(), N, P, C, int(ctx.relu), st))
-            amax_cache.put(dx, am)
+        h, w = lo.shape[-2:]
+        coef = _gn_coef_fwd(ctx, x, weight, bias, groups, eps, pool)
+        if lo.stride()[1:] == (1, w * C, C) and lo.stride(0) >= h * w * C and lo.stride(0) % 4 == 0:
+            lo_c, lo_bs = lo, lo.stride(0)
         else:
-            _lib.check(lib.pd_nc_affine2_f32(gy.data_ptr(), x.data_ptr(), y.data_ptr() if y is not None else None, a.data_ptr(),
-                                             pc.data_ptr(), rc.data_ptr(), dx.data_ptr(), N, P, C, int(ctx.relu), st))
-        return dx, gw, gb, None, None, None
+            lo_c, lo_bs = lo.contiguous(memory_format=torch.channels_last), 0
+        y = torch.empty_like(x, memory_format=torch.channels_last)
+        am = torch.empty(N * H * W, dtype=torch.float32, device=x.device) if C == 256 else None
+        _lib.check(_lib.load().pd_upsample_add_affine_nhwc_f32(lo_c.data_ptr(), lo_bs, x.data_ptr(), coef[0].data_ptr(), coef[1].data_ptr(), y.data_ptr(),
+                                                               am.data_ptr() if am is not None else None, N, h, w, H, W, C, _stream()))
+        ctx.y_am = am
+        ctx.save_for_backward(x, weight, coef)
+        ctx.groups, ctx.lo_dims = groups, (N, C, h, w)
+        return y
+
+    @staticmethod
+    def backward(ctx, dy):
+        x, weight, coef = ctx.saved_tensors
+        B, C, h, w = ctx.lo_dims
+        dy = _nhwc(dy)
+        dlo = None
+        if ctx.needs_input_grad[5]:
+            dlo = torch.empty((B, C, h, w), dtype=torch.float32, device=dy.device, memory_format=torch.channels_last)
+            _lib.check(_lib.load().pd_upsample2x_bwd_nhwc_f32(dy.data_ptr(), dlo.data_ptr(), B, h, w, C, _stream()))
+        dx, gw, gb = _gn_backward(ctx, dy, x, None, weight, coef, False)
+        return dx, gw, gb, None, None, dlo, None
 
 
 def group_norm_nhwc_supported(x, groups):
@@ -349,11 +437,21 @@
             and C % groups == 0 and not torch.is_autocast_enabled())
 
 
-def group_norm_nhwc(x, weight, bias, groups=32, eps=1e-5, relu=False):
+def group_norm_nhwc(x, weight, bias, groups=32, eps=1e-5, relu=False, pool=None, sums=None):
     if not group_norm_nhwc_supported(x, groups):
         raise RuntimeError("pd group norm: fp32 CUDA NCHW-shaped tensor with C = 4*2^k <= 256 required (no fallback here)")
-    y = GroupNormNHWC.apply(_nhwc(x), weight, bias, groups, eps, relu)
+    y = GroupNormNHWC.apply(_nhwc(x), weight, bias, groups, eps, relu, pool, sums)
     am = getattr(y.grad_fn, "y_am", None) if y.grad_fn is not None else None
     if am is not None:
         amax_cache.put(y, am)
     return y
+
+
+def group_norm_upsample_add(x, weight, bias, lo, groups=32, eps=1e-5, pool=None):
+    if not group_norm_nhwc_supported(x, groups):
+        raise RuntimeError("pd group norm: fp32 CUDA NCHW-shaped tensor with C = 4*2^k <= 256 required (no fallback here)")
+    y = GroupNormUpsampleAdd.apply(_nhwc(x), weight, bias, groups, eps, lo, pool)
+    am = getattr(y.grad_fn, "y_am", None) if y.grad_fn is not None else None
+    if am is not None:
+        amax_cache.put(y, am)
+    return y
diff --git a/partdistillation_amd/functions/gemm.py b/partdistillation_amd/functions/gemm.py
--- a/partdistillation_amd/functions/gemm.py
+++ b/partdistillation_amd/functions/gemm.py
@@ -115,6 +115,25 @@
     with _timed_fwd(2.0 * M * N * K, label, 4.0 * (M * K + N * K + M * N)):
         _lib.check(L.pd_gemm_tn_f16x2(*args))
     return (c, bits) if (mode == 1 and want_bits) else c
+
+
+def h2_splitk_slices(M, N, K):
+    return int(_lib.load().pd_gemm_tn_f16x2_splitk_slices(M, N, K))
+
+
+def gemm_tn_h2_splitk(a, b, bias, a_amax, b_amax, slices, sums=None, rows_per_image=0):
+    assert a.is_cuda and a.dtype == torch.float32 and b.dtype == torch.float32 and a.stride(1) == 1 and b.stride(1) == 1
+    M, K = a.shape
+    N = b.shape[0]
+    assert b.shape[1] == K
+    L = _lib.load()
+    c = torch.empty((M, N), dtype=torch.float32, device=a.device)
+    ws = torch.empty(slices * M * N, dtype=torch.float32, device=a.device)
+    p = lambda t: t.data_ptr() if t is not None else None
+    with _timed_fwd(2.0 * M * N * K, f"gemm_tn_f16x2<128, 128, 64, 16, 0> split K x {slices} + reduce", 4.0 * (M * K + N * K + M * N)):
+        _lib.check(L.pd_gemm_tn_f16x2_splitk(a.data_ptr(), b.data_ptr(), p(bias), c.data_ptr(), p(a_amax), p(b_amax), ws.data_ptr(), ws.numel(),
+                                             p(sums), rows_per_image, M, N, K, a.stride(0), b.stride(0), N, slices, _stream()))
+    return c
 
 
 def split3(w, transpose=False):
diff --git a/partdistillation_amd/lib.py b/partdistillation_amd/lib.py
--- a/partdistillation_amd/lib.py
+++ b/partdistillation_amd/lib.py
@@ -7,7 +7,7 @@
 CSRC = os.path.join(_HERE, "csrc")
 
 PD_F32, PD_F64, PD_BF16 = 0, 1, 2
-ABI_VERSION = 49
+ABI_VERSION = 50
 
 _c_int, _c_vp = ctypes.c_int, ctypes.c_void_p
 
@@ -36,6 +36,9 @@
     "pd_gemm_tn_f16x2_which": (_c_int, [_c_int] * 11),
     "pd_gemm_tn_f16x2_bits_words": (ctypes.c_int64, [_c_int] * 2),
     "pd_gemm_tn_f16x2": (_c_int, [_c_vp] * 9 + [_c_int] * 7 + [_c_vp]),
+    "pd_gemm_tn_f16x2_splitk_slices": (_c_int, [_c_int] * 3),
+    "pd_gemm_tn_f16x2_splitk_slices_cu": (_c_int, [_c_int] * 4),
+    "pd_gemm_tn_f16x2_splitk": (_c_int, [_c_vp] * 7 + [ctypes.c_int64, _c_vp] + [_c_int] * 8 + [_c_vp]),
     "pd_gemm_tn_f16x2_bf16out": (_c_int, [_c_vp] * 6 + [_c_int] * 6 + [_c_vp]),
     "pd_cast_bf16_f32_amax": (_c_int, [_c_vp, _c_int, _c_int, _c_vp, _c_vp, _c_vp]),
     "pd_row_amax_f32": (_c_int, [_c_vp, _c_int, _c_int, _c_int, _c_vp, _c_vp]),
@@ -75,6 +78,9 @@
     "pd_attn_fwd_d32_ld": (_c_int, [_c_vp] * 7 + [_c_int] * 4 + [ctypes.c_float, _c_int, _c_int, _c_vp]),
     "pd_attn_bwd_d32_ld": (_c_int, [_c_vp] * 11 + [_c_int] * 4 + [ctypes.c_float, _c_int, _c_int, _c_vp]),
     "pd_nc_sums_f32": (_c_int, [_c_vp] * 6 + [_c_int] * 5 + [_c_vp]),
+    "pd_nc_sums_acc_f32": (_c_int, [_c_vp] * 8 + [_c_int] * 5 + [_c_vp]),
+    "pd_nc_affine2_xmask_f32": (_c_int, [_c_vp] * 9 + [_c_int] * 3 + [_c_vp]),
+    "pd_upsample_add_affine_nhwc_f32": (_c_int, [_c_vp, ctypes.c_int64] + [_c_vp] * 5 + [_c_int] * 6 + [_c_vp]),
     "pd_nc_affine_f32": (_c_int, [_c_vp] * 4 + [_c_int] * 4 + [_c_vp]),
     "pd_nc_affine_amax_f32": (_c_int, [_c_vp] * 5 + [_c_int] * 4 + [_c_vp]),
     "pd_nc_affine2_amax_f32": (_c_int, [_c_vp] * 8 + [_c_int] * 4 + [_c_vp]),
diff --git a/partdistillation_amd/modeling/pixel_decoder/msdeformattn.py b/partdistillation_amd/modeling/pixel_decoder/msdeformattn.py
--- a/partdistillation_amd/modeling/pixel_decoder/msdeformattn.py
+++ b/partdistillation_amd/modeling/pixel_decoder/msdeformattn.py
@@ -10,7 +10,8 @@
 from ...compat.layers import Conv2d, c2_xavier_fill, get_norm
 from ..transformer_decoder.position_encoding import PositionEmbeddingSine
 from ...functions import conv_x3
-from ...functions.fused import group_norm_nhwc, group_norm_nhwc_supported
+from ...functions import fused
+from ...functions.fused import group_norm_nhwc, group_norm_nhwc_supported, group_norm_upsample_add
 from ...functions.gemm import linear_f32
 from .ops.modules import MSDeformAttn
 from ...functions.encoder_core import EncoderCore, EncoderSpec
@@ -217,15 +218,26 @@
     return x.float()
 
 
-def _conv_gn(conv, gn, x, relu=False):
+def _conv(conv, x):
     if CONV_X3 and conv_x3.supported(x, conv):
-        y = conv_x3.conv3x3(x, conv.weight, conv.bias)
-    elif CONV_X3 and conv_x3.conv1x1_supported(x, conv):
-        y = conv_x3.conv1x1(x, conv.weight, conv.bias)
-    else:
-        y = F.conv2d(x, conv.weight, conv.bias, conv.stride, conv.padding, conv.dilation, conv.groups)
+        return conv_x3.conv3x3(x, conv.weight, conv.bias)
+    if CONV_X3 and conv_x3.conv1x1_supported(x, conv):
+        return conv_x3.conv1x1(x, conv.weight, conv.bias)
+    return F.conv2d(x, conv.weight, conv.bias, conv.stride, conv.padding, conv.dilation, conv.groups)
+
+
+def _conv_gn(conv, gn, x, relu=False, pool=None):
+    co = conv.weight.shape[0]
+    if (pool is not None and CONV_X3 and isinstance(gn, nn.GroupNorm) and conv_x3.conv1x1_supported(x, conv) and not torch.is_autocast_enabled()
+            and co % 4 == 0 and co <= 256 and 256 % (co // 4) == 0 and co % gn.num_groups == 0):
+        slices = conv_x3.conv1x1_slices(x, conv)
+        if slices > 1:
+            sums = pool.take(x.shape[0], co, x.device)
+            y = conv_x3.conv1x1(x, conv.weight, conv.bias, (slices, sums))
+            return group_norm_nhwc(y, gn.weight, gn.bias, gn.num_groups, gn.eps, relu, pool, sums)
+    y = _conv(conv, x)
     if isinstance(gn, nn.GroupNorm) and group_norm_nhwc_supported(y, gn.num_groups):
-        return group_norm_nhwc(y, gn.weight, gn.bias, gn.num_groups, gn.eps, relu)
+        return group_norm_nhwc(y, gn.weight, gn.bias, gn.num_groups, gn.eps, relu, pool)
     if gn is not None:
         y = gn(y)
     return F.relu(y) if relu else y
@@ -295,9 +307,11 @@
     def forward_features(self, features):
         with torch.autocast(device_type=next(iter(features.values())).device.type, enabled=False):
             srcs, pos = [], []
+            n_gn = len(self.transformer_in_features) + 2 * self.num_fpn_levels
+            pool = fused.GNSumsPool(2 * n_gn) if fused.PDSHELL_FUSED and next(iter(features.values())).is_cuda else None
             for idx, f in enumerate(self.transformer_in_features[::-1]):
                 x = _as_fp32_input(features[f], self.input_proj[idx][0])
-                srcs.append(_conv_gn(self.input_proj[idx][0], self.input_proj[idx][1], x))
+                srcs.append(_conv_gn(self.input_proj[idx][0], self.input_proj[idx][1], x, pool=pool))
                 pos.append(self.pe_layer(x))
             y, spatial_shapes, level_start_index, shapes_host = self.transformer(srcs, pos)
             bs = y.shape[0]
@@ -306,12 +320,16 @@
             for idx, f in enumerate(self.in_features[: self.num_fpn_levels][::-1]):
                 x = _as_fp32_input(features[f], self.lateral_convs[idx])
                 lat, outc = self.lateral_convs[idx], self.output_convs[idx]
-                cur = _conv_gn(lat, lat.norm, x, relu=lat.activation is not None)
-                if upsample_add_supported(out[-1], cur):
-                    y = upsample_add(out[-1], cur)
+                cur = _conv(lat, x) if pool is not None and isinstance(lat.norm, nn.GroupNorm) and lat.activation is None else None
+                if cur is not None and group_norm_nhwc_supported(cur, lat.norm.num_groups) and upsample_add_supported(out[-1], cur):
+                    y = group_norm_upsample_add(cur, lat.norm.weight, lat.norm.bias, out[-1], lat.norm.num_groups, lat.norm.eps, pool)
                 else:
-                    y = cur + F.interpolate(out[-1], size=cur.shape[-2:], mode="bilinear", align_corners=False)
-                out.append(_conv_gn(outc, outc.norm, y, relu=outc.activation is not None))
+                    cur = _conv_gn(lat, lat.norm, x, relu=lat.activation is not None, pool=pool)
+                    if upsample_add_supported(out[-1], cur):
+                        y = upsample_add(out[-1], cur)
+                    else:
+                        y = cur + F.interpolate(out[-1], size=cur.shape[-2:], mode="bilinear", align_corners=False)
+                out.append(_conv_gn(outc, outc.norm, y, relu=outc.activation is not None, pool=pool))
             multi_scale = out[: self.maskformer_num_feature_levels]
             mf = self.mask_features
             if CONV_X3 and mf.norm is None and mf.activation is None and conv_x3.conv1x1_supported(out[-1], mf):
```

After: 109.2, median of 6. No clear change (+0.6%).
